# igmsalinas/unet-rir

Hardware: AMD Instinct MI355X
Metric: RIR spectrograms/sec (train step) on [B,2,256,256] U-Net (higher is better)
Workload: dtype bf16; 1 GPU; UNet 4 down/4 up, number_filters_0=64, kernels=3, per-GPU batch 32 of [2,256,256] + [2,16] (BASELINE.json configs[1] per GPU; global batch 32), full train step: fwd + loss + bwd + grad all-reduce + Adam; bf16 activations/gradients, fp32 accumulate/statistics/master weights; global_batch=32, parallelism=dp1, rccl_world_size=1, params=68613058, driven_by=Trainer.step(UNetEngine), schedule=side-stream weight gradients + bucket-wise Adam

## Files before the change

### include/unetrir.h

```cpp
#ifndef UNETRIR_H
#define UNETRIR_H

#include <stddef.h>
#include <stdint.h>

#ifdef __cplusplus
extern "C" {
#endif

#define UNETRIR_EINVAL 10001
#define UNETRIR_ABI_VERSION 1

typedef void* unetrir_stream_t;
typedef uint16_t unetrir_bf16;

typedef struct {
    int B, H, W;
    int Cin, Cout;
    int k;
    int stride;
} unetrir_conv_geom;

int unetrir_abi_version(void);

typedef struct {
    int conv3x3, conv3x3g, conv3x3g_pair, conv3x3h, conv3x3s, conv3x3r, stem, upconv3x3g, wgrad3x3g, wgrad3x3r, head_mfma,
        wgrad3x3d, conv3x3d, conv3x3p, upconv3x3q, dyn_tiles, pw1x1, igemm2;
} unetrir_config;
int unetrir_get_config(unetrir_config* out);
int unetrir_set_config(const unetrir_config* in);
int unetrir_reset_tile_tickets(void);

int unetrir_conv2d_fwd_f32(const unetrir_conv_geom* g, const float* x, int ldx, const float* w,
                           const float* bias, const float* addend, int ldadd, float* y, int ldy,
                           unetrir_stream_t stream);
int unetrir_conv2d_dgrad_f32(const unetrir_conv_geom* g, const float* dy, int lddy, const float* wt,
                             const float* addend, int ldadd, float* dx, int lddx,
                             unetrir_stream_t stream);
size_t unetrir_conv2d_wgrad_ws_bytes(const unetrir_conv_geom* g);
int unetrir_conv2d_wgrad_f32(const unetrir_conv_geom* g, const float* x, int ldx, const float* dy,
                             int lddy, float* dw, float reg_coef, const float* w, void* ws,
                             size_t ws_bytes, unetrir_stream_t stream);

int unetrir_conv2d_transpose_fwd_f32(const unetrir_conv_geom* g, const float* x, int ldx,
                                     const float* wt, const float* bias, float* y, int ldy,
                                     unetrir_stream_t stream);
int unetrir_conv2d_transpose_dgrad_f32(const unetrir_conv_geom* g, const float* dy, int lddy,
                                       const float* w, const float* addend, int ldadd, float* dx,
                                       int lddx, unetrir_stream_t stream);
size_t unetrir_conv2d_transpose_wgrad_ws_bytes(const unetrir_conv_geom* g);
int unetrir_conv2d_transpose_wgrad_f32(const unetrir_conv_geom* g, const float* x, int ldx,
                                       const float* dy, int lddy, float* dw, float reg_coef,
                                       const float* w, void* ws, size_t ws_bytes,
                                       unetrir_stream_t stream);

size_t unetrir_dense_fwd_ws_bytes(int B, int K, int N);
int unetrir_dense_fwd_f32(const float* x, int ldx, const float* w, const float* bias, float* y, int ldy, int B, int K,
                          int N, void* ws, size_t ws_bytes, unetrir_stream_t stream);
int unetrir_dense_dgrad_supported(int B, int K, int N);
size_t unetrir_dense_dgrad_ws_bytes(int B, int K, int N);
int unetrir_dense_dgrad_f32(const float* dy, int lddy, const float* w, float* dx, int lddx, int B, int K, int N, void* ws,
                            size_t ws_bytes, unetrir_stream_t stream);

int unetrir_transpose_weight_f32(const float* w, float* wt, int N, int T, int C,
                                 unetrir_stream_t stream);

size_t unetrir_bn_ws_bytes(long long P, int C);
int unetrir_bn_stats_f32(const float* x, int ldx, long long P, int C, const float* gamma,
                         const float* beta, float eps, float momentum, float* moving_mean,
                         float* moving_var, float* affine, float* saved, void* ws, size_t ws_bytes,
                         unetrir_stream_t stream);
int unetrir_bn_apply_f32(const float* x, int ldx, long long P, int C, const float* affine, int relu,
                         float* y, int ldy, unetrir_stream_t stream);
int unetrir_bn_bwd_f32(const float* da, int ldda, const float* x, int ldx, long long P, int C,
                       const float* gamma, const float* affine, const float* saved, int relu,
                       float* dx, int lddx, float* dgamma, float* dbeta, void* ws, size_t ws_bytes,
                       unetrir_stream_t stream);
int unetrir_colsum_f32(const float* x, int ldx, long long P, int C, float* out, void* ws,
                       size_t ws_bytes, unetrir_stream_t stream);
int unetrir_relu_fwd_f32(const float* x, int ldx, long long P, int C, float* y, int ldy,
                         unetrir_stream_t stream);
int unetrir_relu_bwd_f32(const float* da, int ldda, const float* x, int ldx, long long P, int C,
                         float* dx, int lddx, unetrir_stream_t stream);

int unetrir_bn_act_add_f32(const float* x, int ldx, long long P, int C, const float* affine, int act,
                           const float* addend, int ldadd, float* y, int ldy, unetrir_stream_t stream);
int unetrir_act_bwd_f32(const float* da, int ldda, const float* out, int ldo, long long P, int C, int act, float* g,
                        int ldg, unetrir_stream_t stream);
int unetrir_add_f32(const float* a, const float* b, float* y, long long n, unetrir_stream_t stream);
int unetrir_bn_bwd_junction_f32(const float* da, int ldda, const float* x, int ldx, const float* out, int ldo, long long P, int C,
                                const float* affine, const float* saved, int act, float* dx, int lddx, float* gskip, int ldgs,
                                const float* gskip_add, int ldga, float* dgamma, float* dbeta, void* ws, size_t ws_bytes,
                                unetrir_stream_t stream);

int unetrir_nchw_to_nhwc_pad_f32(const float* x, int B, int C, int H, int W, float* y, int Cpad,
                                 unetrir_stream_t stream);

size_t unetrir_loss_ws_bytes(long long npix);
int unetrir_sigmoid_loss_f32(const float* logits, int ldl, const float* target, int B, int H, int W,
                             float alpha, float inv_norm, float* pred, float* dlogits,
                             float* loss_out, void* ws, size_t ws_bytes, unetrir_stream_t stream);
int unetrir_sigmoid_loss_ex_f32(const float* logits, int ldl, const float* target, const float* phase_ref,
                                const float* phase_weight, int B, int H, int W, float alpha, float inv_norm, float* pred,
                                float* dlogits, float* loss_out, void* ws, size_t ws_bytes, unetrir_stream_t stream);
int unetrir_sigmoid_nchw_f32(const float* logits, int ldl, int B, int H, int W, float* pred,
                             unetrir_stream_t stream);
int unetrir_sigmoid_bwd_f32(const float* pred, const float* dpred, int B, int H, int W,
                            float* dlogits, unetrir_stream_t stream);

int unetrir_head6x6_supported(int C);
int unetrir_head6x6_fwd_f32(const float* x, int ldx, int B, int H, int W, int C, const float* w, const float* bias,
                            float* y, int ldy, unetrir_stream_t stream);
size_t unetrir_head6x6_wgrad_ws_bytes(int C);
int unetrir_head6x6_wgrad_f32(const float* x, int ldx, int B, int H, int W, int C, const float* dy, int lddy,
                              float* dw, void* ws, size_t ws_bytes, unetrir_stream_t stream);

int unetrir_embedding_fwd_f32(const int* idx, int n_idx, const float* table, int vocab, int dim,
                              float* out, unetrir_stream_t stream);
int unetrir_embedding_bwd_f32(const int* idx, int n_idx, const float* dout, int vocab, int dim,
                              float* dtable, unetrir_stream_t stream);
int unetrir_mul_f32(const float* x, const float* m, float* y, long long n, unetrir_stream_t stream);
int unetrir_sumsq_f32(const float* x, long long n, float coef, float* out, int accumulate,
                      void* ws, size_t ws_bytes, unetrir_stream_t stream);

int unetrir_adam_f32(float* theta, const float* g, float* m, float* v, long long n, float lr_t,
                     float beta1, float beta2, float eps, float grad_scale,
                     unetrir_stream_t stream);

int unetrir_sgd_f32(float* theta, const float* g, long long n, float lr, float grad_scale, unetrir_stream_t stream);
int unetrir_nadam_f32(float* theta, const float* g, float* m, float* v, long long n, float lr, float beta1, float beta2, float eps,
                      float c_g, float c_m, float c_v, float grad_scale, unetrir_stream_t stream);

int unetrir_step_advance(unsigned long long* state, const float* cfg, float* hyper, int n_draws, int advance_t,
                         unetrir_stream_t stream);
int unetrir_adam_dev_f32(float* theta, const float* g, float* m, float* v, long long n, const float* hyper,
                         unetrir_stream_t stream);
int unetrir_dropout_mask_dev_f32(float* mask, long long n, float p, unsigned long long seed,
                                 const unsigned long long* step_base, unsigned long long step_offset, unetrir_stream_t stream);

int unetrir_conv2d_fwd_bf16(const unetrir_conv_geom* g, const unetrir_bf16* x, int ldx, const unetrir_bf16* w,
                            const float* bias, const unetrir_bf16* addend, int ldadd, unetrir_bf16* y, int ldy,
                            unetrir_stream_t stream);
int unetrir_conv2d_dgrad_bf16(const unetrir_conv_geom* g, const unetrir_bf16* dy, int lddy, const unetrir_bf16* wt,
                              const unetrir_bf16* addend, int ldadd, unetrir_bf16* dx, int lddx,
                              unetrir_stream_t stream);
int unetrir_conv2d_wgrad_bf16(const unetrir_conv_geom* g, const unetrir_bf16* x, int ldx, const unetrir_bf16* dy,
                              int lddy, float* dw, float reg_coef, const float* w, void* ws, size_t ws_bytes,
                              unetrir_stream_t stream);
int unetrir_conv2d_transpose_fwd_bf16(const unetrir_conv_geom* g, const unetrir_bf16* x, int ldx,
                                      const unetrir_bf16* wt, const float* bias, unetrir_bf16* y, int ldy,
                                      unetrir_stream_t stream);
int unetrir_conv2d_transpose_dgrad_bf16(const unetrir_conv_geom* g, const unetrir_bf16* dy, int lddy,
                                        const unetrir_bf16* w, const unetrir_bf16* addend, int ldadd,
                                        unetrir_bf16* dx, int lddx, unetrir_stream_t stream);
int unetrir_conv2d_transpose_wgrad_bf16(const unetrir_conv_geom* g, const unetrir_bf16* x, int ldx,
                                        const unetrir_bf16* dy, int lddy, float* dw, float reg_coef, const float* w,
                                        void* ws, size_t ws_bytes, unetrir_stream_t stream);
typedef struct unetrir_reduce_desc {
    const float* part;
    int nsplit;
    size_t n;
    float* out;
    float reg;
    const float* w;
} unetrir_reduce_desc;
int unetrir_conv2d_wgrad_partials_bf16(const unetrir_conv_geom* g, const unetrir_bf16* x, int ldx, const unetrir_bf16* dy,
                                       int lddy, float* dw, float reg_coef, const float* w, void* ws, size_t ws_bytes,
                                       unetrir_reduce_desc* desc, unetrir_stream_t stream);
int unetrir_conv2d_transpose_wgrad_partials_bf16(const unetrir_conv_geom* g, const unetrir_bf16* x, int ldx,
                                                 const unetrir_bf16* dy, int lddy, float* dw, float reg_coef, const float* w,
                                                 void* ws, size_t ws_bytes, unetrir_reduce_desc* desc, unetrir_stream_t stream);
int unetrir_splitk_reduce_batched(const unetrir_reduce_desc* desc, int n, unetrir_stream_t stream);
size_t unetrir_conv3x3s2_packed_elems(int N, int C);
int unetrir_conv2d_fwd_packed_bf16(const unetrir_conv_geom* g, const unetrir_bf16* x, int ldx, const unetrir_bf16* w,
                                   const unetrir_bf16* w_packed, const float* bias, const unetrir_bf16* addend, int ldadd,
                                   unetrir_bf16* y, int ldy, unetrir_stream_t stream);
int unetrir_conv2d_transpose_dgrad_packed_bf16(const unetrir_conv_geom* g, const unetrir_bf16* dy, int lddy,
                                               const unetrir_bf16* w, const unetrir_bf16* w_packed,
                                               const unetrir_bf16* addend, int ldadd, unetrir_bf16* dx, int lddx,
                                               unetrir_stream_t stream);
int unetrir_cast_weight_bf16(const float* w, unetrir_bf16* o, int N, int T, int C, int Cp, unetrir_stream_t stream);
int unetrir_transpose_cast_weight_bf16(const float* w, unetrir_bf16* wt, int N, int T, int C, int Np,
                                       unetrir_stream_t stream);
typedef struct unetrir_cast_desc {
    const float* w;
    unetrir_bf16* same;
    unetrir_bf16* transposed;
    int N, T, C, Cp, Np, reserved;
    unetrir_bf16* packed_s2;
} unetrir_cast_desc;
int unetrir_cast_weights_batched_bf16(const unetrir_cast_desc* desc, int n_layers, unetrir_stream_t stream);
int unetrir_bn_stats_bf16(const unetrir_bf16* x, int ldx, long long P, int C, const float* gamma, const float* beta,
                          float eps, float momentum, float* moving_mean, float* moving_var, float* affine,
                          float* saved, void* ws, size_t ws_bytes, unetrir_stream_t stream);
int unetrir_bn_apply_bf16(const unetrir_bf16* x, int ldx, long long P, int C, const float* affine, int relu,
                          unetrir_bf16* y, int ldy, unetrir_stream_t stream);
int unetrir_bn_bwd_bf16(const unetrir_bf16* da, int ldda, const unetrir_bf16* x, int ldx, long long P, int C,
                        const float* affine, const float* saved, int relu, unetrir_bf16* dx, int lddx, float* dgamma,
                        float* dbeta, void* ws, size_t ws_bytes, unetrir_stream_t stream);
int unetrir_colsum_bf16(const unetrir_bf16* x, int ldx, long long P, int C, float* out, void* ws, size_t ws_bytes,
                        unetrir_stream_t stream);
int unetrir_relu_bwd_bf16(const unetrir_bf16* da, int ldda, const unetrir_bf16* x, int ldx, long long P, int C,
                          unetrir_bf16* dx, int lddx, unetrir_stream_t stream);
int unetrir_nchw_to_nhwc_pad_bf16(const float* x, int B, int C, int H, int W, unetrir_bf16* y, int Cpad,
                                  unetrir_stream_t stream);
int unetrir_head6x6_fwd_bf16(const unetrir_bf16* x, int ldx, int B, int H, int W, int C, const float* w,
                             const float* bias, float* y, int ldy, unetrir_stream_t stream);
int unetrir_head6x6_wgrad_bf16(const unetrir_bf16* x, int ldx, int B, int H, int W, int C, const unetrir_bf16* dy,
                               int lddy, float* dw, void* ws, size_t ws_bytes, unetrir_stream_t stream);
long long unetrir_conv2d_colstat_rows_bf16(const unetrir_conv_geom* g, int dgrad, int ld_in);
enum { UNETRIR_K3_TAPTABLE = 0, UNETRIR_K3_CONV3X3R = 1, UNETRIR_K3_CONV3X3G = 2, UNETRIR_K3_CONV3X3G_PAIR = 3, UNETRIR_K3_CONV3X3H = 4,
       UNETRIR_K3_CONV3X3S = 5, UNETRIR_K3_CONV3X3P = 6, UNETRIR_K3_STEM = 7, UNETRIR_K3_PATCH = 8 };
int unetrir_conv3x3_kernel_id_bf16(const unetrir_conv_geom* g, int dgrad, int ld_in);
int unetrir_conv2d_fwd_colstat_bf16(const unetrir_conv_geom* g, const unetrir_bf16* x, int ldx, const unetrir_bf16* w,
                                    const float* bias, const unetrir_bf16* addend, int ldadd, unetrir_bf16* y, int ldy,
                                    float* colstat, unetrir_stream_t stream);
int unetrir_conv2d_dgrad_colstat_bf16(const unetrir_conv_geom* g, const unetrir_bf16* dy, int lddy, const unetrir_bf16* wt,
                                      const unetrir_bf16* addend, int ldadd, unetrir_bf16* dx, int lddx, float* colstat,
                                      unetrir_stream_t stream);
long long unetrir_conv2d_transpose_colstat_rows_bf16(const unetrir_conv_geom* g, int ld_in);
int unetrir_conv2d_transpose_fwd_colstat_bf16(const unetrir_conv_geom* g, const unetrir_bf16* x, int ldx, const unetrir_bf16* wt,
                                              const float* bias, unetrir_bf16* y, int ldy, float* colstat,
                                              unetrir_stream_t stream);
int unetrir_bn_stats_colstat(const float* colstat, long long rows, long long P, int C, const float* gamma, const float* beta,
                             float eps, float momentum, float* moving_mean, float* moving_var, float* affine, float* saved,
                             unetrir_stream_t stream);
int unetrir_colsum_colstat(const float* colstat, long long rows, int ldc, int c0, int C, float* out, unetrir_stream_t stream);
int unetrir_bn_colstat_act_add_f32(const float* colstat, long long rows, const float* x, int ldx, long long P, int C, const float* gamma,
                                   const float* beta, float eps, float momentum, float* moving_mean, float* moving_var, float* affine,
                                   float* saved, int act, const float* addend, int ldadd, float* y, int ldy, unetrir_stream_t stream);
int unetrir_bn_colstat_act_add_bf16(const float* colstat, long long rows, const unetrir_bf16* x, int ldx, long long P, int C,
                                    const float* gamma, const float* beta, float eps, float momentum, float* moving_mean,
                                    float* moving_var, float* affine, float* saved, int act, const unetrir_bf16* addend, int ldadd,
                                    unetrir_bf16* y, int ldy, unetrir_stream_t stream);
int unetrir_head6x6_dgrad_supported(int W, int C);
int unetrir_head6x6_dgrad_bf16(const unetrir_bf16* dy, int lddy, int B, int H, int W, const float* w, int C,
                               unetrir_bf16* dx, int lddx, unetrir_stream_t stream);
int unetrir_sigmoid_loss_bf16(const float* logits, int ldl, const float* target, int B, int H, int W, float alpha,
                              float inv_norm, float* pred, unetrir_bf16* dlogits, float* loss_out, void* ws,
                              size_t ws_bytes, unetrir_stream_t stream);
int unetrir_sigmoid_loss_ex_bf16(const float* logits, int ldl, const float* target, const float* phase_ref,
                                 const float* phase_weight, int B, int H, int W, float alpha, float inv_norm, float* pred,
                                 unetrir_bf16* dlogits, float* loss_out, void* ws, size_t ws_bytes, unetrir_stream_t stream);
int unetrir_sigmoid_bwd_bf16(const float* pred, const float* dpred, int B, int H, int W, unetrir_bf16* dlogits,
                             unetrir_stream_t stream);
int unetrir_add_f32_to_bf16(const unetrir_bf16* a, const float* b, unetrir_bf16* y, long long n,
                            unetrir_stream_t stream);
int unetrir_cast_bf16_to_f32(const unetrir_bf16* a, float* y, long long n, unetrir_stream_t stream);
int unetrir_cast_f32_to_bf16(const float* a, unetrir_bf16* y, long long n, unetrir_stream_t stream);
int unetrir_bn_act_add_bf16(const unetrir_bf16* x, int ldx, long long P, int C, const float* affine, int act,
                            const unetrir_bf16* addend, int ldadd, unetrir_bf16* y, int ldy, unetrir_stream_t stream);
int unetrir_act_bwd_bf16(const unetrir_bf16* da, int ldda, const unetrir_bf16* out, int ldo, long long P, int C, int act,
                         unetrir_bf16* g, int ldg, unetrir_stream_t stream);
int unetrir_bn_bwd_junction_bf16(const unetrir_bf16* da, int ldda, const unetrir_bf16* x, int ldx, const unetrir_bf16* out, int ldo,
                                 long long P, int C, const float* affine, const float* saved, int act, unetrir_bf16* dx, int lddx,
                                 unetrir_bf16* gskip, int ldgs, const unetrir_bf16* gskip_add, int ldga, float* dgamma, float* dbeta,
                                 void* ws, size_t ws_bytes, unetrir_stream_t stream);

int unetrir_stft_frames(int T, int hop_length);
int unetrir_stft_features_f32(const float* wav, int B, int T, int n_fft, int win_length, int hop_length, int pad_mode,
                              int remove_mean, int normalize, float* out, int H, int W, unetrir_stream_t stream);
int unetrir_istft_features_f32(const float* feat, int B, int H, int W, int n_bins, int n_frames, int n_fft, int win_length,
                               int hop_length, int denormalize, float* wav, unetrir_stream_t stream);

int unetrir_eval_metrics_f32(const float* pred, const float* target, const float* phase_ref, int B, int H, int W,
                             const float* wav_pred, const float* wav_true, int T, int n50, double* out, unetrir_stream_t stream);
int unetrir_eval_accumulate(const double* out, const int* group, int B, int G, double* acc, unetrir_stream_t stream);

int unetrir_bn_inference_affine_f32(const float* gamma, const float* beta, const float* moving_mean, const float* moving_var,
                                    float eps, int C, float* affine, unetrir_stream_t stream);
int unetrir_dropout_mask_f32(float* mask, long long n, float p, unsigned long long seed, unsigned long long step,
                             unetrir_stream_t stream);
int unetrir_index_to_i32(const void* idx, int elem_bytes, long long n, int* out, unetrir_stream_t stream);

int unetrir_normal_f32(float* out, long long n, unsigned long long seed, unsigned long long step, unetrir_stream_t stream);
int unetrir_normal_dev_f32(float* out, long long n, unsigned long long seed, const unsigned long long* step_base,
                           unsigned long long step_offset, unetrir_stream_t stream);
int unetrir_vae_sample_kl_fwd_f32(const float* mu, int ld_mu, const float* log_var, int ld_lv, const float* eps, int B, int L,
                                  float inv_global_batch, float* z, int ld_z, float* kl_out, unetrir_stream_t stream);
int unetrir_vae_sample_kl_bwd_f32(const float* mu, int ld_mu, const float* log_var, int ld_lv, const float* eps, const float* dz,
                                  int ld_dz, int B, int L, float inv_global_batch, float* dmu, int ld_dmu, float* dlv, int ld_dlv,
                                  unetrir_stream_t stream);
int unetrir_vae_loss_add_f32(const float* kl_out, float* loss_out, unetrir_stream_t stream);

int unetrir_stage_h2d(int n, const void* const* src, void* const* pinned, void* const* dev, const size_t* bytes,
                      unetrir_stream_t stream);

int unetrir_gather_batch_f32(const float* bank, long long N, long long row_elems, const int32_t* emb_bank, int emb_len,
                             const float* wav_bank, long long wav_len, const int32_t* room_bank, const int32_t* idx_in,
                             const int32_t* idx_out, int B, float* spec_in, float* spec_out, int32_t* emb, float* wav_true,
                             int32_t* room, unetrir_stream_t stream);

size_t unetrir_griffinlim_ws_bytes(int B, int n_bins, int n_frames, int n_fft);
int unetrir_griffinlim_f32(const float* feat, int B, int H, int W, int n_bins, int n_frames, int n_fft, int win_length,
                           int hop_length, int pad_mode, int denormalize, int n_iter, float momentum, const float* init_phase,
                           unsigned long long seed, unsigned long long draw, float* wav, void* ws, size_t ws_bytes,
                           unetrir_stream_t stream);
int unetrir_uniform_f32(float* out, long long n, unsigned long long seed, unsigned long long step, unetrir_stream_t stream);

#define UNETRIR_PROF_FAMILIES 8
enum { UNETRIR_FAM_CONV_FWD = 0, UNETRIR_FAM_CONV_DGRAD = 1, UNETRIR_FAM_CONV_WGRAD = 2,
       UNETRIR_FAM_BN = 3, UNETRIR_FAM_OTHER = 4, UNETRIR_FAM_SMALL_CHANNEL = 5,
       UNETRIR_FAM_DOMINANT = 6  };
int unetrir_prof_enable(int on);
int unetrir_prof_collect(int* counts, double* ms, double* flops);

#ifdef __cplusplus
}
#endif
#endif
```

### unet-rir_amd/_lib.py

```python
import ctypes as C
import os

from . import build as _build

_LIB = None

c_f32p = C.c_void_p
c_stream = C.c_void_p


class CastDesc(C.Structure):
    _fields_ = [("w", C.c_void_p), ("same", C.c_void_p), ("transposed", C.c_void_p), ("N", C.c_int), ("T", C.c_int), ("C", C.c_int),
                ("Cp", C.c_int), ("Np", C.c_int), ("reserved", C.c_int), ("packed_s2", C.c_void_p)]


class ReduceDesc(C.Structure):
    _fields_ = [("part", C.c_void_p), ("nsplit", C.c_int), ("n", C.c_size_t), ("out", C.c_void_p), ("reg", C.c_float), ("w", C.c_void_p)]


class Config(C.Structure):
    _fields_ = [(n, C.c_int) for n in ("conv3x3", "conv3x3g", "conv3x3g_pair", "conv3x3h", "conv3x3s", "conv3x3r", "stem",
                                       "upconv3x3g", "wgrad3x3g", "wgrad3x3r", "head_mfma", "wgrad3x3d", "conv3x3d", "conv3x3p", "upconv3x3q", "dyn_tiles", "pw1x1", "igemm2")]


class ConvGeom(C.Structure):
    _fields_ = [("B", C.c_int), ("H", C.c_int), ("W", C.c_int), ("Cin", C.c_int), ("Cout", C.c_int),
                ("k", C.c_int), ("stride", C.c_int)]


_SIGS = {
    "unetrir_abi_version": (C.c_int, []),
    "unetrir_get_config": (C.c_int, [C.POINTER(Config)]),
    "unetrir_set_config": (C.c_int, [C.POINTER(Config)]),
    "unetrir_conv2d_fwd_f32": (C.c_int, [C.POINTER(ConvGeom), c_f32p, C.c_int, c_f32p, c_f32p, c_f32p, C.c_int,
                                         c_f32p, C.c_int, c_stream]),
    "unetrir_conv2d_dgrad_f32": (C.c_int, [C.POINTER(ConvGeom), c_f32p, C.c_int, c_f32p, c_f32p, C.c_int, c_f32p,
                                           C.c_int, c_stream]),
    "unetrir_conv2d_wgrad_ws_bytes": (C.c_size_t, [C.POINTER(ConvGeom)]),
    "unetrir_conv2d_wgrad_f32": (C.c_int, [C.POINTER(ConvGeom), c_f32p, C.c_int, c_f32p, C.c_int, c_f32p, C.c_float,
                                           c_f32p, C.c_void_p, C.c_size_t, c_stream]),
    "unetrir_conv2d_transpose_fwd_f32": (C.c_int, [C.POINTER(ConvGeom), c_f32p, C.c_int, c_f32p, c_f32p, c_f32p,
                                                   C.c_int, c_stream]),
    "unetrir_conv2d_transpose_dgrad_f32": (C.c_int, [C.POINTER(ConvGeom), c_f32p, C.c_int, c_f32p, c_f32p, C.c_int,
                                                     c_f32p, C.c_int, c_stream]),
    "unetrir_conv2d_transpose_wgrad_ws_bytes": (C.c_size_t, [C.POINTER(ConvGeom)]),
    "unetrir_conv2d_transpose_wgrad_f32": (C.c_int, [C.POINTER(ConvGeom), c_f32p, C.c_int, c_f32p, C.c_int, c_f32p,
                                                     C.c_float, c_f32p, C.c_void_p, C.c_size_t, c_stream]),
    "unetrir_dense_fwd_ws_bytes": (C.c_size_t, [C.c_int, C.c_int, C.c_int]),
    "unetrir_dense_fwd_f32": (C.c_int, [c_f32p, C.c_int, c_f32p, c_f32p, c_f32p, C.c_int, C.c_int, C.c_int, C.c_int,
                                        C.c_void_p, C.c_size_t, c_stream]),
    "unetrir_transpose_weight_f32": (C.c_int, [c_f32p, c_f32p, C.c_int, C.c_int, C.c_int, c_stream]),
    "unetrir_bn_ws_bytes": (C.c_size_t, [C.c_longlong, C.c_int]),
    "unetrir_bn_stats_f32": (C.c_int, [c_f32p, C.c_int, C.c_longlong, C.c_int, c_f32p, c_f32p, C.c_float, C.c_float,
                                       c_f32p, c_f32p, c_f32p, c_f32p, C.c_void_p, C.c_size_t, c_stream]),
    "unetrir_bn_apply_f32": (C.c_int, [c_f32p, C.c_int, C.c_longlong, C.c_int, c_f32p, C.c_int, c_f32p, C.c_int,
                                       c_stream]),
    "unetrir_bn_bwd_f32": (C.c_int, [c_f32p, C.c_int, c_f32p, C.c_int, C.c_longlong, C.c_int, c_f32p, c_f32p, c_f32p,
                                     C.c_int, c_f32p, C.c_int, c_f32p, c_f32p, C.c_void_p, C.c_size_t, c_stream]),
    "unetrir_colsum_f32": (C.c_int, [c_f32p, C.c_int, C.c_longlong, C.c_int, c_f32p, C.c_void_p, C.c_size_t,
                                     c_stream]),
    "unetrir_relu_fwd_f32": (C.c_int, [c_f32p, C.c_int, C.c_longlong, C.c_int, c_f32p, C.c_int, c_stream]),
    "unetrir_relu_bwd_f32": (C.c_int, [c_f32p, C.c_int, c_f32p, C.c_int, C.c_longlong, C.c_int, c_f32p, C.c_int,
                                       c_stream]),
    "unetrir_bn_act_add_f32": (C.c_int, [c_f32p, C.c_int, C.c_longlong, C.c_int, c_f32p, C.c_int, c_f32p, C.c_int, c_f32p,
                                         C.c_int, c_stream]),
    "unetrir_act_bwd_f32": (C.c_int, [c_f32p, C.c_int, c_f32p, C.c_int, C.c_longlong, C.c_int, C.c_int, c_f32p, C.c_int,
                                      c_stream]),
    "unetrir_add_f32": (C.c_int, [c_f32p, c_f32p, c_f32p, C.c_longlong, c_stream]),
    "unetrir_nchw_to_nhwc_pad_f32": (C.c_int, [c_f32p, C.c_int, C.c_int, C.c_int, C.c_int, c_f32p, C.c_int,
                                               c_stream]),
    "unetrir_head6x6_supported": (C.c_int, [C.c_int]),
    "unetrir_head6x6_fwd_f32": (C.c_int, [c_f32p, C.c_int, C.c_int, C.c_int, C.c_int, C.c_int, c_f32p, c_f32p, c_f32p,
                                          C.c_int, c_stream]),
    "unetrir_head6x6_wgrad_ws_bytes": (C.c_size_t, [C.c_int]),
    "unetrir_head6x6_wgrad_f32": (C.c_int, [c_f32p, C.c_int, C.c_int, C.c_int, C.c_int, C.c_int, c_f32p, C.c_int, c_f32p,
                                            C.c_void_p, C.c_size_t, c_stream]),
    "unetrir_loss_ws_bytes": (C.c_size_t, [C.c_longlong]),
    "unetrir_sigmoid_loss_f32": (C.c_int, [c_f32p, C.c_int, c_f32p, C.c_int, C.c_int, C.c_int, C.c_float, C.c_float,
                                           c_f32p, c_f32p, c_f32p, C.c_void_p, C.c_size_t, c_stream]),
    "unetrir_sigmoid_nchw_f32": (C.c_int, [c_f32p, C.c_int, C.c_int, C.c_int, C.c_int, c_f32p, c_stream]),
    "unetrir_sigmoid_bwd_f32": (C.c_int, [c_f32p, c_f32p, C.c_int, C.c_int, C.c_int, c_f32p, c_stream]),
    "unetrir_embedding_fwd_f32": (C.c_int, [C.c_void_p, C.c_int, c_f32p, C.c_int, C.c_int, c_f32p, c_stream]),
    "unetrir_embedding_bwd_f32": (C.c_int, [C.c_void_p, C.c_int, c_f32p, C.c_int, C.c_int, c_f32p, c_stream]),
    "unetrir_mul_f32": (C.c_int, [c_f32p, c_f32p, c_f32p, C.c_longlong, c_stream]),
    "unetrir_sumsq_f32": (C.c_int, [c_f32p, C.c_longlong, C.c_float, c_f32p, C.c_int, C.c_void_p, C.c_size_t,
                                    c_stream]),
    "unetrir_adam_f32": (C.c_int, [c_f32p, c_f32p, c_f32p, c_f32p, C.c_longlong, C.c_float, C.c_float, C.c_float,
                                   C.c_float, C.c_float, c_stream]),
    "unetrir_conv2d_fwd_bf16": (C.c_int, [C.POINTER(ConvGeom), c_f32p, C.c_int, c_f32p, c_f32p, c_f32p, C.c_int,
                                          c_f32p, C.c_int, c_stream]),
    "unetrir_conv3x3s2_packed_elems": (C.c_size_t, [C.c_int, C.c_int]),
    "unetrir_conv2d_fwd_packed_bf16": (C.c_int, [C.POINTER(ConvGeom), c_f32p, C.c_int, c_f32p, c_f32p, c_f32p, c_f32p, C.c_int,
                                                 c_f32p, C.c_int, c_stream]),
    "unetrir_conv2d_transpose_dgrad_packed_bf16": (C.c_int, [C.POINTER(ConvGeom), c_f32p, C.c_int, c_f32p, c_f32p, c_f32p, C.c_int,
                                                             c_f32p, C.c_int, c_stream]),
    "unetrir_conv2d_dgrad_bf16": (C.c_int, [C.POINTER(ConvGeom), c_f32p, C.c_int, c_f32p, c_f32p, C.c_int, c_f32p,
                                            C.c_int, c_stream]),
    "unetrir_conv2d_wgrad_bf16": (C.c_int, [C.POINTER(ConvGeom), c_f32p, C.c_int, c_f32p, C.c_int, c_f32p, C.c_float,
                                            c_f32p, C.c_void_p, C.c_size_t, c_stream]),
    "unetrir_conv2d_transpose_fwd_bf16": (C.c_int, [C.POINTER(ConvGeom), c_f32p, C.c_int, c_f32p, c_f32p, c_f32p,
                                                    C.c_int, c_stream]),
    "unetrir_conv2d_transpose_dgrad_bf16": (C.c_int, [C.POINTER(ConvGeom), c_f32p, C.c_int, c_f32p, c_f32p, C.c_int,
                                                      c_f32p, C.c_int, c_stream]),
    "unetrir_conv2d_wgrad_partials_bf16": (C.c_int, [C.POINTER(ConvGeom), c_f32p, C.c_int, c_f32p, C.c_int, c_f32p, C.c_float, c_f32p,
                                                     C.c_void_p, C.c_size_t, C.POINTER(ReduceDesc), c_stream]),
    "unetrir_conv2d_transpose_wgrad_partials_bf16": (C.c_int, [C.POINTER(ConvGeom), c_f32p, C.c_int, c_f32p, C.c_int, c_f32p, C.c_float,
                                                               c_f32p, C.c_void_p, C.c_size_t, C.POINTER(ReduceDesc), c_stream]),
    "unetrir_splitk_reduce_batched": (C.c_int, [C.POINTER(ReduceDesc), C.c_int, c_stream]),
    "unetrir_conv2d_transpose_wgrad_bf16": (C.c_int, [C.POINTER(ConvGeom), c_f32p, C.c_int, c_f32p, C.c_int, c_f32p,
                                                      C.c_float, c_f32p, C.c_void_p, C.c_size_t, c_stream]),
    "unetrir_cast_weight_bf16": (C.c_int, [c_f32p, c_f32p, C.c_int, C.c_int, C.c_int, C.c_int, c_stream]),
    "unetrir_transpose_cast_weight_bf16": (C.c_int, [c_f32p, c_f32p, C.c_int, C.c_int, C.c_int, C.c_int, c_stream]),
    "unetrir_bn_stats_bf16": (C.c_int, [c_f32p, C.c_int, C.c_longlong, C.c_int, c_f32p, c_f32p, C.c_float, C.c_float,
                                        c_f32p, c_f32p, c_f32p, c_f32p, C.c_void_p, C.c_size_t, c_stream]),
    "unetrir_bn_apply_bf16": (C.c_int, [c_f32p, C.c_int, C.c_longlong, C.c_int, c_f32p, C.c_int, c_f32p, C.c_int,
                                        c_stream]),
    "unetrir_bn_bwd_bf16": (C.c_int, [c_f32p, C.c_int, c_f32p, C.c_int, C.c_longlong, C.c_int, c_f32p, c_f32p,
                                      C.c_int, c_f32p, C.c_int, c_f32p, c_f32p, C.c_void_p, C.c_size_t, c_stream]),
    "unetrir_colsum_bf16": (C.c_int, [c_f32p, C.c_int, C.c_longlong, C.c_int, c_f32p, C.c_void_p, C.c_size_t,
                                      c_stream]),
    "unetrir_relu_bwd_bf16": (C.c_int, [c_f32p, C.c_int, c_f32p, C.c_int, C.c_longlong, C.c_int, c_f32p, C.c_int,
                                        c_stream]),
    "unetrir_nchw_to_nhwc_pad_bf16": (C.c_int, [c_f32p, C.c_int, C.c_int, C.c_int, C.c_int, c_f32p, C.c_int,
                                                c_stream]),
    "unetrir_head6x6_fwd_bf16": (C.c_int, [c_f32p, C.c_int, C.c_int, C.c_int, C.c_int, C.c_int, c_f32p, c_f32p, c_f32p,
                                           C.c_int, c_stream]),
    "unetrir_head6x6_wgrad_bf16": (C.c_int, [c_f32p, C.c_int, C.c_int, C.c_int, C.c_int, C.c_int, c_f32p, C.c_int,
                                             c_f32p, C.c_void_p, C.c_size_t, c_stream]),
    "unetrir_stage_h2d": (C.c_int, [C.c_int, C.POINTER(C.c_void_p), C.POINTER(C.c_void_p), C.POINTER(C.c_void_p), C.POINTER(C.c_size_t), c_stream]),
    "unetrir_conv2d_colstat_rows_bf16": (C.c_longlong, [C.POINTER(ConvGeom), C.c_int, C.c_int]),
    "unetrir_conv3x3_kernel_id_bf16": (C.c_int, [C.POINTER(ConvGeom), C.c_int, C.c_int]),
    "unetrir_conv2d_fwd_colstat_bf16": (C.c_int, [C.POINTER(ConvGeom), c_f32p, C.c_int, c_f32p, c_f32p, c_f32p, C.c_int, c_f32p, C.c_int,
                                                  c_f32p, c_stream]),
    "unetrir_conv2d_dgrad_colstat_bf16": (C.c_int, [C.POINTER(ConvGeom), c_f32p, C.c_int, c_f32p, c_f32p, C.c_int, c_f32p, C.c_int,
                                                    c_f32p, c_stream]),
    "unetrir_conv2d_transpose_colstat_rows_bf16": (C.c_longlong, [C.POINTER(ConvGeom), C.c_int]),
    "unetrir_conv2d_transpose_fwd_colstat_bf16": (C.c_int, [C.POINTER(ConvGeom), c_f32p, C.c_int, c_f32p, c_f32p, c_f32p, C.c_int, c_f32p,
                                                            c_stream]),
    "unetrir_bn_stats_colstat": (C.c_int, [c_f32p, C.c_longlong, C.c_longlong, C.c_int, c_f32p, c_f32p, C.c_float, C.c_float,
                                           c_f32p, c_f32p, c_f32p, c_f32p, c_stream]),
    "unetrir_bn_colstat_act_add_f32": (C.c_int, [c_f32p, C.c_longlong, c_f32p, C.c_int, C.c_longlong, C.c_int, c_f32p, c_f32p, C.c_float, C.c_float, c_f32p, c_f32p, c_f32p, c_f32p, C.c_int, c_f32p, C.c_int, c_f32p, C.c_int, c_stream]),
    "unetrir_bn_colstat_act_add_bf16": (C.c_int, [c_f32p, C.c_longlong, c_f32p, C.c_int, C.c_longlong, C.c_int, c_f32p, c_f32p, C.c_float, C.c_float, c_f32p, c_f32p, c_f32p, c_f32p, C.c_int, c_f32p, C.c_int, c_f32p, C.c_int, c_stream]),
    "unetrir_colsum_colstat": (C.c_int, [c_f32p, C.c_longlong, C.c_int, C.c_int, C.c_int, c_f32p, c_stream]),
    "unetrir_cast_weights_batched_bf16": (C.c_int, [C.c_void_p, C.c_int, c_stream]),
    "unetrir_dense_dgrad_supported": (C.c_int, [C.c_int, C.c_int, C.c_int]),
    "unetrir_dense_dgrad_ws_bytes": (C.c_size_t, [C.c_int, C.c_int, C.c_int]),
    "unetrir_dense_dgrad_f32": (C.c_int, [c_f32p, C.c_int, c_f32p, c_f32p, C.c_int, C.c_int, C.c_int, C.c_int, C.c_void_p, C.c_size_t,
                                          c_stream]),
    "unetrir_stft_frames": (C.c_int, [C.c_int, C.c_int]),
    "unetrir_stft_features_f32": (C.c_int, [c_f32p, C.c_int, C.c_int, C.c_int, C.c_int, C.c_int, C.c_int, C.c_int, C.c_int,
                                            c_f32p, C.c_int, C.c_int, c_stream]),
    "unetrir_istft_features_f32": (C.c_int, [c_f32p, C.c_int, C.c_int, C.c_int, C.c_int, C.c_int, C.c_int, C.c_int, C.c_int,
                                             C.c_int, c_f32p, c_stream]),
    "unetrir_eval_metrics_f32": (C.c_int, [c_f32p, c_f32p, c_f32p, C.c_int, C.c_int, C.c_int, c_f32p, c_f32p, C.c_int, C.c_int,
                                           C.c_void_p, c_stream]),
    "unetrir_eval_accumulate": (C.c_int, [C.c_void_p, C.c_void_p, C.c_int, C.c_int, C.c_void_p, c_stream]),
    "unetrir_head6x6_dgrad_supported": (C.c_int, [C.c_int, C.c_int]),
    "unetrir_head6x6_dgrad_bf16": (C.c_int, [c_f32p, C.c_int, C.c_int, C.c_int, C.c_int, c_f32p, C.c_int, c_f32p, C.c_int,
                                             c_stream]),
    "unetrir_sigmoid_loss_bf16": (C.c_int, [c_f32p, C.c_int, c_f32p, C.c_int, C.c_int, C.c_int, C.c_float, C.c_float,
                                            c_f32p, c_f32p, c_f32p, C.c_void_p, C.c_size_t, c_stream]),
    "unetrir_sigmoid_bwd_bf16": (C.c_int, [c_f32p, c_f32p, C.c_int, C.c_int, C.c_int, c_f32p, c_stream]),
    "unetrir_add_f32_to_bf16": (C.c_int, [c_f32p, c_f32p, c_f32p, C.c_longlong, c_stream]),
    "unetrir_cast_bf16_to_f32": (C.c_int, [c_f32p, c_f32p, C.c_longlong, c_stream]),
    "unetrir_cast_f32_to_bf16": (C.c_int, [c_f32p, c_f32p, C.c_longlong, c_stream]),
    "unetrir_bn_act_add_bf16": (C.c_int, [c_f32p, C.c_int, C.c_longlong, C.c_int, c_f32p, C.c_int, c_f32p, C.c_int, c_f32p,
                                          C.c_int, c_stream]),
    "unetrir_act_bwd_bf16": (C.c_int, [c_f32p, C.c_int, c_f32p, C.c_int, C.c_longlong, C.c_int, C.c_int, c_f32p, C.c_int,
                                       c_stream]),
    "unetrir_bn_inference_affine_f32": (C.c_int, [c_f32p, c_f32p, c_f32p, c_f32p, C.c_float, C.c_int, c_f32p, c_stream]),
    "unetrir_dropout_mask_f32": (C.c_int, [c_f32p, C.c_longlong, C.c_float, C.c_ulonglong, C.c_ulonglong, c_stream]),
    "unetrir_index_to_i32": (C.c_int, [C.c_void_p, C.c_int, C.c_longlong, C.c_void_p, c_stream]),
    "unetrir_reset_tile_tickets": (C.c_int, []),
    "unetrir_bn_bwd_junction_f32": (C.c_int, [c_f32p, C.c_int, c_f32p, C.c_int, c_f32p, C.c_int, C.c_longlong, C.c_int, c_f32p, c_f32p, C.c_int, c_f32p, C.c_int, c_f32p, C.c_int, c_f32p, C.c_int, c_f32p, c_f32p, C.c_void_p, C.c_size_t, c_stream]),
    "unetrir_bn_bwd_junction_bf16": (C.c_int, [c_f32p, C.c_int, c_f32p, C.c_int, c_f32p, C.c_int, C.c_longlong, C.c_int, c_f32p, c_f32p, C.c_int, c_f32p, C.c_int, c_f32p, C.c_int, c_f32p, C.c_int, c_f32p, c_f32p, C.c_void_p, C.c_size_t, c_stream]),
    "unetrir_sigmoid_loss_ex_f32": (C.c_int, [c_f32p, C.c_int, c_f32p, c_f32p, c_f32p, C.c_int, C.c_int, C.c_int, C.c_float, C.c_float,
                                              c_f32p, c_f32p, c_f32p, C.c_void_p, C.c_size_t, c_stream]),
    "unetrir_sigmoid_loss_ex_bf16": (C.c_int, [c_f32p, C.c_int, c_f32p, c_f32p, c_f32p, C.c_int, C.c_int, C.c_int, C.c_float, C.c_float,
                                               c_f32p, c_f32p, c_f32p, C.c_void_p, C.c_size_t, c_stream]),
    "unetrir_sgd_f32": (C.c_int, [c_f32p, c_f32p, C.c_longlong, C.c_float, C.c_float, c_stream]),
    "unetrir_nadam_f32": (C.c_int, [c_f32p, c_f32p, c_f32p, c_f32p, C.c_longlong, C.c_float, C.c_float, C.c_float, C.c_float, C.c_float,
                                    C.c_float, C.c_float, C.c_float, c_stream]),
    "unetrir_step_advance": (C.c_int, [C.c_void_p, c_f32p, c_f32p, C.c_int, C.c_int, c_stream]),
    "unetrir_adam_dev_f32": (C.c_int, [c_f32p, c_f32p, c_f32p, c_f32p, C.c_longlong, c_f32p, c_stream]),
    "unetrir_dropout_mask_dev_f32": (C.c_int, [c_f32p, C.c_longlong, C.c_float, C.c_ulonglong, C.c_void_p, C.c_ulonglong, c_stream]),
    "unetrir_normal_f32": (C.c_int, [c_f32p, C.c_longlong, C.c_ulonglong, C.c_ulonglong, c_stream]),
    "unetrir_normal_dev_f32": (C.c_int, [c_f32p, C.c_longlong, C.c_ulonglong, C.c_void_p, C.c_ulonglong, c_stream]),
    "unetrir_vae_sample_kl_fwd_f32": (C.c_int, [c_f32p, C.c_int, c_f32p, C.c_int, c_f32p, C.c_int, C.c_int, C.c_float, c_f32p, C.c_int,
                                                c_f32p, c_stream]),
    "unetrir_vae_sample_kl_bwd_f32": (C.c_int, [c_f32p, C.c_int, c_f32p, C.c_int, c_f32p, c_f32p, C.c_int, C.c_int, C.c_int, C.c_float,
                                                c_f32p, C.c_int, c_f32p, C.c_int, c_stream]),
    "unetrir_vae_loss_add_f32": (C.c_int, [c_f32p, c_f32p, c_stream]),
    "unetrir_gather_batch_f32": (C.c_int, [c_f32p, C.c_longlong, C.c_longlong, C.c_void_p, C.c_int, c_f32p, C.c_longlong, C.c_void_p,
                                           C.c_void_p, C.c_void_p, C.c_int, c_f32p, c_f32p, C.c_void_p, c_f32p, C.c_void_p, c_stream]),
    "unetrir_griffinlim_ws_bytes": (C.c_size_t, [C.c_int, C.c_int, C.c_int, C.c_int]),
    "unetrir_griffinlim_f32": (C.c_int, [c_f32p, C.c_int, C.c_int, C.c_int, C.c_int, C.c_int, C.c_int, C.c_int, C.c_int, C.c_int,
                                         C.c_int, C.c_int, C.c_float, c_f32p, C.c_ulonglong, C.c_ulonglong, c_f32p, C.c_void_p,
                                         C.c_size_t, c_stream]),
    "unetrir_uniform_f32": (C.c_int, [c_f32p, C.c_longlong, C.c_ulonglong, C.c_ulonglong, c_stream]),
    "unetrir_prof_enable": (C.c_int, [C.c_int]),
    "unetrir_prof_collect": (C.c_int, [C.POINTER(C.c_int), C.POINTER(C.c_double), C.POINTER(C.c_double)]),
}

EXPORTS = tuple(_SIGS)
PROF_FAMILIES = 8


class UnetrirError(RuntimeError):
    pass


_LIB_PATH = None


def use_library(path):
    global _LIB_PATH
    if _LIB is not None:
        raise UnetrirError("the library is already loaded")
    _LIB_PATH = path


def lib():
    global _LIB
    if _LIB is not None:
        return _LIB
    path = _LIB_PATH or _build.LIB
    if _LIB_PATH is None and _build.needs_build():
        path = _build.build()
    if not os.path.exists(path):
        raise UnetrirError(f"HIP extension missing: {path}")
    L = C.CDLL(path)
    for name, (res, args) in _SIGS.items():
        fn = getattr(L, name)
        fn.restype = res
        fn.argtypes = args
    if L.unetrir_abi_version() != 1:
        raise UnetrirError("libunetrir.so ABI version mismatch")
    _LIB = L
    return L


def check(err, what):
    if err != 0:
        raise UnetrirError(f"{what} failed with code {err}")
```

### unet-rir_amd/build.py

```python
import os
import subprocess
import sys
from concurrent.futures import ThreadPoolExecutor

HERE = os.path.dirname(os.path.abspath(__file__))
CSRC = os.path.join(HERE, "csrc")
OBJ = os.path.join(HERE, "build")
LIB = os.path.join(HERE, "libunetrir.so")
SOURCES = ["igemm.hip", "api.hip", "elementwise.hip", "head.hip", "head_mfma.hip", "wgrad3x3.hip", "wgrad3x3r.hip", "wgrad3x3g.hip", "wgrad3x3d.hip", "igemm_bf16.hip", "conv3x3.hip", "conv3x3r.hip", "conv3x3g.hip", "conv3x3h.hip", "conv3x3s.hip", "conv3x3d.hip", "conv3x3p.hip", "upconv3x3.hip", "upconv3x3g.hip", "upconv3x3q.hip", "features.hip", "dense.hip", "stem3x3.hip", "pw1x1.hip", "igemm2_bf16.hip", "evalmetrics.hip", "vae.hip", "dataset.hip", "griffinlim.hip"]
FLAGS = ["-O3", "--offload-arch=gfx950", "-std=c++17", "-fPIC", "-Wno-unused-value"]


def _headers():
    return [os.path.join(CSRC, f) for f in os.listdir(CSRC) if f.endswith(".h")] + [
        os.path.join(os.path.dirname(HERE), "include", "unetrir.h")]


def _stale(target, deps):
    if not os.path.exists(target):
        return True
    t = os.path.getmtime(target)
    return any(os.path.getmtime(d) > t for d in deps)


def needs_build():
    deps = [os.path.join(CSRC, f) for f in os.listdir(CSRC)] + _headers()
    return _stale(LIB, deps)


def build(force=False, verbose=False, extra_flags=(), lib=LIB, obj_dir=OBJ):
    if not force and lib == LIB and not needs_build():
        return LIB
    hipcc = os.environ.get("HIPCC", "/opt/rocm/bin/hipcc")
    os.makedirs(obj_dir, exist_ok=True)
    hdrs = _headers()
    jobs = []
    for s in SOURCES:
        src = os.path.join(CSRC, s)
        obj = os.path.join(obj_dir, s[:-4] + ".o")
        if force or _stale(obj, [src] + hdrs):
            jobs.append([hipcc] + FLAGS + list(extra_flags) + ["-c", src, "-o", obj])

    def run(cmd):
        if verbose:
            print(" ".join(cmd), file=sys.stderr)
        subprocess.run(cmd, check=True)

    with ThreadPoolExecutor(max_workers=min(8, os.cpu_count() or 1)) as ex:
        list(ex.map(run, jobs))
    run([hipcc, "--offload-arch=gfx950", "-shared", "-fPIC", "-o", lib] +
        [os.path.join(obj_dir, s[:-4] + ".o") for s in SOURCES])
    return lib


ABL_LIB = os.path.join(HERE, "libunetrir_abl.so")


def build_ablations(verbose=False):
    return build(force=False, verbose=verbose, extra_flags=["-DUNETRIR_ABLATIONS"], lib=ABL_LIB, obj_dir=os.path.join(HERE, "build_abl"))


if __name__ == "__main__":
    if "--ablations" in sys.argv:
        print(build_ablations(verbose=True))
    else:
        print(build(force="--force" in sys.argv, verbose=True))
```

### unet-rir_amd/csrc/api.hip

```cpp
#include <hip/hip_runtime.h>
#include <cstdlib>
#include <cstring>
#include <atomic>
#include <mutex>
#include <utility>
#include <vector>
#include "kernels.h"

namespace {
int env_int(const char* name, int dflt) {
    const char* e = getenv(name);
    return e ? atoi(e) : dflt;
}
const unetrir_config* load_config() {
    unetrir_config* c = new unetrir_config;
    c->conv3x3 = env_int("UNETRIR_CONV3X3", 1);
    c->conv3x3g = env_int("UNETRIR_CONV3X3G", 1);
    c->conv3x3g_pair = env_int("UNETRIR_CONV3X3G_PAIR", 1);
    c->conv3x3h = env_int("UNETRIR_CONV3X3H", 1);
    c->conv3x3s = env_int("UNETRIR_CONV3X3S", 1);
    c->conv3x3r = env_int("UNETRIR_CONV3X3R", 1);
    c->stem = env_int("UNETRIR_STEM", 1);
    c->upconv3x3g = env_int("UNETRIR_UPCONV3X3G", 1);
    c->wgrad3x3g = env_int("UNETRIR_WGRAD3X3G", 1);
    c->wgrad3x3r = env_int("UNETRIR_WGRAD3X3R", 1);
    c->wgrad3x3d = env_int("UNETRIR_WGRAD3X3D", 1);
    c->conv3x3d = env_int("UNETRIR_CONV3X3D", 1);
    c->conv3x3p = env_int("UNETRIR_CONV3X3P", 1);
    c->upconv3x3q = env_int("UNETRIR_UPCONV3X3Q", 1);
    c->dyn_tiles = env_int("UNETRIR_DYN_TILES", 1);
    c->head_mfma = env_int("UNETRIR_HEAD_MFMA", 1);
    c->pw1x1 = env_int("UNETRIR_PW1X1", 1);
    c->igemm2 = env_int("UNETRIR_IGEMM2", 1);
    return c;
}
std::atomic<const unetrir_config*>& config_slot() {
    static std::atomic<const unetrir_config*> p{load_config()};
    return p;
}
}
const unetrir_config& unetrir_cfg() { return *config_slot().load(std::memory_order_acquire); }
extern "C" int unetrir_get_config(unetrir_config* out) {
    if (!out) return UNETRIR_EINVAL;
    *out = unetrir_cfg();
    return 0;
}
extern "C" int unetrir_set_config(const unetrir_config* in) {
    if (!in) return UNETRIR_EINVAL;
    config_slot().store(new unetrir_config(*in), std::memory_order_release);
    return 0;
}

#ifdef UNETRIR_ABLATIONS
int g_unetrir_abl = 0;
extern "C" int unetrir_abl_set(int v) { g_unetrir_abl = v; return 0; }
__global__ void abl_hog_kernel(long long cycles, int lds, unsigned* sink) {
    extern __shared__ unsigned hog_smem[];
    if (lds > 0) hog_smem[threadIdx.x] = threadIdx.x;
    const long long t0 = wall_clock64();
    unsigned acc = 0;
    while (wall_clock64() - t0 < cycles) acc += hog_smem[(threadIdx.x + acc) & 63];
    if (acc == 0xFFFFFFFFu) *sink = acc;
}
extern "C" int unetrir_abl_hog(int n, long long cycles, int lds, void* sink, void* stream) {
    hipLaunchKernelGGL(abl_hog_kernel, dim3(n), dim3(256), (size_t)lds, (hipStream_t)stream, cycles, lds, (unsigned*)sink);
    return (int)hipGetLastError();
}
#endif

__device__ unsigned g_sched_slots[128][80];
namespace {
struct SlotTable { std::atomic<unsigned*> sched{nullptr}; hipStream_t owner[128]; std::atomic<int> used{0}; };
constexpr int MAX_DEV = 16;
std::mutex g_slot_mu;
SlotTable g_slot_tab[MAX_DEV];

int slot_index(hipStream_t s, unsigned** base) {
    int dev = -1;
    if (hipGetDevice(&dev) != hipSuccess || dev < 0 || dev >= MAX_DEV) return -1;
    SlotTable& d = g_slot_tab[dev];
    unsigned* sched = d.sched.load(std::memory_order_acquire);
    if (sched) {
        const int n = d.used.load(std::memory_order_acquire);
        for (int i = 0; i < n; ++i) if (d.owner[i] == s) { *base = sched; return i; }
    }
    std::lock_guard<std::mutex> lk(g_slot_mu);
    sched = d.sched.load(std::memory_order_relaxed);
    if (!sched) {
        void* p = nullptr;
        if (hipGetSymbolAddress(&p, HIP_SYMBOL(g_sched_slots)) != hipSuccess) return -1;
        if (hipMemset(p, 0, sizeof(unsigned) * 128 * 80) != hipSuccess) {
            (void)hipGetLastError();
            return -1;
        }
        sched = (unsigned*)p;
        d.sched.store(sched, std::memory_order_release);
    }
    *base = sched;
    const int n = d.used.load(std::memory_order_relaxed);
    for (int i = 0; i < n; ++i) if (d.owner[i] == s) return i;
    if (n == 128) return -1;
    d.owner[n] = s;
    d.used.store(n + 1, std::memory_order_release);
    return n;
}
}

unsigned* sched_slot(hipStream_t s) {
    if (!unetrir_cfg().dyn_tiles) return nullptr;
    unsigned* base = nullptr;
    const int i = slot_index(s, &base);
    return i < 0 ? nullptr : base + i * 80;
}

extern "C" int unetrir_reset_tile_tickets(void) {
    void* p = nullptr;
    if (hipGetSymbolAddress(&p, HIP_SYMBOL(g_sched_slots)) != hipSuccess) return UNETRIR_EINVAL;
    return (int)hipMemset(p, 0, sizeof(unsigned) * 128 * 80);
}

namespace {

struct Same { int out, before; };
inline Same same_geom(int n_in, int k, int s) {
    Same r;
    r.out = (n_in + s - 1) / s;
    int total = (r.out - 1) * s + k - n_in;
    if (total < 0) total = 0;
    r.before = total / 2;
    return r;
}

inline uint32_t pack_tap(int dy, int dx, int widx) {
    return (uint32_t)(uint8_t)(int8_t)dy | ((uint32_t)(uint8_t)(int8_t)dx << 8) | ((uint32_t)widx << 16);
}

inline bool geom_ok(const unetrir_conv_geom* g) {
    return g && g->B > 0 && g->H > 0 && g->W > 0 && g->Cin > 0 && g->Cout > 0 && g->k >= 1 && g->k <= 6 &&
           (g->stride == 1 || g->stride == 2);
}

struct ProfRec { int fam, tag; hipEvent_t e0, e1; double flops; };
std::mutex g_prof_mu;
bool g_prof_on = false;
unsigned g_prof_mask = ~0u;
std::vector<ProfRec> g_prof;

struct ProfScope {
    bool on; ProfRec r; hipStream_t s;
    ProfScope(int fam, double flops, hipStream_t st, int tag = -1) : on(g_prof_on && ((g_prof_mask >> fam) & 1u)), s(st) {
        if (!on) return;
        r.fam = fam; r.tag = tag; r.flops = flops;
        hipEventCreate(&r.e0); hipEventCreate(&r.e1);
        hipEventRecord(r.e0, s);
    }
    ~ProfScope() {
        if (!on) return;
        hipEventRecord(r.e1, s);
        std::lock_guard<std::mutex> lk(g_prof_mu);
        g_prof.push_back(r);
    }
};

inline double conv_flops(const unetrir_conv_geom* g) {
    const Same sy = same_geom(g->H, g->k, g->stride), sx = same_geom(g->W, g->k, g->stride);
    return 2.0 * g->B * sy.out * sx.out * (double)g->Cout * g->Cin * g->k * g->k;
}
inline int conv_family(const unetrir_conv_geom* g, int fam) {
    return (g->Cin <= 8 || g->Cout <= 8) ? 5 : fam;
}

enum class Kern { TAPTABLE, TAPTABLE_CLASSES, PATCH, STEM, CONV3X3G_PAIR, CONV3X3P, CONV3X3G, CONV3X3S, CONV3X3H, CONV3X3R, CONV3X3D,
                  UPCONV3X3, UPCONV3X3G, UPCONV3X3Q, PW1X1 };
struct ConvPlan {
    Kern kernel;
    long long colstat_rows;
};

enum Dir { FWD, DGRAD, TFWD };
struct ConvCall {
    const unetrir_conv_geom* g; Dir dir;
    const void* in; int ldi; const void* w; const void* wpk; const float* bias; const void* addend; int ldadd; void* out; int ldo;
    float* colstat;
};

inline double patch_util(int H, int W) { return (double)H * W / ((double)((H + 7) / 8 * 8) * ((W + 31) / 32 * 32)); }

Conv3Args conv3_args(const ConvCall& c) {
    const unetrir_conv_geom* g = c.g;
    const bool dg = c.dir != FWD;
    Conv3Args a{};
    a.in = c.in; a.ldi = c.ldi; a.w = c.w; a.bias = c.bias; a.addend = c.addend; a.ldadd = c.ldadd; a.out = c.out; a.ldo = c.ldo;
    a.colstat = c.colstat;
    a.B = g->B; a.H = g->H; a.W = g->W; a.C = dg ? g->Cout : g->Cin; a.N = dg ? g->Cin : g->Cout;
    if (g->stride == 1) {
        a.flip = dg ? 1 : UNETRIR_ABL(UNETRIR_ABL_HOST(), 256) ? 2 : 0;
    } else if (dg) {
        a.H = same_geom(g->H, 3, 2).out; a.W = same_geom(g->W, 3, 2).out;
    } else {
        a.wpk = (g->Cin % 64 == 0 && g->Cout % 64 == 0) ? c.wpk : nullptr;
    }
    return a;
}

PwArgs pw_args(const ConvCall& c) {
    const unetrir_conv_geom* g = c.g;
    const Same sy = same_geom(g->H, 1, g->stride), sx = same_geom(g->W, 1, g->stride);
    PwArgs a{};
    a.in = (const __bf16*)c.in; a.ldi = c.ldi; a.w = (const __bf16*)c.w; a.bias = c.bias; a.addend = (const __bf16*)c.addend;
    a.ldadd = c.ldadd; a.out = (__bf16*)c.out; a.ldo = c.ldo; a.colstat = c.colstat;
    a.B = g->B; a.PH = sy.out; a.PW = sx.out;
    if (c.dir == FWD) {
        a.IH = g->H; a.IW = g->W; a.OH = sy.out; a.OW = sx.out; a.SI = g->stride; a.SO = 1; a.C = g->Cin; a.N = g->Cout;
    } else {
        a.IH = sy.out; a.IW = sx.out; a.OH = g->H; a.OW = g->W; a.SI = 1; a.SO = g->stride; a.fill = g->stride == 2; a.C = g->Cout;
        a.N = g->Cin;
    }
    return a;
}

long long taptable_rows(const unetrir_conv_geom* g, Dir dir) {
    const Same sy = same_geom(g->H, g->k, g->stride), sx = same_geom(g->W, g->k, g->stride);
    if (dir == FWD) return igemm_colstat_rows((long long)g->B * sy.out * sx.out, g->Cout);
    if (g->stride == 1) return igemm_colstat_rows((long long)g->B * g->H * g->W, g->Cin);
    return 4 * igemm_colstat_rows((long long)g->B * sy.out * sx.out, g->Cin, 4);
}

ConvPlan plan_conv(const ConvCall& c, bool bf16, bool stats) {
    const unetrir_config& cfg = unetrir_cfg();
    const unetrir_conv_geom* g = c.g;
    if (g->k == 3 && g->stride == 1) {
        const Conv3Args a = conv3_args(c);
        const bool pair = bf16 && cfg.conv3x3g_pair && conv3x3g_pair_applies(a, cfg.conv3x3g_pair == 2);
        if ((cfg.conv3x3 && patch_util(g->H, g->W) >= 0.7) || pair) {
            if (!bf16) return {Kern::PATCH, 0};
            if (cfg.stem && !stats && stem3x3_applies(a)) return {Kern::STEM, 0};
            if (cfg.conv3x3g) {
                if (pair) return {Kern::CONV3X3G_PAIR, conv3x3g_colstat_rows(a, true)};
                if (cfg.conv3x3p && conv3x3p_applies(a)) return {Kern::CONV3X3P, conv3x3p_colstat_rows(a)};
                if (conv3x3g_applies(a)) return {Kern::CONV3X3G, conv3x3g_colstat_rows(a, false)};
            }
            if (cfg.conv3x3s && conv3x3s_applies(a)) return {Kern::CONV3X3S, conv3x3s_colstat_rows(a)};
            if (cfg.conv3x3h && conv3x3h_applies(a)) return {Kern::CONV3X3H, conv3x3h_colstat_rows(a)};
            if (cfg.conv3x3r && !(a.flip & 2)) return {Kern::CONV3X3R, conv3x3r_colstat_rows(a)};
            return {Kern::PATCH, 0};
        }
    }
    if (bf16 && g->k == 1 && cfg.pw1x1 && !(stats && c.addend) && pw1x1_applies(pw_args(c)))
        return {Kern::PW1X1, pw1x1_colstat_rows(pw_args(c))};
    if (g->stride == 1) return {Kern::TAPTABLE, taptable_rows(g, c.dir)};
    if (c.dir == FWD) {
        if (bf16 && g->k == 3 && cfg.conv3x3d && conv3x3d_applies(conv3_args(c))) return {Kern::CONV3X3D, 0};
        return {Kern::TAPTABLE, g->k == 3 ? 0 : taptable_rows(g, c.dir)};
    }
    const Same sy = same_geom(g->H, g->k, 2), sx = same_geom(g->W, g->k, 2);
    if (g->k == 3 && sy.before == 0 && sx.before == 0 && g->H == 2 * sy.out && g->W == 2 * sx.out && patch_util(sy.out, sx.out) >= 0.7) {
        const Conv3Args a = conv3_args(c);
        if (bf16 && cfg.upconv3x3g && upconv3x3g_applies(a))
            return {cfg.upconv3x3q && upconv3x3q_applies(a) ? Kern::UPCONV3X3Q : Kern::UPCONV3X3G, 0};
        if (cfg.conv3x3) return {Kern::UPCONV3X3, 0};
    }
    return {Kern::TAPTABLE_CLASSES, c.dir == TFWD && g->k != 3 ? taptable_rows(g, c.dir) : 0};
}

struct F32 {
    static constexpr int is_bf16 = 0;
    using T = float; using Args = IgemmArgs;
    static int launch(const Args& a, hipStream_t s) { return launch_igemm_fwd(a, s); }
    static int launch_classes(const Args* a, hipStream_t s) {
        for (int i = 0; i < 4; ++i) { const int err = launch_igemm_fwd(a[i], s); if (err) return err; }
        return 0;
    }
};
struct BF16 {
    static constexpr int is_bf16 = 1;
    using T = __bf16; using Args = IgemmArgsH;
    static int launch(const Args& a, hipStream_t s) { return launch_igemm_fwd_bf16(a, s); }
    static int launch_classes(const Args* a, hipStream_t s) {
        return launch_igemm_fwd_bf16_x4(a, s);
    }
};

template <class P>
int launch_taptable(const ConvCall& c, hipStream_t s) {
    const unetrir_conv_geom* g = c.g;
    const Same sy = same_geom(g->H, g->k, g->stride), sx = same_geom(g->W, g->k, g->stride);
    typename P::Args a{};
    a.g.B = g->B; a.g.wtaps = g->k * g->k; a.g.ntaps = g->k * g->k; a.g.SI = 1; a.g.SO = 1; a.g.ooy = 0; a.g.oox = 0;
    a.g.ldi = c.ldi; a.g.ldo = c.ldo;
    a.in = (const typename P::T*)c.in; a.w = (const typename P::T*)c.w; a.bias = c.bias; a.addend = (const typename P::T*)c.addend;
    a.ldadd = c.ldadd; a.out = (typename P::T*)c.out;
    if constexpr (P::is_bf16) a.colstat = c.colstat;
    if (c.dir == FWD) {
        a.g.PH = sy.out; a.g.PW = sx.out; a.g.IH = g->H; a.g.IW = g->W; a.g.C = g->Cin;
        a.g.OH = sy.out; a.g.OW = sx.out; a.g.N = g->Cout; a.g.SI = g->stride;
        for (int kh = 0; kh < g->k; ++kh)
            for (int kw = 0; kw < g->k; ++kw)
                a.g.tap[kh * g->k + kw] = pack_tap(kh - sy.before, kw - sx.before, kh * g->k + kw);
        return P::launch(a, s);
    }
    a.g.IH = sy.out; a.g.IW = sx.out; a.g.C = g->Cout;
    a.g.OH = g->H; a.g.OW = g->W; a.g.N = g->Cin;
    if (g->stride == 1) {
        a.g.PH = g->H; a.g.PW = g->W;
        for (int kh = 0; kh < g->k; ++kh)
            for (int kw = 0; kw < g->k; ++kw)
                a.g.tap[kh * g->k + kw] = pack_tap(-(kh - sy.before), -(kw - sx.before), kh * g->k + kw);
        return P::launch(a, s);
    }
    a.g.PH = (g->H + 1) / 2; a.g.PW = (g->W + 1) / 2; a.g.SO = 2;
    typename P::Args cls[4];
    for (int ay = 0; ay < 2; ++ay)
        for (int ax = 0; ax < 2; ++ax) {
            int nt = 0;
            for (int kh = 0; kh < g->k; ++kh) {
                const int offy = kh - sy.before;
                if (((offy - ay) & 1) != 0) continue;
                for (int kw = 0; kw < g->k; ++kw) {
                    const int offx = kw - sx.before;
                    if (((offx - ax) & 1) != 0) continue;
                    a.g.tap[nt++] = pack_tap((ay - offy) / 2, (ax - offx) / 2, kh * g->k + kw);
                }
            }
            a.g.ntaps = nt; a.g.ooy = ay; a.g.oox = ax;
            if constexpr (P::is_bf16) {
                if (c.colstat) a.colstat = c.colstat + (size_t)(ay * 2 + ax) * igemm_colstat_rows((long long)g->B * a.g.PH * a.g.PW, g->Cin, 4) * g->Cin * 2;
            }
            cls[ay * 2 + ax] = a;
        }
    return P::launch_classes(cls, s);
}

template <class P>
int launch_planned(const ConvCall& c, Kern k, hipStream_t s) {
    switch (k) {
        case Kern::TAPTABLE: case Kern::TAPTABLE_CLASSES: return launch_taptable<P>(c, s);
        case Kern::PATCH: return launch_conv3x3(conv3_args(c), P::is_bf16, s);
        case Kern::STEM: return launch_stem3x3_bf16(conv3_args(c), s);
        case Kern::CONV3X3G_PAIR: return launch_conv3x3g_bf16(conv3_args(c), true, s);
        case Kern::CONV3X3P: return launch_conv3x3p_bf16(conv3_args(c), s);
        case Kern::CONV3X3G: return launch_conv3x3g_bf16(conv3_args(c), false, s);
        case Kern::CONV3X3S: return launch_conv3x3s_bf16(conv3_args(c), s);
        case Kern::CONV3X3H: return launch_conv3x3h_bf16(conv3_args(c), s);
        case Kern::CONV3X3R: return launch_conv3x3r_bf16(conv3_args(c), s);
        case Kern::CONV3X3D: return launch_conv3x3d_bf16(conv3_args(c), s);
        case Kern::UPCONV3X3: return launch_upconv3x3(conv3_args(c), P::is_bf16, s);
        case Kern::UPCONV3X3G: return launch_upconv3x3g_bf16(conv3_args(c), s);
        case Kern::UPCONV3X3Q: return launch_upconv3x3q_bf16(conv3_args(c), s);
        case Kern::PW1X1: return launch_pw1x1_bf16(pw_args(c), s);
    }
    return UNETRIR_EINVAL;
}

template <class P>
int run_conv(const ConvCall& c, int fam, double flops, hipStream_t s, bool dominant = false) {
    const ConvPlan p = plan_conv(c, P::is_bf16, c.colstat != nullptr);
    if (c.colstat && p.colstat_rows == 0) return UNETRIR_EINVAL;
    ProfScope ps(fam, flops, s, dominant && p.kernel == Kern::CONV3X3P ? UNETRIR_FAM_DOMINANT : -1);
    return launch_planned<P>(c, p.kernel, s);
}

ConvPlan plan_query(const unetrir_conv_geom* g, Dir dir, int ld_in, bool stats) {
    const ConvCall c{g, dir, nullptr, ld_in, nullptr, nullptr, nullptr, nullptr, 0, nullptr, dir == FWD ? g->Cout : g->Cin, nullptr};
    return plan_conv(c, true, stats);
}

enum class WgKern { TAPTABLE, PATCH, PATCH1X1, WGRAD3X3G, WGRAD3X3R, WGRAD3X3D };
struct WgradPlan {
    WgKern kernel;
    int nslabs;
    long long per_split;
    int npy, npx;
};

void wgrad_args(const unetrir_conv_geom* g, int ldx, int lddy, WgradArgs* a) {
    const Same sy = same_geom(g->H, g->k, g->stride), sx = same_geom(g->W, g->k, g->stride);
    a->g.B = g->B; a->g.PH = sy.out; a->g.PW = sx.out;
    a->g.IH = g->H; a->g.IW = g->W; a->g.C = g->Cin; a->g.ldi = ldx;
    a->g.N = g->Cout; a->g.SI = g->stride;
    a->g.ntaps = g->k * g->k; a->g.wtaps = g->k * g->k;
    for (int kh = 0; kh < g->k; ++kh)
        for (int kw = 0; kw < g->k; ++kw)
            a->g.tap[kh * g->k + kw] = pack_tap(kh - sy.before, kw - sx.before, kh * g->k + kw);
    a->lddy = lddy;
}

template <class A>
A wgrad3_args(const unetrir_conv_geom* g, const void* x, int ldx, const void* dy, int lddy) {
    const Same sy = same_geom(g->H, g->k, g->stride), sx = same_geom(g->W, g->k, g->stride);
    A a{};
    a.x = (decltype(a.x))x; a.ldx = ldx; a.IH = g->H; a.IW = g->W;
    a.dy = (decltype(a.dy))dy; a.lddy = lddy; a.OH = sy.out; a.OW = sx.out;
    a.B = g->B; a.C = g->Cin; a.N = g->Cout;
    a.pad_t = sy.before; a.pad_l = sx.before;
    return a;
}

WgradPlan plan_patch(WgKern kernel, int tph, int tpw, const unetrir_conv_geom* g) {
    const Same sy = same_geom(g->H, g->k, g->stride), sx = same_geom(g->W, g->k, g->stride);
    WgradPlan p{kernel};
    p.npy = (sy.out + tph - 1) / tph;
    p.npx = (sx.out + tpw - 1) / tpw;
    const long long G = (long long)g->B * p.npy * p.npx;
    const long long tiles = (long long)((g->Cout + 63) / 64) * ((g->Cin + 63) / 64);
    long long want = (512 + tiles - 1) / tiles;
    long long maxs = (G + 3) / 4;
    if (maxs < 1) maxs = 1;
    if (want > maxs) want = maxs;
    if (want < 1) want = 1;
    p.per_split = (G + want - 1) / want;
    p.nslabs = (int)((G + p.per_split - 1) / p.per_split);
    return p;
}
WgradPlan plan_wgrad3x3g(const unetrir_conv_geom* g) {
    WgradPlan p = plan_patch(WgKern::WGRAD3X3G, WG_ROW_TPH, WG_ROW_TPW, g);
    p.nslabs = (p.nslabs + 1) / 2;
    return p;
}
WgradPlan plan_wgrad3x3d(const unetrir_conv_geom* g) {
    const Same sy = same_geom(g->H, 3, 2), sx = same_geom(g->W, 3, 2);
    WgradPlan p{WgKern::WGRAD3X3D};
    int per;
    wgrad3x3d_plan(g->B, sy.out, sx.out, g->Cout, g->Cin, &p.nslabs, &per, &p.npy, &p.npx);
    p.per_split = per;
    return p;
}
WgradPlan plan_taptable(const unetrir_conv_geom* g) {
    WgradArgs a{};
    wgrad_args(g, g->Cin, g->Cout, &a);
    WgradPlan p{WgKern::TAPTABLE};
    wgrad_plan(a.g, &p.nslabs, &p.per_split);
    return p;
}

WgradPlan plan_wgrad(const unetrir_conv_geom* g, bool bf16, int ldx, int lddy) {
    const unetrir_config& cfg = unetrir_cfg();
    const bool s1 = g->stride == 1;
    if (g->k == 3 && !bf16) return plan_patch(WgKern::PATCH, s1 ? WG_F32_TPH_S1 : WG_F32_TPH_S2, WG_TPW, g);
    if (g->k == 3) {
        const Wgrad3ArgsH a = wgrad3_args<Wgrad3ArgsH>(g, nullptr, ldx, nullptr, lddy);
        if (s1 && cfg.wgrad3x3g && wgrad3x3g_applies(a, true)) return plan_wgrad3x3g(g);
        if (s1 && cfg.wgrad3x3r && wgrad3x3r_applies(a)) return plan_patch(WgKern::WGRAD3X3R, WG_ROW_TPH, WG_ROW_TPW, g);
        if (!s1 && cfg.wgrad3x3d && wgrad3x3d_applies(a, true)) return plan_wgrad3x3d(g);
        return plan_patch(WgKern::PATCH, s1 ? WG_BF16_TPH_S1 : WG_BF16_TPH_S2, WG_TPW, g);
    }
    if (g->k == 1 && bf16) return plan_patch(WgKern::PATCH1X1, s1 ? WG_1X1_TPH_S1 : WG_1X1_TPH_S2, WG_TPW, g);
    return plan_taptable(g);
}

size_t wgrad_ws_bytes(const unetrir_conv_geom* g) {
    int slabs = 0;
    auto cover = [&](const WgradPlan& p) { if (p.nslabs > slabs) slabs = p.nslabs; };
    if (g->k == 3) {
        const Wgrad3ArgsH a = wgrad3_args<Wgrad3ArgsH>(g, nullptr, g->Cin, nullptr, g->Cout);
        const bool s1 = g->stride == 1;
        cover(plan_patch(WgKern::PATCH, s1 ? WG_F32_TPH_S1 : WG_F32_TPH_S2, WG_TPW, g));
        cover(plan_patch(WgKern::PATCH, s1 ? WG_BF16_TPH_S1 : WG_BF16_TPH_S2, WG_TPW, g));
        if (s1 && wgrad3x3g_applies(a, false)) cover(plan_wgrad3x3g(g));
        if (s1 && wgrad3x3r_applies(a)) cover(plan_patch(WgKern::WGRAD3X3R, WG_ROW_TPH, WG_ROW_TPW, g));
        if (!s1 && wgrad3x3d_applies(a, false)) cover(plan_wgrad3x3d(g));
    } else {
        cover(plan_taptable(g));
        if (g->k == 1) {
            cover(plan_patch(WgKern::PATCH1X1, WG_1X1_TPH_S1, WG_TPW, g));
            cover(plan_patch(WgKern::PATCH1X1, WG_1X1_TPH_S2, WG_TPW, g));
        }
    }
    return (size_t)slabs * g->Cout * g->k * g->k * g->Cin * sizeof(float);
}

int launch_wgrad(const unetrir_conv_geom* g, const WgradPlan& p, bool bf16, const void* x, int ldx, const void* dy, int lddy, float* part,
                 hipStream_t s) {
    if (p.kernel == WgKern::TAPTABLE) {
        WgradArgs a{};
        wgrad_args(g, ldx, lddy, &a);
        a.x = (const float*)x; a.dy = (const float*)dy; a.part = part; a.chunks_per_split = p.per_split;
        return launch_igemm_wgrad(a, p.nslabs, s, bf16);
    }
    if (!bf16) {
        Wgrad3Args a = wgrad3_args<Wgrad3Args>(g, x, ldx, dy, lddy);
        a.part = part; a.patches_per_split = (int)p.per_split; a.npy = p.npy; a.npx = p.npx;
        return launch_wgrad3x3(a, g->stride, p.nslabs, s);
    }
    Wgrad3ArgsH a = wgrad3_args<Wgrad3ArgsH>(g, x, ldx, dy, lddy);
    a.part = part; a.patches_per_split = (int)p.per_split; a.npy = p.npy; a.npx = p.npx;
    switch (p.kernel) {
        case WgKern::WGRAD3X3G: return launch_wgrad3x3g_bf16(a, p.nslabs, s);
        case WgKern::WGRAD3X3R: return launch_wgrad3x3r_bf16(a, p.nslabs, s);
        case WgKern::WGRAD3X3D: return launch_wgrad3x3d_bf16(a, p.nslabs, s);
        case WgKern::PATCH1X1: return launch_wgrad1x1_bf16(a, g->stride, p.nslabs, s);
        default: return launch_wgrad3x3_bf16(a, g->stride, p.nslabs, s);
    }
}

inline unetrir_conv_geom adjoint_geom(const unetrir_conv_geom* g) {
    unetrir_conv_geom c = *g;
    c.H = g->H * g->stride; c.W = g->W * g->stride;
    c.Cin = g->Cout; c.Cout = g->Cin;
    return c;
}

inline bool ld_ok(int ld, int c) { return ld >= c && (ld & 3) == 0; }
inline bool ldh_ok(int ld, int c) { return ld >= c && (ld & 7) == 0; }

template <class P>
int run_wgrad(const unetrir_conv_geom* gin, bool transposed, const void* x, int ldx, const void* dy, int lddy, float* dw, float reg,
              const float* w, void* ws, size_t ws_bytes, unetrir_reduce_desc* defer, hipStream_t s) {
    if (defer) *defer = unetrir_reduce_desc{};
    if (!geom_ok(gin)) return UNETRIR_EINVAL;
    const unetrir_conv_geom g = transposed ? adjoint_geom(gin) : *gin;
    if (transposed) { std::swap(x, dy); std::swap(ldx, lddy); }
    const bool ld_fits = P::is_bf16 ? (g.Cin & 7) == 0 && (g.Cout & 7) == 0 && ldh_ok(ldx, g.Cin) && ldh_ok(lddy, g.Cout)
                                    : (g.Cin & 3) == 0 && ld_ok(ldx, g.Cin) && ld_ok(lddy, g.Cout);
    if (!x || !dy || !dw || !ld_fits || (reg != 0.f && !w)) return UNETRIR_EINVAL;
    ProfScope ps(conv_family(&g, UNETRIR_FAM_CONV_WGRAD), conv_flops(&g), s);
    const WgradPlan p = plan_wgrad(&g, P::is_bf16, ldx, lddy);
    const size_t nout = (size_t)g.Cout * g.k * g.k * g.Cin;
    const bool direct = p.nslabs == 1 && reg == 0.f;
    if (!direct && ws_bytes < (size_t)p.nslabs * nout * sizeof(float)) return UNETRIR_EINVAL;
    float* part = direct ? dw : (float*)ws;
    const int err = launch_wgrad(&g, p, P::is_bf16, x, ldx, dy, lddy, part, s);
    if (err || direct) return err;
    if (!defer) return launch_splitk_reduce(part, p.nslabs, nout, dw, reg, w, s);
    *defer = unetrir_reduce_desc{part, p.nslabs, nout, dw, reg, w};
    return 0;
}

}

extern "C" {

int unetrir_abi_version(void) { return UNETRIR_ABI_VERSION; }

int unetrir_conv2d_fwd_f32(const unetrir_conv_geom* g, const float* x, int ldx, const float* w, const float* bias,
                           const float* addend, int ldadd, float* y, int ldy, unetrir_stream_t stream) {
    if (!geom_ok(g) || !x || !w || !y || (g->Cin & 3) || !ld_ok(ldx, g->Cin) || ldy < g->Cout) return UNETRIR_EINVAL;
    return run_conv<F32>({g, FWD, x, ldx, w, nullptr, bias, addend, ldadd, y, ldy, nullptr}, conv_family(g, UNETRIR_FAM_CONV_FWD),
                         conv_flops(g), (hipStream_t)stream);
}

int unetrir_conv2d_dgrad_f32(const unetrir_conv_geom* g, const float* dy, int lddy, const float* wt,
                             const float* addend, int ldadd, float* dx, int lddx, unetrir_stream_t stream) {
    if (!geom_ok(g) || !dy || !wt || !dx || (g->Cout & 3) || !ld_ok(lddy, g->Cout) || lddx < g->Cin) return UNETRIR_EINVAL;
    return run_conv<F32>({g, DGRAD, dy, lddy, wt, nullptr, nullptr, addend, ldadd, dx, lddx, nullptr},
                         conv_family(g, UNETRIR_FAM_CONV_DGRAD), conv_flops(g), (hipStream_t)stream);
}

size_t unetrir_conv2d_wgrad_ws_bytes(const unetrir_conv_geom* g) { return geom_ok(g) ? wgrad_ws_bytes(g) : 0; }

int unetrir_conv2d_wgrad_f32(const unetrir_conv_geom* g, const float* x, int ldx, const float* dy, int lddy, float* dw,
                             float reg_coef, const float* w, void* ws, size_t ws_bytes, unetrir_stream_t stream) {
    return run_wgrad<F32>(g, false, x, ldx, dy, lddy, dw, reg_coef, w, ws, ws_bytes, nullptr, (hipStream_t)stream);
}

int unetrir_conv2d_transpose_fwd_f32(const unetrir_conv_geom* g, const float* x, int ldx, const float* wt,
                                     const float* bias, float* y, int ldy, unetrir_stream_t stream) {
    if (!geom_ok(g) || !x || !wt || !y || (g->Cin & 3) || !ld_ok(ldx, g->Cin) || ldy < g->Cout)
        return UNETRIR_EINVAL;
    const unetrir_conv_geom c = adjoint_geom(g);
    return run_conv<F32>({&c, TFWD, x, ldx, wt, nullptr, bias, nullptr, 0, y, ldy, nullptr}, conv_family(g, UNETRIR_FAM_CONV_FWD),
                         conv_flops(&c), (hipStream_t)stream);
}

int unetrir_conv2d_transpose_dgrad_f32(const unetrir_conv_geom* g, const float* dy, int lddy, const float* w,
                                       const float* addend, int ldadd, float* dx, int lddx, unetrir_stream_t stream) {
    if (!geom_ok(g) || !dy || !w || !dx || (g->Cout & 3) || !ld_ok(lddy, g->Cout) || lddx < g->Cin)
        return UNETRIR_EINVAL;
    const unetrir_conv_geom c = adjoint_geom(g);
    return run_conv<F32>({&c, FWD, dy, lddy, w, nullptr, nullptr, addend, ldadd, dx, lddx, nullptr},
                         conv_family(g, UNETRIR_FAM_CONV_DGRAD), conv_flops(&c), (hipStream_t)stream);
}

size_t unetrir_conv2d_transpose_wgrad_ws_bytes(const unetrir_conv_geom* g) {
    if (!geom_ok(g)) return 0;
    const unetrir_conv_geom c = adjoint_geom(g);
    return wgrad_ws_bytes(&c);
}

int unetrir_conv2d_transpose_wgrad_f32(const unetrir_conv_geom* g, const float* x, int ldx, const float* dy, int lddy,
                                       float* dw, float reg_coef, const float* w, void* ws, size_t ws_bytes,
                                       unetrir_stream_t stream) {
    return run_wgrad<F32>(g, true, x, ldx, dy, lddy, dw, reg_coef, w, ws, ws_bytes, nullptr, (hipStream_t)stream);
}

int unetrir_conv2d_fwd_bf16(const unetrir_conv_geom* g, const unetrir_bf16* x, int ldx, const unetrir_bf16* w, const float* bias,
                            const unetrir_bf16* addend, int ldadd, unetrir_bf16* y, int ldy, unetrir_stream_t stream) {
    if (!geom_ok(g) || !x || !w || !y || (g->Cin & 7) || !ldh_ok(ldx, g->Cin) || ldy < g->Cout) return UNETRIR_EINVAL;
    return run_conv<BF16>({g, FWD, x, ldx, w, nullptr, bias, addend, ldadd, y, ldy, nullptr}, conv_family(g, UNETRIR_FAM_CONV_FWD),
                          conv_flops(g), (hipStream_t)stream, true);
}

size_t unetrir_conv3x3s2_packed_elems(int N, int C) {
    if (N <= 0 || C <= 0 || (N & 63) || (C & 63)) return 0;
    return (size_t)((N + 127) / 128) * 128 * 9 * C;
}

int unetrir_conv2d_fwd_packed_bf16(const unetrir_conv_geom* g, const unetrir_bf16* x, int ldx, const unetrir_bf16* w,
                                   const unetrir_bf16* w_packed, const float* bias, const unetrir_bf16* addend, int ldadd,
                                   unetrir_bf16* y, int ldy, unetrir_stream_t stream) {
    if (!geom_ok(g) || !x || !w || !y || (g->Cin & 7) || !ldh_ok(ldx, g->Cin) || ldy < g->Cout) return UNETRIR_EINVAL;
    return run_conv<BF16>({g, FWD, x, ldx, w, w_packed, bias, addend, ldadd, y, ldy, nullptr}, conv_family(g, UNETRIR_FAM_CONV_FWD),
                          conv_flops(g), (hipStream_t)stream);
}

int unetrir_conv2d_dgrad_bf16(const unetrir_conv_geom* g, const unetrir_bf16* dy, int lddy, const unetrir_bf16* wt,
                              const unetrir_bf16* addend, int ldadd, unetrir_bf16* dx, int lddx, unetrir_stream_t stream) {
    if (!geom_ok(g) || !dy || !wt || !dx || (g->Cout & 7) || !ldh_ok(lddy, g->Cout) || lddx < g->Cin) return UNETRIR_EINVAL;
    return run_conv<BF16>({g, DGRAD, dy, lddy, wt, nullptr, nullptr, addend, ldadd, dx, lddx, nullptr},
                          conv_family(g, UNETRIR_FAM_CONV_DGRAD), conv_flops(g), (hipStream_t)stream, true);
}

long long unetrir_conv2d_colstat_rows_bf16(const unetrir_conv_geom* g, int dgrad, int ld_in) {
    return geom_ok(g) ? plan_query(g, dgrad ? DGRAD : FWD, ld_in, true).colstat_rows : 0;
}

long long unetrir_conv2d_transpose_colstat_rows_bf16(const unetrir_conv_geom* g, int ld_in) {
    if (!geom_ok(g)) return 0;
    const unetrir_conv_geom c = adjoint_geom(g);
    return plan_query(&c, TFWD, ld_in, true).colstat_rows;
}

int unetrir_conv3x3_kernel_id_bf16(const unetrir_conv_geom* g, int dgrad, int ld_in) {
    if (!geom_ok(g) || g->k != 3 || g->stride != 1) return UNETRIR_K3_TAPTABLE;
    switch (plan_query(g, dgrad ? DGRAD : FWD, ld_in, false).kernel) {
        case Kern::PATCH: return UNETRIR_K3_PATCH;
        case Kern::STEM: return UNETRIR_K3_STEM;
        case Kern::CONV3X3G_PAIR: return UNETRIR_K3_CONV3X3G_PAIR;
        case Kern::CONV3X3P: return UNETRIR_K3_CONV3X3P;
        case Kern::CONV3X3G: return UNETRIR_K3_CONV3X3G;
        case Kern::CONV3X3S: return UNETRIR_K3_CONV3X3S;
        case Kern::CONV3X3H: return UNETRIR_K3_CONV3X3H;
        case Kern::CONV3X3R: return UNETRIR_K3_CONV3X3R;
        default: return UNETRIR_K3_TAPTABLE;
    }
}

int unetrir_conv2d_fwd_colstat_bf16(const unetrir_conv_geom* g, const unetrir_bf16* x, int ldx, const unetrir_bf16* w, const float* bias,
                                    const unetrir_bf16* addend, int ldadd, unetrir_bf16* y, int ldy, float* colstat,
                                    unetrir_stream_t stream) {
    if (!geom_ok(g) || !x || !w || !y || !colstat || (g->Cin & 7) || !ldh_ok(ldx, g->Cin) || ldy < g->Cout) return UNETRIR_EINVAL;
    return run_conv<BF16>({g, FWD, x, ldx, w, nullptr, bias, addend, ldadd, y, ldy, colstat}, conv_family(g, UNETRIR_FAM_CONV_FWD),
                          conv_flops(g), (hipStream_t)stream, true);
}

int unetrir_conv2d_dgrad_colstat_bf16(const unetrir_conv_geom* g, const unetrir_bf16* dy, int lddy, const unetrir_bf16* wt,
                                      const unetrir_bf16* addend, int ldadd, unetrir_bf16* dx, int lddx, float* colstat,
                                      unetrir_stream_t stream) {
    if (!geom_ok(g) || !dy || !wt || !dx || !colstat || (g->Cout & 7) || !ldh_ok(lddy, g->Cout) || lddx < g->Cin) return UNETRIR_EINVAL;
    return run_conv<BF16>({g, DGRAD, dy, lddy, wt, nullptr, nullptr, addend, ldadd, dx, lddx, colstat},
                          conv_family(g, UNETRIR_FAM_CONV_DGRAD), conv_flops(g), (hipStream_t)stream, true);
}

int unetrir_conv2d_transpose_fwd_colstat_bf16(const unetrir_conv_geom* g, const unetrir_bf16* x, int ldx, const unetrir_bf16* wt,
                                              const float* bias, unetrir_bf16* y, int ldy, float* colstat, unetrir_stream_t stream) {
    if (!geom_ok(g) || !x || !wt || !y || !colstat || (g->Cin & 7) || !ldh_ok(ldx, g->Cin) || ldy < g->Cout) return UNETRIR_EINVAL;
    const unetrir_conv_geom c = adjoint_geom(g);
    return run_conv<BF16>({&c, TFWD, x, ldx, wt, nullptr, bias, nullptr, 0, y, ldy, colstat}, conv_family(g, UNETRIR_FAM_CONV_FWD),
                          conv_flops(&c), (hipStream_t)stream);
}

int unetrir_conv2d_wgrad_bf16(const unetrir_conv_geom* g, const unetrir_bf16* x, int ldx, const unetrir_bf16* dy, int lddy,
                              float* dw, float reg_coef, const float* w, void* ws, size_t ws_bytes, unetrir_stream_t stream) {
    return run_wgrad<BF16>(g, false, x, ldx, dy, lddy, dw, reg_coef, w, ws, ws_bytes, nullptr, (hipStream_t)stream);
}

int unetrir_conv2d_wgrad_partials_bf16(const unetrir_conv_geom* g, const unetrir_bf16* x, int ldx, const unetrir_bf16* dy, int lddy,
                                       float* dw, float reg_coef, const float* w, void* ws, size_t ws_bytes, unetrir_reduce_desc* desc,
                                       unetrir_stream_t stream) {
    if (!desc) return UNETRIR_EINVAL;
    return run_wgrad<BF16>(g, false, x, ldx, dy, lddy, dw, reg_coef, w, ws, ws_bytes, desc, (hipStream_t)stream);
}

int unetrir_conv2d_transpose_wgrad_partials_bf16(const unetrir_conv_geom* g, const unetrir_bf16* x, int ldx, const unetrir_bf16* dy,
                                                 int lddy, float* dw, float reg_coef, const float* w, void* ws, size_t ws_bytes,
                                                 unetrir_reduce_desc* desc, unetrir_stream_t stream) {
    if (!desc) return UNETRIR_EINVAL;
    return run_wgrad<BF16>(g, true, x, ldx, dy, lddy, dw, reg_coef, w, ws, ws_bytes, desc, (hipStream_t)stream);
}

int unetrir_conv2d_transpose_fwd_bf16(const unetrir_conv_geom* g, const unetrir_bf16* x, int ldx, const unetrir_bf16* wt,
                                      const float* bias, unetrir_bf16* y, int ldy, unetrir_stream_t stream) {
    if (!geom_ok(g) || !x || !wt || !y || (g->Cin & 7) || !ldh_ok(ldx, g->Cin) || ldy < g->Cout)
        return UNETRIR_EINVAL;
    const unetrir_conv_geom c = adjoint_geom(g);
    return run_conv<BF16>({&c, TFWD, x, ldx, wt, nullptr, bias, nullptr, 0, y, ldy, nullptr}, conv_family(g, UNETRIR_FAM_CONV_FWD),
                          conv_flops(&c), (hipStream_t)stream);
}

int unetrir_conv2d_transpose_dgrad_packed_bf16(const unetrir_conv_geom* g, const unetrir_bf16* dy, int lddy, const unetrir_bf16* w,
                                               const unetrir_bf16* w_packed, const unetrir_bf16* addend, int ldadd,
                                               unetrir_bf16* dx, int lddx, unetrir_stream_t stream) {
    if (!geom_ok(g) || !dy || !w || !dx || (g->Cout & 7) || !ldh_ok(lddy, g->Cout) || lddx < g->Cin)
        return UNETRIR_EINVAL;
    const unetrir_conv_geom c = adjoint_geom(g);
    return run_conv<BF16>({&c, FWD, dy, lddy, w, w_packed, nullptr, addend, ldadd, dx, lddx, nullptr},
                          conv_family(g, UNETRIR_FAM_CONV_DGRAD), conv_flops(&c), (hipStream_t)stream);
}

int unetrir_conv2d_transpose_dgrad_bf16(const unetrir_conv_geom* g, const unetrir_bf16* dy, int lddy, const unetrir_bf16* w,
                                        const unetrir_bf16* addend, int ldadd, unetrir_bf16* dx, int lddx,
                                        unetrir_stream_t stream) {
    if (!geom_ok(g) || !dy || !w || !dx || (g->Cout & 7) || !ldh_ok(lddy, g->Cout) || lddx < g->Cin)
        return UNETRIR_EINVAL;
    const unetrir_conv_geom c = adjoint_geom(g);
    return run_conv<BF16>({&c, FWD, dy, lddy, w, nullptr, nullptr, addend, ldadd, dx, lddx, nullptr},
                          conv_family(g, UNETRIR_FAM_CONV_DGRAD), conv_flops(&c), (hipStream_t)stream);
}

int unetrir_conv2d_transpose_wgrad_bf16(const unetrir_conv_geom* g, const unetrir_bf16* x, int ldx, const unetrir_bf16* dy,
                                        int lddy, float* dw, float reg_coef, const float* w, void* ws, size_t ws_bytes,
                                        unetrir_stream_t stream) {
    return run_wgrad<BF16>(g, true, x, ldx, dy, lddy, dw, reg_coef, w, ws, ws_bytes, nullptr, (hipStream_t)stream);
}

int unetrir_cast_weight_bf16(const float* w, unetrir_bf16* o, int N, int T, int C, int Cp, unetrir_stream_t stream) {
    if (!w || !o || N <= 0 || T <= 0 || C <= 0 || Cp < C) return UNETRIR_EINVAL;
    return launch_cast_weight(w, o, N, T, C, Cp, (hipStream_t)stream);
}

int unetrir_transpose_cast_weight_bf16(const float* w, unetrir_bf16* wt, int N, int T, int C, int Np, unetrir_stream_t stream) {
    if (!w || !wt || N <= 0 || T <= 0 || C <= 0 || Np < N) return UNETRIR_EINVAL;
    return launch_transpose_cast_weight(w, wt, N, T, C, Np, (hipStream_t)stream);
}

int unetrir_cast_weights_batched_bf16(const unetrir_cast_desc* desc, int n_layers, unetrir_stream_t stream) {
    if (!desc || n_layers <= 0 || n_layers > 65535) return UNETRIR_EINVAL;
    return launch_cast_weights_batched(desc, n_layers, (hipStream_t)stream);
}

size_t unetrir_dense_fwd_ws_bytes(int B, int K, int N) { return dense_fwd_ws_bytes(B, K, N); }

int unetrir_dense_fwd_f32(const float* x, int ldx, const float* w, const float* bias, float* y, int ldy, int B, int K, int N,
                          void* ws, size_t ws_bytes, unetrir_stream_t stream) {
    if (!x || !w || !y || !ws || B <= 0 || K <= 0 || N <= 0 || (K & 3) || ldx < K || (ldx & 3) || ldy < N) return UNETRIR_EINVAL;
    return launch_dense_fwd(x, ldx, w, bias, y, ldy, B, K, N, ws, ws_bytes, (hipStream_t)stream);
}

int unetrir_dense_dgrad_supported(int B, int K, int N) { return dense_dgrad_applies(B, K, N) ? 1 : 0; }

size_t unetrir_dense_dgrad_ws_bytes(int B, int K, int N) { return dense_dgrad_applies(B, K, N) ? dense_dgrad_ws_bytes(B, K, N) : 0; }

int unetrir_dense_dgrad_f32(const float* dy, int lddy, const float* w, float* dx, int lddx, int B, int K, int N, void* ws,
                            size_t ws_bytes, unetrir_stream_t stream) {
    if (!dy || !w || !dx || !ws || !dense_dgrad_applies(B, K, N) || lddy < N || lddx < K || ((uintptr_t)w & 15) || ((uintptr_t)ws & 15))
        return UNETRIR_EINVAL;
    return launch_dense_dgrad(dy, lddy, w, dx, lddx, B, K, N, ws, ws_bytes, (hipStream_t)stream);
}

int unetrir_transpose_weight_f32(const float* w, float* wt, int N, int T, int C, unetrir_stream_t stream) {
    if (!w || !wt || N <= 0 || T <= 0 || C <= 0) return UNETRIR_EINVAL;
    return launch_transpose_weight(w, wt, N, T, C, (hipStream_t)stream);
}

int unetrir_stage_h2d(int n, const void* const* src, void* const* pinned, void* const* dev, const size_t* bytes,
                      unetrir_stream_t stream) {
    if (n <= 0 || !src || !pinned || !dev || !bytes) return UNETRIR_EINVAL;
    for (int k = 0; k < n; ++k) {
        if (!src[k] || !pinned[k] || !dev[k]) return UNETRIR_EINVAL;
        std::memcpy(pinned[k], src[k], bytes[k]);
        const hipError_t e = hipMemcpyAsync(dev[k], pinned[k], bytes[k], hipMemcpyHostToDevice, (hipStream_t)stream);
        if (e != hipSuccess) return (int)e;
    }
    return 0;
}

int unetrir_eval_metrics_f32(const float* pred, const float* target, const float* phase_ref, int B, int H, int W,
                             const float* wav_pred, const float* wav_true, int T, int n50, double* out, unetrir_stream_t stream) {
    if (!pred || !target || !out || B <= 0 || H <= 0 || W <= 0) return UNETRIR_EINVAL;
    if ((wav_pred == nullptr) != (wav_true == nullptr)) return UNETRIR_EINVAL;
    if (wav_pred && (T <= 0 || n50 <= 0)) return UNETRIR_EINVAL;
    return launch_eval_metrics(pred, target, phase_ref, B, H, W, wav_pred, wav_true, T, n50, out, (hipStream_t)stream);
}

int unetrir_eval_accumulate(const double* out, const int* group, int B, int G, double* acc, unetrir_stream_t stream) {
    if (!out || !group || !acc || B <= 0 || G < 1 || G > (0x7fffffff >> 3) - 1) return UNETRIR_EINVAL;
    return launch_eval_accumulate(out, group, B, G, acc, (hipStream_t)stream);
}

int unetrir_prof_enable(int on) {
    std::lock_guard<std::mutex> lk(g_prof_mu);
    g_prof_on = on != 0;
    g_prof_mask = on == 2 ? (1u << UNETRIR_FAM_CONV_FWD) : ~0u;
    if (!g_prof_on) {
        for (auto& r : g_prof) { hipEventDestroy(r.e0); hipEventDestroy(r.e1); }
        g_prof.clear();
    }
    return 0;
}

int unetrir_prof_collect(int* counts, double* ms, double* flops) {
    std::lock_guard<std::mutex> lk(g_prof_mu);
    for (int i = 0; i < UNETRIR_PROF_FAMILIES; ++i) { counts[i] = 0; ms[i] = 0.0; flops[i] = 0.0; }
    for (auto& r : g_prof) {
        hipEventSynchronize(r.e1);
        float t = 0.f;
        hipEventElapsedTime(&t, r.e0, r.e1);
        if (r.fam >= 0 && r.fam < UNETRIR_PROF_FAMILIES) { counts[r.fam]++; ms[r.fam] += t; flops[r.fam] += r.flops; }
        if (r.tag >= 0 && r.tag < UNETRIR_PROF_FAMILIES) { counts[r.tag]++; ms[r.tag] += t; flops[r.tag] += r.flops; }
        hipEventDestroy(r.e0); hipEventDestroy(r.e1);
    }
    g_prof.clear();
    return 0;
}

}
```

### unet-rir_amd/csrc/kernels.h

```cpp
#pragma once
#include <hip/hip_runtime.h>
#include <stdint.h>
#include <stddef.h>
#include "../../include/unetrir.h"

#define UNETRIR_MAX_TAPS 36

const unetrir_config& unetrir_cfg();

#ifdef UNETRIR_ABLATIONS
extern int g_unetrir_abl;
#define UNETRIR_ABL_HOST() g_unetrir_abl
#define UNETRIR_ABL(v, bit) (((v) & (bit)) != 0)
#else
#define UNETRIR_ABL_HOST() 0
#define UNETRIR_ABL(v, bit) false
#endif

struct IgemmGeom {
    int B, PH, PW;
    int IH, IW, C, ldi;
    int OH, OW, N, ldo;
    int SI, SO, ooy, oox;
    int ntaps, wtaps;
    uint32_t tap[UNETRIR_MAX_TAPS];
};

struct IgemmArgs {
    IgemmGeom g;
    const float* in;
    const float* w;
    const float* bias;
    const float* addend;
    int ldadd;
    float* out;
    int ksplit;
    float* part;
};

struct WgradArgs {
    IgemmGeom g;
    const float* x;
    const float* dy;
    int lddy;
    float* part;
    long long chunks_per_split;
};

int launch_igemm_fwd(const IgemmArgs& a, hipStream_t s);
int launch_transpose_weight(const float* w, float* wt, int N, int T, int C, hipStream_t s);
int launch_splitk_reduce(const float* part, int nsplit, size_t n, float* out, float reg, const float* w, hipStream_t s);

#define WG_TPW 8
#define WG_F32_TPH_S1 4
#define WG_F32_TPH_S2 2
#define WG_BF16_TPH_S1 8
#define WG_BF16_TPH_S2 4
#define WG_1X1_TPH_S1 16
#define WG_1X1_TPH_S2 8
#define WG_ROW_TPH 8
#define WG_ROW_TPW 16
int wgrad_plan(const IgemmGeom& g, int* nsplit, long long* chunks_per_split);
int launch_igemm_wgrad(const WgradArgs& a, int nsplit, hipStream_t s, int bf16_operands);

struct Wgrad3Args {
    const float* x; int ldx; int IH, IW;
    const float* dy; int lddy; int OH, OW;
    int B, C, N;
    int pad_t, pad_l;
    float* part;
    int patches_per_split, npy, npx;
};
int launch_wgrad3x3(const Wgrad3Args& a, int stride, int nslabs, hipStream_t s);

struct IgemmArgsH {
    IgemmGeom g;
    const __bf16* in;
    const __bf16* w;
    const float* bias;
    const __bf16* addend;
    int ldadd;
    __bf16* out;
    float* colstat;
};
int igemm_bf16_tile_m(long long M, int N, int ncls);
int launch_igemm2_fwd_bf16(const IgemmArgsH* a, int ncls, hipStream_t s);
struct IgemmArgsH4 { IgemmArgsH a[4]; };
inline long long igemm_colstat_rows(long long M, int N, int ncls = 1) {
    const int bm = igemm_bf16_tile_m(M, N, ncls);
    return (M + (bm ? bm : 128) - 1) / (bm ? bm : 128);
}
struct Wgrad3ArgsH {
    const __bf16* x; int ldx; int IH, IW;
    const __bf16* dy; int lddy; int OH, OW;
    int B, C, N;
    int pad_t, pad_l;
    float* part;
    int patches_per_split, npy, npx;
    int xcd_remap;
};
int launch_igemm_fwd_bf16(const IgemmArgsH& a, hipStream_t s);
int launch_igemm_fwd_bf16_x4(const IgemmArgsH* a, hipStream_t s);
int launch_wgrad3x3_bf16(const Wgrad3ArgsH& a, int stride, int nslabs, hipStream_t s);
int launch_wgrad1x1_bf16(const Wgrad3ArgsH& a, int stride, int nslabs, hipStream_t s);
bool wgrad3x3g_applies(const Wgrad3ArgsH& a, bool with_ld);
int launch_wgrad3x3g_bf16(Wgrad3ArgsH a, int ns, hipStream_t s);
bool wgrad3x3r_applies(const Wgrad3ArgsH& a);
int launch_wgrad3x3r_bf16(const Wgrad3ArgsH& a, int nslabs, hipStream_t s);
bool wgrad3x3d_applies(const Wgrad3ArgsH& a, bool with_ld);
void wgrad3x3d_plan(int B, int OH, int OW, int N, int C, int* nsplit, int* per_split, int* npy, int* npx);
int launch_wgrad3x3d_bf16(Wgrad3ArgsH a, int nslabs, hipStream_t s);
int launch_cast_weight(const float* w, void* o, int N, int T, int C, int Cp, hipStream_t s);
int launch_cast_weights_batched(const unetrir_cast_desc* desc_dev, int n_layers, hipStream_t s);
int launch_transpose_cast_weight(const float* w, void* wt, int N, int T, int C, int Np, hipStream_t s);

struct Conv3Args {
    const void* in; int ldi;
    const void* w;
    const float* bias;
    const void* addend; int ldadd;
    void* out; int ldo;
    int B, H, W, C, N;
    int flip;
    const void* wpk;
    float* colstat;
};
int launch_conv3x3(const Conv3Args& a, int bf16, hipStream_t s);
long long conv3x3r_colstat_rows(const Conv3Args& a);
int launch_conv3x3r_bf16(const Conv3Args& a, hipStream_t s);
bool head_mfma_applies(int W, int C);
int launch_head_fwd_mfma(const void* x, int ldx, int B, int H, int W, int C, const float* w, const float* bias, float* y, int ldy, hipStream_t s);
int launch_head_wgrad_mfma(const void* x, int ldx, int B, int H, int W, int C, const void* dy, int lddy, float* part, int max_blocks,
                           int* nblk_out, hipStream_t s);
bool head_dgrad_mfma_applies(int W, int C);
int launch_head_dgrad_mfma(const void* dy, int lddy, int B, int H, int W, const float* w, int C, void* dx, int lddx, hipStream_t s);
bool upconv3x3g_applies(const Conv3Args& a);
bool upconv3x3q_applies(const Conv3Args& a);
int launch_upconv3x3q_bf16(const Conv3Args& a, hipStream_t s);
int launch_upconv3x3g_bf16(const Conv3Args& a, hipStream_t s);
bool conv3x3g_applies(const Conv3Args& a);
bool conv3x3g_pair_applies(const Conv3Args& a, bool any_size);
long long conv3x3g_colstat_rows(const Conv3Args& a, bool pair);
int launch_conv3x3g_bf16(const Conv3Args& a, bool pair, hipStream_t s);
bool stem3x3_applies(const Conv3Args& a);
int launch_stem3x3_bf16(const Conv3Args& a, hipStream_t s);
bool conv3x3s_applies(const Conv3Args& a);
long long conv3x3s_colstat_rows(const Conv3Args& a);
int launch_conv3x3s_bf16(const Conv3Args& a, hipStream_t s);
unsigned* sched_slot(hipStream_t s);
bool conv3x3p_applies(const Conv3Args& a);
long long conv3x3p_colstat_rows(const Conv3Args& a);
int launch_conv3x3p_bf16(const Conv3Args& a, hipStream_t s);
bool conv3x3d_applies(const Conv3Args& a);
int launch_conv3x3d_bf16(const Conv3Args& a, hipStream_t s);
bool conv3x3h_applies(const Conv3Args& a);
long long conv3x3h_colstat_rows(const Conv3Args& a);
int launch_conv3x3h_bf16(const Conv3Args& a, hipStream_t s);
int launch_dense_fwd(const float* x, int ldx, const float* w, const float* bias, float* y, int ldy, int B, int K, int N,
                     void* ws, size_t ws_bytes, hipStream_t s);
size_t dense_fwd_ws_bytes(int B, int K, int N);
int launch_splitk_rows_reduce(const float* part, int nsplit, long long M, int N, const float* bias, float* y, int ldy, hipStream_t s);
bool dense_dgrad_applies(int B, int K, int N);
size_t dense_dgrad_ws_bytes(int B, int K, int N);
int launch_dense_dgrad(const float* dy, int lddy, const float* w, float* dx, int lddx, int B, int K, int N, void* ws, size_t ws_bytes,
                       hipStream_t s);
int launch_upconv3x3(const Conv3Args& a, int bf16, hipStream_t s);

struct PwArgs {
    const __bf16* in; int ldi; int IH, IW;
    const __bf16* w;
    const float* bias;
    const __bf16* addend; int ldadd;
    __bf16* out; int ldo; int OH, OW;
    int B, PH, PW, SI, SO, fill;
    int C, N;
    float* colstat;
};
bool pw1x1_applies(const PwArgs& a);
long long pw1x1_colstat_rows(const PwArgs& a);
int launch_pw1x1_bf16(const PwArgs& a, hipStream_t s);

__device__ __forceinline__ unsigned long long mix64(unsigned long long z) {
    z = (z ^ (z >> 30)) * 0xBF58476D1CE4E5B9ULL;
    z = (z ^ (z >> 27)) * 0x94D049BB133111EBULL;
    return z ^ (z >> 31);
}

int launch_eval_metrics(const float* pred, const float* target, const float* phase_ref, int B, int H, int W, const float* wav_pred,
                        const float* wav_true, int T, int n50, double* out, hipStream_t s);
int launch_eval_accumulate(const double* out, const int* group, int B, int G, double* acc, hipStream_t s);
```

### unet-rir_amd/engine.py

```python
import math

import torch

from . import _lib, ops
from .engine_base import BN_EPS, BN_MOMENTUM, L2_COEF, EngineBase, ParamSpec
from .ops import Act

VOCAB, EMB_DIM, VEC_CH = 2000, 256, 16


def same_out(n, s):
    return -(-n // s)


def pick_concurrent_streams(device, n, candidates=12):
    dev = torch.device(device)
    main = torch.cuda.current_stream(dev)
    a = torch.empty(64 << 20, dtype=torch.uint8, device=dev)
    b = torch.empty_like(a)
    tiny = torch.zeros(64, device=dev)

    def runs_beside(busy, cand):
        torch.cuda.synchronize(dev)
        with torch.cuda.stream(busy):
            for _ in range(24):
                b.copy_(a, non_blocking=True)
            end_busy = torch.cuda.Event()
            end_busy.record(busy)
        with torch.cuda.stream(cand):
            tiny.add_(1.0)
            end_cand = torch.cuda.Event()
            end_cand.record(cand)
        end_cand.synchronize()
        ok = not end_busy.query()
        torch.cuda.synchronize(dev)
        return ok

    chosen, pool = [], [torch.cuda.Stream(device=dev) for _ in range(candidates)]
    for c in pool:
        if len(chosen) == n:
            break
        if all(runs_beside(o, c) and runs_beside(c, o) for o in [main] + chosen):
            chosen.append(c)
    for c in pool:
        if len(chosen) == n:
            break
        if c not in chosen:
            chosen.append(c)
    return chosen


class UNetEngine(EngineBase):
    mask_on_side_stream = True

    def __init__(self, H, W, B, F0=32, k=3, depth=4, batchnorm=True, inf_vector_shape=(2, 16), s0=1, s=2,
                 device="cuda:0", n_replicas=1, dtype="f32", overlap_wgrad=False, runtime=None, share=None):
        super().__init__(device, n_replicas, dtype, runtime, share)
        if s0 != 1 or s != 2:
            raise NotImplementedError("HIP path implements resize_factor_0=[1,1], res_factor=[2,2] (the reference defaults)")
        self._cst_rows, self._cst_buf, self._cst_gen = {}, None, ops.config_generation()
        if F0 % self.PAD:
            raise ValueError(f"number_filters_0 must be a multiple of {self.PAD} for dtype {dtype}")
        if k < 1 or k > 6:
            raise ValueError("kernels must be in 1..6")
        self.H, self.W, self.B, self.F0, self.k, self.depth = H, W, B, F0, k, depth
        self.batchnorm = batchnorm
        self.inf_vector_shape = tuple(inf_vector_shape)
        self.L = depth + 1
        self.ch = [F0 * 2 ** l for l in range(self.L)]
        self.hw = [(H, W)]
        for _ in range(depth):
            h, w = self.hw[-1]
            self.hw.append((same_out(h, 2), same_out(w, 2)))
        for l in range(depth):
            if self.hw[l][0] != 2 * self.hw[l + 1][0] or self.hw[l][1] != 2 * self.hw[l + 1][1]:
                raise ValueError("spatial size must halve exactly at every level that feeds a skip concat")
        self.h5, self.w5 = self.hw[-1]
        self.n_idx = int(math.prod(self.inf_vector_shape))
        self.vec_in = self.n_idx * EMB_DIM
        self.vec_dim = self.h5 * self.w5 * VEC_CH
        if share is not None and (share.H, share.W, share.F0, share.k, share.depth, share.batchnorm, share.dtype, share.inf_vector_shape) != \
                (H, W, F0, k, depth, batchnorm, dtype, self.inf_vector_shape):
            raise ValueError("share= needs an engine of the same configuration (only the batch size may differ)")
        self._build_params(share)
        self._alloc()
        self.ws = ops.Workspace(self.device)
        self._reserve_workspace()
        self._init_side_stream(share, overlap_wgrad, 96 << 20, park_max_bytes=16 << 20)
        self.head_direct = ops.head6x6_supported(self.ch[0])
        if self.head_direct:
            self.ws.reserve(512 * 2 * 36 * self.ch[0] * 4)
            self.ws_w.reserve(512 * 2 * 36 * self.ch[0] * 4)
        elif self.dtype == "bf16":
            raise ValueError("the bf16 path needs number_filters_0 % 8 == 0 (direct head kernels)")

    def _build_params(self, share=None):
        k, ch, L = self.k, self.ch, self.L
        specs = []

        def add(name, shape, kind, keras_shape):
            specs.append(ParamSpec(name, shape, kind, keras_shape))

        def bn(prefix, c):
            if self.batchnorm:
                add(prefix + ".gamma", (c,), "gamma", (c,))
                add(prefix + ".beta", (c,), "beta", (c,))

        PAD = self.PAD
        add("head.kernel", (PAD, 6, 6, ch[0]), "conv_padout", (6, 6, ch[0], 2))
        add("head.bias", (PAD,), "bias_pad", (2,))
        for l in range(1, self.depth + 1):
            c = ch[l - 1]
            add(f"dec{l}.cb1b.kernel", (c, 3, 3, c), "conv", (3, 3, c, c))
            add(f"dec{l}.cb1b.bias", (c,), "bias", (c,))
            bn(f"dec{l}.cb1b", c)
            add(f"dec{l}.cb1a.kernel", (c, k, k, 2 * c), "conv", (k, k, 2 * c, c))
            add(f"dec{l}.cb1a.bias", (c,), "bias", (c,))
            bn(f"dec{l}.cb1a", c)
            add(f"dec{l}.up.kernel", (ch[l], k, k, c), "convT", (k, k, c, ch[l]))
            add(f"dec{l}.up.bias", (c,), "bias", (c,))
        add("vec.conv.kernel", (ch[-1], 1, 1, VEC_CH), "conv", (1, 1, VEC_CH, ch[-1]))
        add("vec.conv.bias", (ch[-1],), "bias", (ch[-1],))
        add("vec.dense.kernel", (self.vec_dim, self.vec_in), "dense", (self.vec_in, self.vec_dim))
        add("vec.dense.bias", (self.vec_dim,), "bias", (self.vec_dim,))
        add("vec.embedding", (VOCAB, EMB_DIM), "embedding", (VOCAB, EMB_DIM))
        for l in range(L, 0, -1):
            c = ch[l - 1]
            cin = ch[l - 2] if l > 1 else 2
            add(f"enc{l}.cb1.kernel", (c, 3, 3, c), "conv", (3, 3, c, c))
            add(f"enc{l}.cb1.bias", (c,), "bias", (c,))
            bn(f"enc{l}.cb1", c)
            if l > 1:
                add(f"enc{l}.down.kernel", (c, k, k, cin), "conv", (k, k, cin, c))
            else:
                add(f"enc{l}.down.kernel", (c, k, k, PAD), "conv_padin", (k, k, 2, c))
            add(f"enc{l}.down.bias", (c,), "bias", (c,))
        self.dense_direct = ops.dense_dgrad_supported(self.B, self.vec_in, self.vec_dim) if share is None else share.dense_direct
        if share is not None and self.dense_direct and not ops.dense_dgrad_supported(self.B, self.vec_in, self.vec_dim):
            raise ValueError("this batch size needs a transposed Dense kernel copy the shared parameter set does not hold")
        t_names = [s_.name for s_ in specs if s_.kind in ("conv", "convT", "conv_padout") or (s_.kind == "dense" and not self.dense_direct)]
        trunk = [s_ for s_ in specs if s_.kind in ("conv", "convT", "conv_padin", "conv_padout") and not s_.name.startswith("vec.")]
        trunk = trunk if self.dtype == "bf16" else []
        strided = lambda n: n.endswith(".up.kernel") or (n.endswith(".down.kernel") and not n.startswith("enc1."))
        self._layout_params(specs, t_names, [s_.name for s_ in trunk], [s_.name for s_ in trunk if strided(s_.name) and s_.shape[1] == 3], share)
        dev = self.device
        self.bn_names = [n[:-len(".gamma")] for n in self.specs if n.endswith(".gamma")]
        self.moving = share.moving if share is not None else {}
        for b in self.bn_names if share is None else ():
            c = self.specs[b + ".gamma"].numel
            self.moving[b + ".moving_mean"] = torch.zeros(c, dtype=torch.float32, device=dev)
            self.moving[b + ".moving_variance"] = torch.ones(c, dtype=torch.float32, device=dev)
        self.l2_names = [f"enc{l}.down.kernel" for l in range(1, L + 1)] + [f"dec{l}.up.kernel" for l in range(1, self.depth + 1)]

    def _alloc(self):
        B, dev, ch, hw, D = self.B, self.device, self.ch, self.hw, self.depth
        A = lambda h, w, c: ops.new_act(B, h, w, c, dev, dtype=self.adt)
        F = lambda h, w, c: ops.new_act(B, h, w, c, dev)
        PAD = self.PAD
        self.x4, self.down, self.y, self.a = A(self.H, self.W, PAD), {}, {}, {}
        self.cat, self.g_cat = {}, {}
        self.g_down, self.g_y = {}, {}
        for l in range(1, self.L + 1):
            h, w = hw[l - 1]
            c = ch[l - 1]
            self.down[l], self.y[l] = A(h, w, c), A(h, w, c)
            self.g_down[l], self.g_y[l] = A(h, w, c), A(h, w, c)
            if l <= D:
                self.cat[l], self.g_cat[l] = A(h, w, 2 * c), A(h, w, 2 * c)
                self.a[l] = self.cat[l].slice(0, c)
            else:
                self.a[l] = A(h, w, c)
        cL = ch[-1]
        self.emb_out = torch.empty((B * self.n_idx, EMB_DIM), dtype=torch.float32, device=dev)
        self.g_emb_out = torch.empty_like(self.emb_out)
        self.flat = Act(self.emb_out.view(B, 1, 1, self.vec_in))
        self.g_flat = Act(self.g_emb_out.view(B, 1, 1, self.vec_in))
        self.v = ops.new_act(B, 1, 1, self.vec_dim, dev)
        self.vd = ops.new_act(B, 1, 1, self.vec_dim, dev)
        self.g_v = ops.new_act(B, 1, 1, self.vec_dim, dev)
        self.g_vd = ops.new_act(B, 1, 1, self.vec_dim, dev)
        self.vd_sp = Act(self.vd.base.view(B, self.h5, self.w5, VEC_CH))
        self.g_vd_sp = Act(self.g_vd.base.view(B, self.h5, self.w5, VEC_CH))
        self.z, self.g_z = A(self.h5, self.w5, cL), A(self.h5, self.w5, cL)
        self.ya, self.aa, self.yb, self.ab = {}, {}, {}, {}
        self.g_ya, self.g_aa, self.g_yb, self.g_ab = {}, {}, {}, {}
        for l in range(1, D + 1):
            h, w = hw[l - 1]
            c = ch[l - 1]
            for d_ in (self.ya, self.aa, self.yb, self.ab, self.g_ya, self.g_aa, self.g_yb, self.g_ab):
                d_[l] = A(h, w, c)
        self.logits, self.g_logits = F(self.H, self.W, 4), A(self.H, self.W, PAD)
        if self.dtype == "bf16":
            self.v1x1, self.g_z32 = F(self.h5, self.w5, cL), F(self.h5, self.w5, cL)
        self.pred = torch.empty((B, 2, self.H, self.W), dtype=torch.float32, device=dev)
        self.loss_out = torch.zeros(4, dtype=torch.float32, device=dev)
        self.reg_out = torch.zeros(1, dtype=torch.float32, device=dev)
        self.loss_tot = torch.zeros(1, dtype=torch.float32, device=dev)
        self.bn_affine = {b: torch.empty(2 * self.specs[b + ".gamma"].numel, dtype=torch.float32, device=dev) for b in self.bn_names}
        self.bn_saved = {b: torch.empty(2 * self.specs[b + ".gamma"].numel, dtype=torch.float32, device=dev) for b in self.bn_names}
        self._mask = None
        self.emb_idx = torch.zeros(B * self.n_idx, dtype=torch.int32, device=dev)
        G, k = ops.geom, self.k
        self.geo = {}
        for l in range(1, self.L + 1):
            h, w = hw[l - 1]
            c = ch[l - 1]
            if l == 1:
                self.geo["enc1.down"] = G(B, h, w, PAD, c, k, 1)
            else:
                hi, wi = hw[l - 2]
                self.geo[f"enc{l}.down"] = G(B, hi, wi, ch[l - 2], c, k, 2)
            self.geo[f"enc{l}.cb1"] = G(B, h, w, c, c, 3, 1)
        self.geo["vec.dense"] = G(B, 1, 1, self.vec_in, self.vec_dim, 1, 1)
        self.geo["vec.conv"] = G(B, self.h5, self.w5, VEC_CH, cL, 1, 1)
        for l in range(1, D + 1):
            h, w = hw[l - 1]
            c = ch[l - 1]
            hl, wl = hw[l]
            self.geo[f"dec{l}.up"] = G(B, hl, wl, ch[l], c, k, 2)
            self.geo[f"dec{l}.cb1a"] = G(B, h, w, 2 * c, c, k, 1)
            self.geo[f"dec{l}.cb1b"] = G(B, h, w, c, c, 3, 1)
        self.geo["head"] = G(B, self.H, self.W, ch[0], PAD, 6, 1)

    def _reserve_workspace(self):
        need = 1 << 16
        for n, g in self.geo.items():
            if n.endswith(".up"):
                need = max(need, ops.conv2d_transpose_wgrad_ws_bytes(g))
            else:
                need = max(need, ops.conv2d_wgrad_ws_bytes(g))
        P0 = self.B * self.H * self.W
        need = max(need, ops.bn_ws_bytes(P0, max(self.ch[0], 4)), ops.bn_ws_bytes(self.B * self.h5 * self.w5, self.ch[-1]),
                   ops.bn_ws_bytes(self.B, self.vec_dim))
        for l in range(1, self.L + 1):
            h, w = self.hw[l - 1]
            need = max(need, ops.bn_ws_bytes(self.B * h * w, 2 * self.ch[l - 1]))
        if self.dense_direct:
            need = max(need, _lib.lib().unetrir_dense_dgrad_ws_bytes(self.B, self.vec_in, self.vec_dim))
        self.ws.reserve(need)

    def wf(self, name):
        return self.ph[name] if self.dtype == "bf16" else self.p[name]

    def wb(self, name):
        return self.pth[name] if self.dtype == "bf16" else self.pt[name]

    def _bn_relu_fwd(self, name, y: Act, out: Act):
        if self.batchnorm:
            if self.training:
                ops.bn_stats(y, self.p[name + ".gamma"], self.p[name + ".beta"], self.bn_affine[name], self.bn_saved[name],
                             self.ws, self.moving[name + ".moving_mean"], self.moving[name + ".moving_variance"],
                             BN_EPS, BN_MOMENTUM)
            else:
                ops.bn_inference_affine(self.p[name + ".gamma"], self.p[name + ".beta"], self.moving[name + ".moving_mean"],
                                        self.moving[name + ".moving_variance"], BN_EPS, self.bn_affine[name])
            ops.bn_apply(y, self.bn_affine[name], out, relu=True)
        else:
            ops.relu_fwd(y, out)

    def _colstat(self, name, dgrad, x: Act, n_out):
        key = (name, dgrad)
        if self._cst_gen != ops.config_generation():
            self._cst_rows, self._cst_gen = {}, ops.config_generation()
        if key not in self._cst_rows:
            self._cst_rows[key] = ops.conv2d_colstat_rows(self.geo[name], dgrad, x) if self.dtype == "bf16" else 0
        rows = self._cst_rows[key]
        if rows == 0:
            return 0, None
        need = rows * n_out * 2
        if self._cst_buf is None or self._cst_buf.numel() < need:
            self._cst_buf = torch.empty(need, device=self.device, dtype=torch.float32)
        return rows, self._cst_buf

    def _conv_bn_relu_fwd(self, name, x: Act, y: Act, out: Act):
        p = self.p
        rows, buf = self._colstat(name, 0, x, y.C) if (self.batchnorm and self.training) else (0, None)
        if rows == 0:
            ops.conv2d_fwd(self.geo[name], x, self.wf(name + ".kernel"), p[name + ".bias"], y)
            self._bn_relu_fwd(name, y, out)
            return
        ops.conv2d_fwd_colstat(self.geo[name], x, self.wf(name + ".kernel"), p[name + ".bias"], y, buf)
        ops.bn_colstat_act_add(buf, rows, y, p[name + ".gamma"], p[name + ".beta"], self.bn_affine[name], self.bn_saved[name], out, 1, None,
                               self.moving[name + ".moving_mean"], self.moving[name + ".moving_variance"], BN_EPS, BN_MOMENTUM)

    def _dgrad_colsum(self, name, dy: Act, dx: Act, bias_grad, c0, c_n):
        rows, buf = self._colstat(name, 1, dy, dx.C)
        if rows == 0:
            ops.conv2d_dgrad(self.geo[name], dy, self.wb(name + ".kernel"), dx)
            return False
        ops.conv2d_dgrad_colstat(self.geo[name], dy, self.wb(name + ".kernel"), dx, buf)
        ops.colsum_colstat(buf, rows, dx.C, c0, c_n, bias_grad)
        return True

    def _bn_relu_bwd(self, name, da: Act, y: Act, dy: Act):
        if self.batchnorm:
            ops.bn_bwd(da, y, self.p[name + ".gamma"], self.bn_affine[name], self.bn_saved[name], dy,
                       self.g[name + ".gamma"], self.g[name + ".beta"], self.ws, relu=True)
        else:
            ops.relu_bwd(da, y, dy)

    def forward(self, spec, emb, dropout_mask=None, target=None, global_batch=None, alpha=0.9):
        B, D, p = self.B, self.depth, self.p
        if tuple(spec.shape) != (B, 2, self.H, self.W) or spec.dtype != torch.float32 or not spec.is_contiguous():
            raise ValueError(f"spec must be a contiguous float32 [{B},2,{self.H},{self.W}] tensor, got {tuple(spec.shape)} {spec.dtype}")
        if tuple(emb.shape) != (B,) + self.inf_vector_shape:
            raise ValueError(f"emb must be [{B},{self.inf_vector_shape}]")
        if spec.device != self.device:
            raise ValueError("inputs must live on the engine's device")
        if self.t_dirty or self.training:
            self.refresh_transposed()
        if emb.dtype not in (torch.int32, torch.int64):
            emb = emb.to(torch.int64)
        if emb.device != self.device:
            emb = emb.to(self.device)
        ops.index_to_i32(emb.contiguous(), self.emb_idx)
        self._mask = dropout_mask

        def vec_branch(ws_):
            ops.embedding_fwd(self.emb_idx, p["vec.embedding"], self.emb_out)
            ops.dense_fwd(self.flat, p["vec.dense.kernel"], p["vec.dense.bias"], self.v, ws_)
            if dropout_mask is not None:
                ops.mul(self.v.base, dropout_mask, self.vd.base)
                vsp_ = self.vd_sp
            else:
                vsp_ = Act(self.v.base.view(B, self.h5, self.w5, VEC_CH))
            if self.dtype != "f32":
                ops.conv2d_fwd(self.geo["vec.conv"], vsp_, p["vec.conv.kernel"], p["vec.conv.bias"], self.v1x1)
            return vsp_

        vsp = None
        if self.wg_stream is not None:
            with self._wg() as ws_:
                vsp = vec_branch(ws_)
        ops.nchw_to_nhwc_pad(spec, self.x4)
        prev = self.x4
        for l in range(1, self.L + 1):
            ops.conv2d_fwd(self.geo[f"enc{l}.down"], prev, self.wf(f"enc{l}.down.kernel"), p[f"enc{l}.down.bias"], self.down[l],
                           w_packed=self.ppk.get(f"enc{l}.down.kernel"))
            self._conv_bn_relu_fwd(f"enc{l}.cb1", self.down[l], self.y[l], self.a[l])
            prev = self.a[l]
        if self.wg_stream is None:
            vsp = vec_branch(self.ws)
        else:
            self._join_wg()
        if self.dtype == "f32":
            ops.conv2d_fwd(self.geo["vec.conv"], vsp, p["vec.conv.kernel"], p["vec.conv.bias"], self.z, addend=self.a[self.L])
        else:
            ops.add_f32_to_bf16(self.a[self.L], self.v1x1, self.z)
        cur = self.z
        for l in range(D, 0, -1):
            c = self.ch[l - 1]
            ops.conv2d_transpose_fwd(self.geo[f"dec{l}.up"], cur, self.wb(f"dec{l}.up.kernel"), p[f"dec{l}.up.bias"],
                                     self.cat[l].slice(c, c))
            self._conv_bn_relu_fwd(f"dec{l}.cb1a", self.cat[l], self.ya[l], self.aa[l])
            self._conv_bn_relu_fwd(f"dec{l}.cb1b", self.aa[l], self.yb[l], self.ab[l])
            cur = self.ab[l]
        if self.head_direct:
            ops.head6x6_fwd(cur, p["head.kernel"], p["head.bias"], self.logits)
        else:
            ops.conv2d_fwd(self.geo["head"], cur, p["head.kernel"], p["head.bias"], self.logits)
        if target is not None:
            gb = B if global_batch is None else global_batch
            inv_norm = 1.0 / (2.0 * self.H * self.W * gb)
            ops.sigmoid_loss(self.logits, target, alpha, inv_norm, self.pred, self.g_logits, self.loss_out, self.ws, **self._loss_extras(spec))
        else:
            self._last_spec = spec
            ops.sigmoid_nchw(self.logits, self.pred)
        return self.pred

    def loss_from_logits(self, target, global_batch=None, alpha=0.9):
        gb = self.B if global_batch is None else global_batch
        if tuple(target.shape) != (self.B, 2, self.H, self.W) or target.dtype != torch.float32 or not target.is_contiguous():
            raise ValueError(f"target must be a contiguous float32 [{self.B},2,{self.H},{self.W}] tensor")
        ops.sigmoid_loss(self.logits, target, alpha, 1.0 / (2.0 * self.H * self.W * gb), self.pred, self.g_logits, self.loss_out, self.ws,
                         **self._loss_extras())

    def backward(self, dpred=None, on_ready=None, include_reg=True):
        D, p, pt, g, ws = self.depth, self.p, self.pt, self.g, self.ws
        reg = 2.0 * L2_COEF / self.n_replicas if include_reg else 0.0
        if dpred is not None:
            ops.sigmoid_bwd(self.pred, dpred, self.g_logits)

        def ready(name):
            if on_ready is not None:
                self._ready(on_ready, self.specs[name].end)

        gl = self.g_logits
        if self.head_direct:
            with self._wg() as ws_:
                ops.head6x6_wgrad(self.ab[1] if D >= 1 else self.a[1], gl, g["head.kernel"], ws_)
        else:
            with self._wg() as ws_:
                ops.conv2d_wgrad(self.geo["head"], self.ab[1] if D >= 1 else self.a[1], gl, g["head.kernel"], ws_)
        with self._wg() as ws_:
            ops.colsum(gl, g["head.bias"], ws_)
        top = self.ab[1] if D >= 1 else self.a[1]
        g_cur = self.g_ab[1] if D >= 1 else self.g_z
        if self.head_direct and self.dtype == "bf16" and ops.head6x6_dgrad_supported(self.W, self.ch[0]):
            ops.head6x6_dgrad(gl, self.p["head.kernel"], g_cur)
        else:
            ops.conv2d_dgrad(self.geo["head"], gl, self.wb("head.kernel"), g_cur)
        ready("head.bias")
        for l in range(1, D + 1):
            c = self.ch[l - 1]
            self._bn_relu_bwd(f"dec{l}.cb1b", self.g_ab[l], self.yb[l], self.g_yb[l])
            with self._wg() as ws_:
                ops.conv2d_wgrad(self.geo[f"dec{l}.cb1b"], self.aa[l], self.g_yb[l], g[f"dec{l}.cb1b.kernel"], ws_, defer=self._rb if self.park_reduces else None)
            if not self.batchnorm:
                with self._wg() as ws_:
                    ops.colsum(self.g_yb[l], g[f"dec{l}.cb1b.bias"], ws_)
            ops.conv2d_dgrad(self.geo[f"dec{l}.cb1b"], self.g_yb[l], self.wb(f"dec{l}.cb1b.kernel"), self.g_aa[l])
            self._bn_relu_bwd(f"dec{l}.cb1a", self.g_aa[l], self.ya[l], self.g_ya[l])
            with self._wg() as ws_:
                ops.conv2d_wgrad(self.geo[f"dec{l}.cb1a"], self.cat[l], self.g_ya[l], g[f"dec{l}.cb1a.kernel"], ws_, defer=self._rb if self.park_reduces else None)
            if not self.batchnorm:
                with self._wg() as ws_:
                    ops.colsum(self.g_ya[l], g[f"dec{l}.cb1a.bias"], ws_)
            up_bias_done = self._dgrad_colsum(f"dec{l}.cb1a", self.g_ya[l], self.g_cat[l], g[f"dec{l}.up.bias"], c, c)
            g_up = self.g_cat[l].slice(c, c)
            x_in = self.ab[l + 1] if l < D else self.z
            g_in = self.g_ab[l + 1] if l < D else self.g_z
            with self._wg() as ws_:
                ops.conv2d_transpose_wgrad(self.geo[f"dec{l}.up"], x_in, g_up, g[f"dec{l}.up.kernel"], ws_, reg=reg,
                                           w=p[f"dec{l}.up.kernel"], defer=self._rb if self.park_reduces else None)
            if not up_bias_done:
                with self._wg() as ws_:
                    ops.colsum(g_up, g[f"dec{l}.up.bias"], ws_)
            ops.conv2d_transpose_dgrad(self.geo[f"dec{l}.up"], g_up, self.wf(f"dec{l}.up.kernel"), g_in,
                                       w_packed=self.ppk.get(f"dec{l}.up.kernel"))
            ready(f"dec{l}.up.bias")
        B = self.B
        has_do = self._mask is not None
        vsp = self.vd_sp if has_do else Act(self.v.base.view(B, self.h5, self.w5, VEC_CH))
        with self._wg() as ws_:
            gz = self.g_z
            if self.dtype == "bf16":
                ops.cast_bf16_to_f32(self.g_z, self.g_z32)
                gz = self.g_z32
            ops.conv2d_wgrad(self.geo["vec.conv"], vsp, gz, g["vec.conv.kernel"], ws_)
            ops.colsum(gz, g["vec.conv.bias"], ws_)
            ops.conv2d_dgrad(self.geo["vec.conv"], gz, pt["vec.conv.kernel"], self.g_vd_sp)
            if has_do:
                ops.mul(self.g_vd.base, self._mask, self.g_v.base)
                gv = self.g_v
            else:
                gv = self.g_vd
            ops.conv2d_wgrad(self.geo["vec.dense"], self.flat, gv, g["vec.dense.kernel"], ws_)
            ops.colsum(gv, g["vec.dense.bias"], ws_)
            if self.dense_direct:
                ops.dense_dgrad(gv, p["vec.dense.kernel"], self.g_flat, ws_)
            else:
                ops.dense_fwd(gv, pt["vec.dense.kernel"], None, self.g_flat, ws_)
            ops.embedding_bwd(self.emb_idx, self.g_emb_out, g["vec.embedding"])
        ready("vec.embedding")
        g_a = self.g_z
        for l in range(self.L, 0, -1):
            self._bn_relu_bwd(f"enc{l}.cb1", g_a, self.y[l], self.g_y[l])
            with self._wg() as ws_:
                ops.conv2d_wgrad(self.geo[f"enc{l}.cb1"], self.down[l], self.g_y[l], g[f"enc{l}.cb1.kernel"], ws_, defer=self._rb if self.park_reduces else None)
            if not self.batchnorm:
                with self._wg() as ws_:
                    ops.colsum(self.g_y[l], g[f"enc{l}.cb1.bias"], ws_)
            down_bias_done = self._dgrad_colsum(f"enc{l}.cb1", self.g_y[l], self.g_down[l], g[f"enc{l}.down.bias"], 0, self.g_down[l].C)
            x_in = self.a[l - 1] if l > 1 else self.x4
            with self._wg() as ws_:
                ops.conv2d_wgrad(self.geo[f"enc{l}.down"], x_in, self.g_down[l], g[f"enc{l}.down.kernel"], ws_, reg=reg,
                                 w=p[f"enc{l}.down.kernel"], defer=self._rb if self.park_reduces else None)
            if not down_bias_done:
                with self._wg() as ws_:
                    ops.colsum(self.g_down[l], g[f"enc{l}.down.bias"], ws_)
            ready(f"enc{l}.down.bias")
            if l > 1:
                skip = self.g_cat[l - 1].slice(0, self.ch[l - 2])
                ops.conv2d_dgrad(self.geo[f"enc{l}.down"], self.g_down[l], self.wb(f"enc{l}.down.kernel"), skip, addend=skip)
                g_a = skip
        self._end_backward()

    def make_dropout_mask(self, generator=None):
        return self.dropout_mask(self.vec_dim, generator)
```

### unet-rir_amd/ops.py

```python
import ctypes as C

import torch

from . import _lib
from ._lib import ConvGeom, check


class Act:
    __slots__ = ("base", "B", "H", "W", "C", "ld", "c0", "ptr", "sfx")

    def __init__(self, base: torch.Tensor, c0: int = 0, C_: int = None):
        if base.dim() != 4 or not base.is_contiguous() or base.dtype not in (torch.float32, torch.bfloat16):
            raise ValueError("Act needs a contiguous fp32 or bf16 [B,H,W,ld] tensor")
        self.base = base
        self.B, self.H, self.W, self.ld = base.shape
        self.c0 = c0
        self.C = self.ld - c0 if C_ is None else C_
        self.sfx = "f32" if base.dtype == torch.float32 else "bf16"
        al = 16 // base.element_size()
        if self.c0 % al or self.ld % al or self.c0 + self.C > self.ld:
            raise ValueError(f"channel offset and pixel stride must be multiples of {al}")
        self.ptr = base.data_ptr() + base.element_size() * c0

    @property
    def P(self):
        return self.B * self.H * self.W

    def slice(self, c0, C_):
        return Act(self.base, self.c0 + c0, C_)

    def dense(self):
        return self.base[..., self.c0:self.c0 + self.C].contiguous()


def new_act(B, H, W, C_, device, ld=None, dtype=torch.float32):
    return Act(torch.empty((B, H, W, C_ if ld is None else ld), dtype=dtype, device=device), 0, C_)


def _fn(name, sfx):
    return getattr(_lib.lib(), f"unetrir_{name}_{sfx}")


def _stream():
    return C.c_void_p(torch.cuda.current_stream().cuda_stream)


def _p(t):
    if t is None:
        return None
    if isinstance(t, Act):
        return C.c_void_p(t.ptr)
    return C.c_void_p(t.data_ptr())


def geom(B, H, W, Cin, Cout, k, stride):
    return ConvGeom(B, H, W, Cin, Cout, k, stride)


class Workspace:

    def __init__(self, device, nbytes=0):
        self.device = device
        self.buf = torch.empty(max(nbytes, 16), dtype=torch.uint8, device=device)

    def reserve(self, nbytes):
        if nbytes > self.buf.numel():
            self.buf = torch.empty(int(nbytes), dtype=torch.uint8, device=self.device)

    @property
    def ptr(self):
        return C.c_void_p(self.buf.data_ptr())

    @property
    def nbytes(self):
        return self.buf.numel()



def conv3x3s2_packed_elems(N, C_):
    return int(_lib.lib().unetrir_conv3x3s2_packed_elems(int(N), int(C_)))


def conv2d_fwd(g, x: Act, w, bias, y: Act, addend: Act = None, w_packed=None):
    if w_packed is not None:
        check(_lib.lib().unetrir_conv2d_fwd_packed_bf16(C.byref(g), _p(x), x.ld, _p(w), _p(w_packed), _p(bias), _p(addend),
                                                        addend.ld if addend is not None else 0, _p(y), y.ld, _stream()),
              "conv2d_fwd_packed")
        return
    check(_fn("conv2d_fwd", x.sfx)(C.byref(g), _p(x), x.ld, _p(w), _p(bias), _p(addend),
                                            addend.ld if addend is not None else 0, _p(y), y.ld, _stream()),
          "conv2d_fwd")


def conv2d_dgrad(g, dy: Act, wt, dx: Act, addend: Act = None):
    check(_fn("conv2d_dgrad", dy.sfx)(C.byref(g), _p(dy), dy.ld, _p(wt), _p(addend),
                                              addend.ld if addend is not None else 0, _p(dx), dx.ld, _stream()),
          "conv2d_dgrad")


def conv2d_colstat_rows(g, dgrad, x: Act):
    if x.sfx != "bf16":
        return 0
    return int(_lib.lib().unetrir_conv2d_colstat_rows_bf16(C.byref(g), int(bool(dgrad)), x.ld))


K3_NAMES = ("tap-table", "conv3x3r", "conv3x3g", "conv3x3g pair", "conv3x3h", "conv3x3s", "conv3x3p", "stem", "patch")


def conv3x3_kernel(g, dgrad, x: Act):
    return K3_NAMES[int(_lib.lib().unetrir_conv3x3_kernel_id_bf16(C.byref(g), int(bool(dgrad)), x.ld))]


def conv2d_fwd_colstat(g, x: Act, w, bias, y: Act, colstat, addend: Act = None):
    check(_lib.lib().unetrir_conv2d_fwd_colstat_bf16(C.byref(g), _p(x), x.ld, _p(w), _p(bias), _p(addend),
                                                     addend.ld if addend is not None else 0, _p(y), y.ld, _p(colstat), _stream()),
          "conv2d_fwd_colstat")


def conv2d_dgrad_colstat(g, dy: Act, wt, dx: Act, colstat, addend: Act = None):
    check(_lib.lib().unetrir_conv2d_dgrad_colstat_bf16(C.byref(g), _p(dy), dy.ld, _p(wt), _p(addend),
                                                       addend.ld if addend is not None else 0, _p(dx), dx.ld, _p(colstat), _stream()),
          "conv2d_dgrad_colstat")


def conv2d_transpose_colstat_rows(g, x: Act):
    if x.sfx != "bf16":
        return 0
    return int(_lib.lib().unetrir_conv2d_transpose_colstat_rows_bf16(C.byref(g), x.ld))


def conv2d_transpose_fwd_colstat(g, x: Act, wt, bias, y: Act, colstat):
    check(_lib.lib().unetrir_conv2d_transpose_fwd_colstat_bf16(C.byref(g), _p(x), x.ld, _p(wt), _p(bias), _p(y), y.ld, _p(colstat),
                                                               _stream()), "conv2d_transpose_fwd_colstat")


def bn_stats_colstat(colstat, rows, P, C_, gamma, beta, affine, saved, moving_mean=None, moving_var=None, eps=1e-3, momentum=0.99):
    check(_lib.lib().unetrir_bn_stats_colstat(_p(colstat), rows, P, C_, _p(gamma), _p(beta), eps, momentum, _p(moving_mean),
                                              _p(moving_var), _p(affine), _p(saved), _stream()), "bn_stats_colstat")


def bn_colstat_act_add(colstat, rows, x: Act, gamma, beta, affine, saved, y: Act, act=2, addend: Act = None, moving_mean=None,
                       moving_var=None, eps=1e-3, momentum=0.99):
    check(_fn("bn_colstat_act_add", x.sfx)(_p(colstat), rows, _p(x), x.ld, x.P, x.C, _p(gamma), _p(beta), eps, momentum, _p(moving_mean),
                                            _p(moving_var), _p(affine), _p(saved), int(act), _p(addend),
                                            addend.ld if addend is not None else 0, _p(y), y.ld, _stream()), "bn_colstat_act_add")


def colsum_colstat(colstat, rows, ldc, c0, C_, out):
    check(_lib.lib().unetrir_colsum_colstat(_p(colstat), rows, ldc, c0, C_, _p(out), _stream()), "colsum_colstat")


def conv2d_wgrad_ws_bytes(g):
    return _lib.lib().unetrir_conv2d_wgrad_ws_bytes(C.byref(g))


def wgrad_defer_supported(storage):
    return storage == "bf16"


class ReduceBatch:

    def __init__(self, device, arena_bytes, capacity=64, park_max_bytes=None):
        self.arena = Workspace(device, int(arena_bytes))
        self.descs = (_lib.ReduceDesc * capacity)()
        self.n, self.used, self.capacity = 0, 0, capacity
        self.park_max_bytes = park_max_bytes

    def __len__(self):
        return self.n

    def take(self, nbytes):
        nbytes = -(-int(nbytes) // 256) * 256
        if self.n == 0 and nbytes > self.arena.nbytes:
            self.arena.reserve(4 * nbytes)
        if self.n == self.capacity or self.used + nbytes > self.arena.nbytes:
            return None
        ptr = self.arena.buf.data_ptr() + self.used
        self.used += nbytes
        return C.c_void_p(ptr), nbytes

    def flush(self):
        if self.n:
            check(_lib.lib().unetrir_splitk_reduce_batched(self.descs, self.n, _stream()), "splitk_reduce_batched")
        self.n, self.used = 0, 0


def _wgrad(name, g, x: Act, dy: Act, dw, ws: Workspace, reg, w, defer, need):
    if defer is not None and x.sfx == "bf16" and (defer.park_max_bytes is None or need <= defer.park_max_bytes):
        got = defer.take(need)
        if got is None and len(defer):
            defer.flush()
            got = defer.take(need)
        if got is not None:
            ptr, nbytes = got
            check(getattr(_lib.lib(), f"unetrir_{name}_partials_bf16")(C.byref(g), _p(x), x.ld, _p(dy), dy.ld, _p(dw), float(reg), _p(w), ptr, nbytes,
                                                                       C.byref(defer.descs[defer.n]), _stream()), name + "_partials")
            if defer.descs[defer.n].nsplit:
                defer.n += 1
            else:
                defer.used -= nbytes
            return
    ws.reserve(need)
    check(_fn(name, x.sfx)(C.byref(g), _p(x), x.ld, _p(dy), dy.ld, _p(dw), float(reg), _p(w), ws.ptr, ws.nbytes, _stream()), name)


def conv2d_wgrad(g, x: Act, dy: Act, dw, ws: Workspace, reg=0.0, w=None, defer: ReduceBatch = None):
    _wgrad("conv2d_wgrad", g, x, dy, dw, ws, reg, w, defer, conv2d_wgrad_ws_bytes(g))


def conv2d_transpose_fwd(g, x: Act, wt, bias, y: Act):
    check(_fn("conv2d_transpose_fwd", x.sfx)(C.byref(g), _p(x), x.ld, _p(wt), _p(bias), _p(y), y.ld,
                                                      _stream()), "conv2d_transpose_fwd")


def conv2d_transpose_dgrad(g, dy: Act, w, dx: Act, addend: Act = None, w_packed=None):
    if w_packed is not None:
        check(_lib.lib().unetrir_conv2d_transpose_dgrad_packed_bf16(C.byref(g), _p(dy), dy.ld, _p(w), _p(w_packed), _p(addend),
                                                                    addend.ld if addend is not None else 0, _p(dx), dx.ld,
                                                                    _stream()), "conv2d_transpose_dgrad_packed")
        return
    check(_fn("conv2d_transpose_dgrad", dy.sfx)(C.byref(g), _p(dy), dy.ld, _p(w), _p(addend),
                                                        addend.ld if addend is not None else 0, _p(dx), dx.ld,
                                                        _stream()), "conv2d_transpose_dgrad")


def conv2d_transpose_wgrad_ws_bytes(g):
    return _lib.lib().unetrir_conv2d_transpose_wgrad_ws_bytes(C.byref(g))


def conv2d_transpose_wgrad(g, x: Act, dy: Act, dw, ws: Workspace, reg=0.0, w=None, defer: ReduceBatch = None):
    _wgrad("conv2d_transpose_wgrad", g, x, dy, dw, ws, reg, w, defer, conv2d_transpose_wgrad_ws_bytes(g))


def dense_fwd(x: Act, w, bias, y: Act, ws: Workspace):
    B, K, N = x.B, x.C, y.C
    ws.reserve(_lib.lib().unetrir_dense_fwd_ws_bytes(B, K, N))
    check(_lib.lib().unetrir_dense_fwd_f32(_p(x), x.ld, _p(w), _p(bias), _p(y), y.ld, B, K, N, ws.ptr, ws.nbytes, _stream()),
          "dense_fwd")


def dense_dgrad_supported(B, K, N):
    return bool(_lib.lib().unetrir_dense_dgrad_supported(B, K, N))


def dense_dgrad(dy: Act, w, dx: Act, ws: Workspace):
    B, N, K = dy.P, dy.C, dx.C
    ws.reserve(_lib.lib().unetrir_dense_dgrad_ws_bytes(B, K, N))
    check(_lib.lib().unetrir_dense_dgrad_f32(_p(dy), dy.ld, _p(w), _p(dx), dx.ld, B, K, N, ws.ptr, ws.nbytes, _stream()),
          "dense_dgrad")


def transpose_weight(w, wt, N, T, C_):
    check(_lib.lib().unetrir_transpose_weight_f32(_p(w), _p(wt), N, T, C_, _stream()), "transpose_weight")


def cast_weight_bf16(w, o, N, T, C_, Cp):
    check(_lib.lib().unetrir_cast_weight_bf16(_p(w), _p(o), N, T, C_, Cp, _stream()), "cast_weight_bf16")


def transpose_cast_weight_bf16(w, wt, N, T, C_, Np):
    check(_lib.lib().unetrir_transpose_cast_weight_bf16(_p(w), _p(wt), N, T, C_, Np, _stream()),
          "transpose_cast_weight_bf16")


def make_cast_table(entries, device):
    arr = (_lib.CastDesc * len(entries))()
    for i, ent in enumerate(entries):
        w, same, tr, N, T, C_, Cp, Np = ent[:8]
        pk = ent[8] if len(ent) > 8 else None
        arr[i] = _lib.CastDesc(w.data_ptr(), same.data_ptr() if same is not None else None,
                               tr.data_ptr() if tr is not None else None, N, T, C_, Cp, Np, 0,
                               pk.data_ptr() if pk is not None else None)
    raw = torch.frombuffer(bytearray(bytes(arr)), dtype=torch.uint8)
    return raw.to(device), len(entries)


def cast_weights_batched(table):
    dev, n = table
    check(_lib.lib().unetrir_cast_weights_batched_bf16(dev.data_ptr(), n, _stream()), "cast_weights_batched")


def stage_h2d(src_ptrs, pinned, dev, stream):
    n = len(src_ptrs)
    vp, sz = C.c_void_p * n, C.c_size_t * n
    nbytes = [p.numel() * p.element_size() for p in pinned]
    check(_lib.lib().unetrir_stage_h2d(n, vp(*src_ptrs), vp(*[p.data_ptr() for p in pinned]), vp(*[d.data_ptr() for d in dev]),
                                       sz(*nbytes), C.c_void_p(stream.cuda_stream)), "stage_h2d")


def add_f32_to_bf16(a: Act, b: Act, y: Act):
    check(_lib.lib().unetrir_add_f32_to_bf16(_p(a), _p(b), _p(y), a.base.numel(), _stream()), "add_f32_to_bf16")


def cast_f32_to_bf16(a: Act, y: Act):
    check(_lib.lib().unetrir_cast_f32_to_bf16(_p(a), _p(y), a.base.numel(), _stream()), "cast_f32_to_bf16")


def cast_bf16_to_f32(a: Act, y: Act):
    check(_lib.lib().unetrir_cast_bf16_to_f32(_p(a), _p(y), a.base.numel(), _stream()), "cast_bf16_to_f32")



def bn_ws_bytes(P, C_):
    return _lib.lib().unetrir_bn_ws_bytes(P, C_)


def bn_stats(x: Act, gamma, beta, affine, saved, ws: Workspace, moving_mean=None, moving_var=None,
             eps=1e-3, momentum=0.99):
    ws.reserve(bn_ws_bytes(x.P, x.C))
    check(_fn("bn_stats", x.sfx)(_p(x), x.ld, x.P, x.C, _p(gamma), _p(beta), eps, momentum,
                                          _p(moving_mean), _p(moving_var), _p(affine), _p(saved), ws.ptr, ws.nbytes,
                                          _stream()), "bn_stats")


def bn_apply(x: Act, affine, y: Act, relu=True):
    check(_fn("bn_apply", x.sfx)(_p(x), x.ld, x.P, x.C, _p(affine), int(relu), _p(y), y.ld, _stream()),
          "bn_apply")


def bn_bwd(da: Act, x: Act, gamma, affine, saved, dx: Act, dgamma, dbeta, ws: Workspace, relu=True):
    ws.reserve(bn_ws_bytes(x.P, x.C))
    if x.sfx == "f32":
        check(_lib.lib().unetrir_bn_bwd_f32(_p(da), da.ld, _p(x), x.ld, x.P, x.C, _p(gamma), _p(affine), _p(saved),
                                            int(relu), _p(dx), dx.ld, _p(dgamma), _p(dbeta), ws.ptr, ws.nbytes,
                                            _stream()), "bn_bwd")
    else:
        check(_lib.lib().unetrir_bn_bwd_bf16(_p(da), da.ld, _p(x), x.ld, x.P, x.C, _p(affine), _p(saved), int(relu),
                                             _p(dx), dx.ld, _p(dgamma), _p(dbeta), ws.ptr, ws.nbytes, _stream()),
              "bn_bwd")


def bn_inference_affine(gamma, beta, moving_mean, moving_var, eps, affine):
    check(_lib.lib().unetrir_bn_inference_affine_f32(_p(gamma), _p(beta), _p(moving_mean), _p(moving_var), eps, moving_mean.numel(),
                                                     _p(affine), _stream()), "bn_inference_affine")


def bn_act_add(x: Act, affine, y: Act, act=2, addend: Act = None):
    check(_fn("bn_act_add", x.sfx)(_p(x), x.ld, x.P, x.C, _p(affine), int(act), _p(addend),
                                   addend.ld if addend is not None else 0, _p(y), y.ld, _stream()), "bn_act_add")


def bn_bwd_junction(da: Act, x: Act, out: Act, affine, saved, dx: Act, dgamma, dbeta, ws: Workspace, act=2, gskip: Act = None,
                    gskip_add: Act = None):
    ws.reserve(bn_ws_bytes(x.P, x.C))
    check(_fn("bn_bwd_junction", x.sfx)(_p(da), da.ld, _p(x), x.ld, _p(out), out.ld, x.P, x.C, _p(affine), _p(saved), int(act), _p(dx), dx.ld,
                                        _p(gskip), gskip.ld if gskip is not None else 0, _p(gskip_add),
                                        gskip_add.ld if gskip_add is not None else 0, _p(dgamma), _p(dbeta), ws.ptr, ws.nbytes, _stream()),
          "bn_bwd_junction")


def act_bwd(da: Act, out: Act, g: Act, act=2):
    check(_fn("act_bwd", out.sfx)(_p(da), da.ld, _p(out), out.ld, out.P, out.C, int(act), _p(g), g.ld, _stream()), "act_bwd")


def add(a, b, y):
    check(_lib.lib().unetrir_add_f32(_p(a), _p(b), _p(y), a.numel(), _stream()), "add")


def colsum(x: Act, out, ws: Workspace):
    ws.reserve(bn_ws_bytes(x.P, x.C))
    check(_fn("colsum", x.sfx)(_p(x), x.ld, x.P, x.C, _p(out), ws.ptr, ws.nbytes, _stream()), "colsum")


def relu_fwd(x: Act, y: Act):
    if x.sfx == "f32":
        check(_lib.lib().unetrir_relu_fwd_f32(_p(x), x.ld, x.P, x.C, _p(y), y.ld, _stream()), "relu_fwd")
    else:
        check(_lib.lib().unetrir_bn_apply_bf16(_p(x), x.ld, x.P, x.C, None, 1, _p(y), y.ld, _stream()), "relu_fwd")


def relu_bwd(da: Act, x: Act, dx: Act):
    check(_fn("relu_bwd", x.sfx)(_p(da), da.ld, _p(x), x.ld, x.P, x.C, _p(dx), dx.ld, _stream()),
          "relu_bwd")



def nchw_to_nhwc_pad(x, y: Act):
    B, C_, H, W = x.shape
    check(_fn("nchw_to_nhwc_pad", y.sfx)(_p(x), B, C_, H, W, _p(y), y.ld, _stream()), "nchw_to_nhwc_pad")


def head6x6_supported(C_):
    return bool(_lib.lib().unetrir_head6x6_supported(C_))


def head6x6_fwd(x: Act, w, bias, y: Act):
    check(_fn("head6x6_fwd", x.sfx)(_p(x), x.ld, x.B, x.H, x.W, x.C, _p(w), _p(bias), _p(y), y.ld, _stream()),
          "head6x6_fwd")


def head6x6_wgrad(x: Act, dy: Act, dw, ws: Workspace):
    ws.reserve(_lib.lib().unetrir_head6x6_wgrad_ws_bytes(x.C))
    check(_fn("head6x6_wgrad", x.sfx)(_p(x), x.ld, x.B, x.H, x.W, x.C, _p(dy), dy.ld, _p(dw), ws.ptr, ws.nbytes,
                                               _stream()), "head6x6_wgrad")


def head6x6_dgrad_supported(W_, C_):
    return bool(_lib.lib().unetrir_head6x6_dgrad_supported(W_, C_))


def head6x6_dgrad(dy: Act, w, dx: Act):
    if dy.sfx != "bf16" or dx.sfx != "bf16":
        raise ValueError("head6x6_dgrad is a bf16-storage kernel")
    check(_lib.lib().unetrir_head6x6_dgrad_bf16(_p(dy), dy.ld, dy.B, dy.H, dy.W, _p(w), dx.C, _p(dx), dx.ld, _stream()),
          "head6x6_dgrad")



PAD_MODES = {"reflect": 0, "constant": 1}


def stft_frames(T, hop_length):
    return _lib.lib().unetrir_stft_frames(int(T), int(hop_length))


def stft_features(wav, out, n_fft=256, win_length=128, hop_length=64, pad_mode="reflect", remove_mean=True, normalize=True):
    if wav.dtype != torch.float32 or out.dtype != torch.float32 or not wav.is_contiguous() or not out.is_contiguous():
        raise ValueError("stft_features takes contiguous fp32 tensors")
    if wav.dim() != 2 or out.dim() != 4 or out.shape[0] != wav.shape[0] or out.shape[1] != 2:
        raise ValueError("stft_features: wav [B, T], out [B, 2, H, W]")
    if pad_mode not in PAD_MODES:
        raise ValueError(f"pad_mode must be one of {sorted(PAD_MODES)}")
    B, T = wav.shape
    check(_lib.lib().unetrir_stft_features_f32(_p(wav), B, T, n_fft, win_length, hop_length, PAD_MODES[pad_mode], int(remove_mean),
                                               int(normalize), _p(out), out.shape[2], out.shape[3], _stream()), "stft_features")


def istft_features(feat, wav, n_bins, n_frames, n_fft=256, win_length=128, hop_length=64, denormalize=True):
    if feat.dtype != torch.float32 or wav.dtype != torch.float32 or not feat.is_contiguous() or not wav.is_contiguous():
        raise ValueError("istft_features takes contiguous fp32 tensors")
    if feat.dim() != 4 or feat.shape[1] != 2 or wav.dim() != 2 or wav.shape[0] != feat.shape[0] or \
            wav.shape[1] != hop_length * (n_frames - 1):
        raise ValueError("istft_features: feat [B, 2, H, W], wav [B, hop_length * (n_frames - 1)]")
    B, _, H, W = feat.shape
    check(_lib.lib().unetrir_istft_features_f32(_p(feat), B, H, W, n_bins, n_frames, n_fft, win_length, hop_length,
                                                int(denormalize), _p(wav), _stream()), "istft_features")


def griffinlim_ws_bytes(B, n_bins, n_frames, n_fft):
    return int(_lib.lib().unetrir_griffinlim_ws_bytes(int(B), int(n_bins), int(n_frames), int(n_fft)))


def griffinlim(feat, wav, n_bins, n_frames, n_fft, win_length, hop_length, ws: Workspace, pad_mode="reflect", denormalize=True,
               n_iter=32, momentum=0.99, init_phase=None, seed=0, draw=0):
    if feat.dtype != torch.float32 or wav.dtype != torch.float32 or not feat.is_contiguous() or not wav.is_contiguous():
        raise ValueError("griffinlim takes contiguous fp32 tensors")
    if feat.dim() != 4 or feat.shape[1] != 2 or wav.dim() != 2 or wav.shape[0] != feat.shape[0] or \
            wav.shape[1] != hop_length * (n_frames - 1):
        raise ValueError("griffinlim: feat [B, 2, H, W], wav [B, hop_length * (n_frames - 1)]")
    if pad_mode not in PAD_MODES:
        raise ValueError(f"pad_mode must be one of {sorted(PAD_MODES)}")
    B, _, H, W = feat.shape
    if init_phase is not None:
        _f32c(init_phase, (B, n_bins, n_frames), "init_phase", feat)
    need = griffinlim_ws_bytes(B, n_bins, n_frames, n_fft)
    if need:
        ws.reserve(need)
    check(_lib.lib().unetrir_griffinlim_f32(_p(feat), B, H, W, n_bins, n_frames, n_fft, win_length, hop_length, PAD_MODES[pad_mode],
                                            int(denormalize), int(n_iter), float(momentum), _p(init_phase), int(seed), int(draw),
                                            _p(wav), ws.ptr, ws.nbytes, _stream()), "griffinlim")


def uniform(out, seed, step):
    check(_lib.lib().unetrir_uniform_f32(_p(out), out.numel(), int(seed), int(step), _stream()), "uniform")


def _f32c(t, shape, what, like):
    if t.dtype != torch.float32 or not t.is_contiguous() or tuple(t.shape) != tuple(shape) or t.device != like.device:
        raise ValueError(f"{what} must be a contiguous float32 tensor of shape {tuple(shape)} on {like.device}")


def eval_metrics(pred, target, out, wav_pred=None, wav_true=None, phase_ref=None, n50=2400):
    if not pred.is_cuda or pred.dim() != 4 or pred.shape[1] != 2:
        raise ValueError("eval_metrics: pred must be a CUDA tensor [B, 2, H, W]")
    B, _, H, W = pred.shape
    _f32c(pred, pred.shape, "pred", pred)
    _f32c(target, pred.shape, "target", pred)
    if phase_ref is not None:
        _f32c(phase_ref, pred.shape, "phase_ref", pred)
    if (wav_pred is None) != (wav_true is None):
        raise ValueError("eval_metrics: wav_pred and wav_true come as a pair")
    T = 0
    if wav_pred is not None:
        if wav_pred.dim() != 2 or wav_pred.shape[0] != B:
            raise ValueError("eval_metrics: waveforms must be [B, T]")
        T = wav_pred.shape[1]
        _f32c(wav_pred, (B, T), "wav_pred", pred)
        _f32c(wav_true, (B, T), "wav_true", pred)
    if out.dtype != torch.float64 or not out.is_contiguous() or tuple(out.shape) != (B, 7) or out.device != pred.device:
        raise ValueError(f"eval_metrics: out must be a contiguous float64 [{B}, 7] tensor on {pred.device}")
    check(_lib.lib().unetrir_eval_metrics_f32(_p(pred), _p(target), _p(phase_ref), B, H, W, _p(wav_pred), _p(wav_true), T, int(n50),
                                              _p(out), _stream()), "eval_metrics")


def eval_accumulate(out, group, acc):
    if not out.is_cuda or out.dtype != torch.float64 or out.dim() != 2 or out.shape[1] != 7 or not out.is_contiguous():
        raise ValueError("eval_accumulate: out must be a contiguous float64 CUDA tensor [B, 7]")
    B = out.shape[0]
    if group.dtype != torch.int32 or tuple(group.shape) != (B,) or not group.is_contiguous() or group.device != out.device:
        raise ValueError(f"eval_accumulate: group must be a contiguous int32 [{B}] tensor on {out.device}")
    if acc.dtype != torch.float64 or acc.dim() != 2 or acc.shape[0] < 2 or acc.shape[1] != 8 or not acc.is_contiguous() or \
            acc.device != out.device:
        raise ValueError(f"eval_accumulate: acc must be a contiguous float64 [G + 1, 8] tensor on {out.device}")
    check(_lib.lib().unetrir_eval_accumulate(_p(out), _p(group), B, acc.shape[0] - 1, _p(acc), _stream()), "eval_accumulate")



def _bank(t, dtype, what, like=None, rows=None):
    if not isinstance(t, torch.Tensor) or not t.is_cuda or t.dtype != dtype or not t.is_contiguous():
        raise ValueError(f"gather_batch: {what} must be a contiguous {dtype} CUDA tensor")
    if like is not None and t.device != like.device:
        raise ValueError(f"gather_batch: {what} lives on {t.device}, the bank on {like.device}")
    if rows is not None and (t.dim() < 1 or t.shape[0] != rows):
        raise ValueError(f"gather_batch: {what} must have {rows} rows")


def gather_batch(bank, emb_bank, idx_in, idx_out, spec_in, spec_out, emb, wav_bank=None, room_bank=None, wav_true=None, room=None):
    _bank(bank, torch.float32, "bank")
    if bank.dim() < 2:
        raise ValueError("gather_batch: bank must be [N, ...]")
    N, B = bank.shape[0], idx_in.numel()
    _bank(emb_bank, torch.int32, "emb_bank", bank, N)
    if emb_bank.dim() != 2:
        raise ValueError("gather_batch: emb_bank must be [N, L]")
    _bank(idx_in, torch.int32, "idx_in", bank)
    _bank(idx_out, torch.int32, "idx_out", bank, B)
    if idx_in.dim() != 1:
        raise ValueError("gather_batch: idx_in / idx_out must be [B]")
    for t, what in ((spec_in, "spec_in"), (spec_out, "spec_out")):
        _bank(t, torch.float32, what, bank)
        if tuple(t.shape) != (B,) + tuple(bank.shape[1:]):
            raise ValueError(f"gather_batch: {what} must be {(B,) + tuple(bank.shape[1:])}")
    _bank(emb, torch.int32, "emb", bank)
    if tuple(emb.shape) != (B, 2, emb_bank.shape[1]):
        raise ValueError(f"gather_batch: emb must be {(B, 2, emb_bank.shape[1])}")
    T = 0
    if (wav_true is None) != (wav_bank is None):
        raise ValueError("gather_batch: wav_true and wav_bank come as a pair")
    if wav_bank is not None:
        _bank(wav_bank, torch.float32, "wav_bank", bank, N)
        _bank(wav_true, torch.float32, "wav_true", bank, B)
        if wav_bank.dim() != 2 or tuple(wav_true.shape) != (B, wav_bank.shape[1]):
            raise ValueError("gather_batch: wav_bank [N, T], wav_true [B, T]")
        T = wav_bank.shape[1]
    if room is not None:
        if room_bank is None:
            raise ValueError("gather_batch: room needs room_bank")
        _bank(room_bank, torch.int32, "room_bank", bank, N)
        _bank(room, torch.int32, "room", bank, B)
        if room_bank.dim() != 1 or room.dim() != 1:
            raise ValueError("gather_batch: room_bank [N], room [B]")
    else:
        room_bank = None
    check(_lib.lib().unetrir_gather_batch_f32(_p(bank), N, bank[0].numel(), _p(emb_bank), emb_bank.shape[1], _p(wav_bank), T,
                                              _p(room_bank), _p(idx_in), _p(idx_out), B, _p(spec_in), _p(spec_out), _p(emb),
                                              _p(wav_true), _p(room), _stream()), "gather_batch")


def sigmoid_loss(logits: Act, target, alpha, inv_norm, pred, dlogits: Act, loss_out, ws: Workspace, phase_ref=None, phase_weight=None):
    B, _, H, W = target.shape
    ws.reserve(_lib.lib().unetrir_loss_ws_bytes(B * H * W))
    if phase_ref is None and phase_weight is None:
        check(_fn("sigmoid_loss", dlogits.sfx)(_p(logits), logits.ld, _p(target), B, H, W, alpha, inv_norm, _p(pred),
                                               _p(dlogits), _p(loss_out), ws.ptr, ws.nbytes, _stream()), "sigmoid_loss")
        return
    if phase_ref is not None and (tuple(phase_ref.shape) != tuple(target.shape) or phase_ref.dtype != torch.float32 or
                                  not phase_ref.is_contiguous() or phase_ref.device != target.device):
        raise ValueError("phase_ref must be a contiguous float32 tensor of the target's shape on the same device")
    if phase_weight is not None and (tuple(phase_weight.shape) != (W,) or phase_weight.dtype != torch.float32 or
                                     phase_weight.device != target.device):
        raise ValueError(f"phase_weight must be float32 [{W}] on the target's device")
    check(_fn("sigmoid_loss_ex", dlogits.sfx)(_p(logits), logits.ld, _p(target), _p(phase_ref), _p(phase_weight), B, H, W, alpha,
                                              inv_norm, _p(pred), _p(dlogits), _p(loss_out), ws.ptr, ws.nbytes, _stream()),
          "sigmoid_loss_ex")


def sigmoid_nchw(logits: Act, pred):
    B, _, H, W = pred.shape
    check(_lib.lib().unetrir_sigmoid_nchw_f32(_p(logits), logits.ld, B, H, W, _p(pred), _stream()), "sigmoid_nchw")


def sigmoid_bwd(pred, dpred, dlogits: Act):
    B, _, H, W = pred.shape
    check(_fn("sigmoid_bwd", dlogits.sfx)(_p(pred), _p(dpred), B, H, W, _p(dlogits), _stream()), "sigmoid_bwd")



def embedding_fwd(idx, table, out):
    check(_lib.lib().unetrir_embedding_fwd_f32(_p(idx), idx.numel(), _p(table), table.shape[0], table.shape[1],
                                               _p(out), _stream()), "embedding_fwd")


def embedding_bwd(idx, dout, dtable):
    check(_lib.lib().unetrir_embedding_bwd_f32(_p(idx), idx.numel(), _p(dout), dtable.shape[0], dtable.shape[1],
                                               _p(dtable), _stream()), "embedding_bwd")


def dropout_mask(mask, p, seed, step):
    check(_lib.lib().unetrir_dropout_mask_f32(_p(mask), mask.numel(), float(p), int(seed), int(step), _stream()), "dropout_mask")


def index_to_i32(idx, out):
    if idx.dtype not in (torch.int32, torch.int64) or not idx.is_contiguous() or idx.numel() != out.numel():
        raise ValueError("indices must be a contiguous int32 or int64 tensor of the expected size")
    if idx.device != out.device:
        raise ValueError(f"indices live on {idx.device}, the engine on {out.device}")
    check(_lib.lib().unetrir_index_to_i32(_p(idx), idx.element_size(), idx.numel(), _p(out), _stream()), "index_to_i32")


def mul(x, m, y):
    check(_lib.lib().unetrir_mul_f32(_p(x), _p(m), _p(y), x.numel(), _stream()), "mul")


def sumsq(x, coef, out, accumulate, ws: Workspace):
    ws.reserve(512 * 8)
    check(_lib.lib().unetrir_sumsq_f32(_p(x), x.numel(), float(coef), _p(out), int(accumulate), ws.ptr, ws.nbytes,
                                       _stream()), "sumsq")


def adam(theta, g, m, v, lr_t, beta1=0.9, beta2=0.999, eps=1e-7, grad_scale=1.0):
    check(_lib.lib().unetrir_adam_f32(_p(theta), _p(g), _p(m), _p(v), theta.numel(), float(lr_t), beta1, beta2, eps,
                                      float(grad_scale), _stream()), "adam")


def sgd(theta, g, lr, grad_scale=1.0):
    check(_lib.lib().unetrir_sgd_f32(_p(theta), _p(g), theta.numel(), float(lr), float(grad_scale), _stream()), "sgd")


def nadam(theta, g, m, v, lr, beta1, beta2, eps, c_g, c_m, c_v, grad_scale=1.0):
    check(_lib.lib().unetrir_nadam_f32(_p(theta), _p(g), _p(m), _p(v), theta.numel(), float(lr), beta1, beta2, eps, float(c_g), float(c_m),
                                       float(c_v), float(grad_scale), _stream()), "nadam")


def adam_dev(theta, g, m, v, hyper):
    check(_lib.lib().unetrir_adam_dev_f32(_p(theta), _p(g), _p(m), _p(v), theta.numel(), _p(hyper), _stream()), "adam_dev")


def dropout_mask_dev(mask, p, seed, state, offset):
    check(_lib.lib().unetrir_dropout_mask_dev_f32(_p(mask), mask.numel(), float(p), int(seed), C.c_void_p(state.data_ptr() + 16),
                                                  int(offset), _stream()), "dropout_mask_dev")


def step_advance(state, cfg, hyper, n_draws, advance_t=True):
    check(_lib.lib().unetrir_step_advance(_p(state), _p(cfg), _p(hyper), int(n_draws), int(bool(advance_t)), _stream()), "step_advance")



def normal(out, seed, step):
    check(_lib.lib().unetrir_normal_f32(_p(out), out.numel(), int(seed), int(step), _stream()), "normal")


def normal_dev(out, seed, state, offset):
    check(_lib.lib().unetrir_normal_dev_f32(_p(out), out.numel(), int(seed), C.c_void_p(state.data_ptr() + 16), int(offset), _stream()),
          "normal_dev")


def vae_sample_kl_fwd(mu: Act, log_var: Act, eps, inv_global_batch, z: Act, kl_out):
    if eps.dtype != torch.float32 or not eps.is_contiguous() or eps.numel() != mu.B * mu.C:
        raise ValueError(f"eps must be a contiguous float32 [{mu.B},{mu.C}] tensor")
    check(_lib.lib().unetrir_vae_sample_kl_fwd_f32(_p(mu), mu.ld, _p(log_var), log_var.ld, _p(eps), mu.P, mu.C, float(inv_global_batch),
                                                   _p(z), z.ld, _p(kl_out), _stream()), "vae_sample_kl_fwd")


def vae_sample_kl_bwd(mu: Act, log_var: Act, eps, dz: Act, inv_global_batch, dmu: Act, dlv: Act):
    check(_lib.lib().unetrir_vae_sample_kl_bwd_f32(_p(mu), mu.ld, _p(log_var), log_var.ld, _p(eps), _p(dz), dz.ld, mu.P, mu.C,
                                                   float(inv_global_batch), _p(dmu), dmu.ld, _p(dlv), dlv.ld, _stream()),
          "vae_sample_kl_bwd")


def vae_loss_add(kl_out, loss_out):
    check(_lib.lib().unetrir_vae_loss_add_f32(_p(kl_out), _p(loss_out), _stream()), "vae_loss_add")


def reset_tile_tickets():
    check(_lib.lib().unetrir_reset_tile_tickets(), "reset_tile_tickets")



def get_config():
    c = _lib.Config()
    check(_lib.lib().unetrir_get_config(C.byref(c)), "get_config")
    return {n: getattr(c, n) for n, _ in _lib.Config._fields_}


_CONFIG_GEN = [0]


def config_generation():
    return _CONFIG_GEN[0]


def set_config(**switches):
    old = get_config()
    new = dict(old)
    for k, v in switches.items():
        if k not in new:
            raise KeyError(f"unknown switch {k}")
        new[k] = int(v)
    c = _lib.Config(*[new[n] for n, _ in _lib.Config._fields_])
    check(_lib.lib().unetrir_set_config(C.byref(c)), "set_config")
    if new != old:
        _CONFIG_GEN[0] += 1
    return old



def prof_enable(on):
    _lib.lib().unetrir_prof_enable(int(on))


def prof_collect():
    n = _lib.PROF_FAMILIES
    counts = (C.c_int * n)()
    ms = (C.c_double * n)()
    fl = (C.c_double * n)()
    _lib.lib().unetrir_prof_collect(counts, ms, fl)
    return list(counts), list(ms), list(fl)
```

Measured before the change: 2584 spectrograms/s.

## Fuse bottleneck vector 1x1 conv with residual add and add small-Cin wgrad kernel

Result: no change. 2593 spectrograms/s (median of 6 runs) (+0.4%).

```diff
diff --git a/include/unetrir.h b/include/unetrir.h
--- a/include/unetrir.h
+++ b/include/unetrir.h
@@ -248,6 +248,12 @@
                             unetrir_stream_t stream);
 int unetrir_cast_bf16_to_f32(const unetrir_bf16* a, float* y, long long n, unetrir_stream_t stream);
 int unetrir_cast_f32_to_bf16(const float* a, unetrir_bf16* y, long long n, unetrir_stream_t stream);
+int unetrir_vec1x1_supported(int K, int N);
+int unetrir_vec1x1_fwd_bf16(const float* v, int ldv, const float* w, const float* bias, const unetrir_bf16* a, int lda, unetrir_bf16* z,
+                            int ldz, long long P, int K, int N, unetrir_stream_t stream);
+size_t unetrir_vec1x1_bwd_ws_bytes(long long P, int K, int N);
+int unetrir_vec1x1_bwd_bf16(const unetrir_bf16* g, int ldg, const float* v, int ldv, const float* wt, long long P, int K, int N, float* dw,
+                            float* db, float* dv, int lddv, void* ws, size_t ws_bytes, unetrir_stream_t stream);
 int unetrir_bn_act_add_bf16(const unetrir_bf16* x, int ldx, long long P, int C, const float* affine, int act,
                             const unetrir_bf16* addend, int ldadd, unetrir_bf16* y, int ldy, unetrir_stream_t stream);
 int unetrir_act_bwd_bf16(const unetrir_bf16* da, int ldda, const unetrir_bf16* out, int ldo, long long P, int C, int act,
diff --git a/unet-rir_amd/_lib.py b/unet-rir_amd/_lib.py
--- a/unet-rir_amd/_lib.py
+++ b/unet-rir_amd/_lib.py
@@ -164,6 +164,12 @@
     "unetrir_add_f32_to_bf16": (C.c_int, [c_f32p, c_f32p, c_f32p, C.c_longlong, c_stream]),
     "unetrir_cast_bf16_to_f32": (C.c_int, [c_f32p, c_f32p, C.c_longlong, c_stream]),
     "unetrir_cast_f32_to_bf16": (C.c_int, [c_f32p, c_f32p, C.c_longlong, c_stream]),
+    "unetrir_vec1x1_supported": (C.c_int, [C.c_int, C.c_int]),
+    "unetrir_vec1x1_fwd_bf16": (C.c_int, [c_f32p, C.c_int, c_f32p, c_f32p, c_f32p, C.c_int, c_f32p, C.c_int, C.c_longlong, C.c_int, C.c_int,
+                                          c_stream]),
+    "unetrir_vec1x1_bwd_ws_bytes": (C.c_size_t, [C.c_longlong, C.c_int, C.c_int]),
+    "unetrir_vec1x1_bwd_bf16": (C.c_int, [c_f32p, C.c_int, c_f32p, C.c_int, c_f32p, C.c_longlong, C.c_int, C.c_int, c_f32p, c_f32p, c_f32p,
+                                          C.c_int, C.c_void_p, C.c_size_t, c_stream]),
     "unetrir_bn_act_add_bf16": (C.c_int, [c_f32p, C.c_int, C.c_longlong, C.c_int, c_f32p, C.c_int, c_f32p, C.c_int, c_f32p,
                                           C.c_int, c_stream]),
     "unetrir_act_bwd_bf16": (C.c_int, [c_f32p, C.c_int, c_f32p, C.c_int, C.c_longlong, C.c_int, C.c_int, c_f32p, C.c_int,
diff --git a/unet-rir_amd/build.py b/unet-rir_amd/build.py
--- a/unet-rir_amd/build.py
+++ b/unet-rir_amd/build.py
@@ -7,7 +7,7 @@
 CSRC = os.path.join(HERE, "csrc")
 OBJ = os.path.join(HERE, "build")
 LIB = os.path.join(HERE, "libunetrir.so")
-SOURCES = ["igemm.hip", "api.hip", "elementwise.hip", "head.hip", "head_mfma.hip", "wgrad3x3.hip", "wgrad3x3r.hip", "wgrad3x3g.hip", "wgrad3x3d.hip", "igemm_bf16.hip", "conv3x3.hip", "conv3x3r.hip", "conv3x3g.hip", "conv3x3h.hip", "conv3x3s.hip", "conv3x3d.hip", "conv3x3p.hip", "upconv3x3.hip", "upconv3x3g.hip", "upconv3x3q.hip", "features.hip", "dense.hip", "stem3x3.hip", "pw1x1.hip", "igemm2_bf16.hip", "evalmetrics.hip", "vae.hip", "dataset.hip", "griffinlim.hip"]
+SOURCES = ["igemm.hip", "api.hip", "elementwise.hip", "head.hip", "head_mfma.hip", "wgrad3x3.hip", "wgrad3x3r.hip", "wgrad3x3g.hip", "wgrad3x3d.hip", "wgrad3x3c.hip", "igemm_bf16.hip", "conv3x3.hip", "conv3x3r.hip", "conv3x3g.hip", "conv3x3h.hip", "conv3x3s.hip", "conv3x3d.hip", "conv3x3p.hip", "upconv3x3.hip", "upconv3x3g.hip", "upconv3x3q.hip", "features.hip", "dense.hip", "stem3x3.hip", "pw1x1.hip", "vec1x1.hip", "igemm2_bf16.hip", "evalmetrics.hip", "vae.hip", "dataset.hip", "griffinlim.hip"]
 FLAGS = ["-O3", "--offload-arch=gfx950", "-std=c++17", "-fPIC", "-Wno-unused-value"]
 
 
diff --git a/unet-rir_amd/csrc/api.hip b/unet-rir_amd/csrc/api.hip
--- a/unet-rir_amd/csrc/api.hip
+++ b/unet-rir_amd/csrc/api.hip
@@ -365,7 +365,7 @@
     return plan_conv(c, true, stats);
 }
 
-enum class WgKern { TAPTABLE, PATCH, PATCH1X1, WGRAD3X3G, WGRAD3X3R, WGRAD3X3D };
+enum class WgKern { TAPTABLE, PATCH, PATCH1X1, WGRAD3X3G, WGRAD3X3R, WGRAD3X3D, WGRAD3X3C };
 struct WgradPlan {
     WgKern kernel;
     int nslabs;
@@ -425,6 +425,15 @@
     p.per_split = per;
     return p;
 }
+WgradPlan plan_wgrad3x3c(const unetrir_conv_geom* g) {
+    const WgradPlan cap = plan_patch(WgKern::PATCH, WG_BF16_TPH_S1, WG_TPW, g);
+    const Wgrad3ArgsH a = wgrad3_args<Wgrad3ArgsH>(g, nullptr, g->Cin, nullptr, g->Cout);
+    WgradPlan p{WgKern::WGRAD3X3C};
+    int per;
+    wgrad3x3c_plan(a, cap.nslabs, &p.nslabs, &per);
+    p.per_split = per;
+    return p;
+}
 WgradPlan plan_taptable(const unetrir_conv_geom* g) {
     WgradArgs a{};
     wgrad_args(g, g->Cin, g->Cout, &a);
@@ -439,6 +448,7 @@
     if (g->k == 3 && !bf16) return plan_patch(WgKern::PATCH, s1 ? WG_F32_TPH_S1 : WG_F32_TPH_S2, WG_TPW, g);
     if (g->k == 3) {
         const Wgrad3ArgsH a = wgrad3_args<Wgrad3ArgsH>(g, nullptr, ldx, nullptr, lddy);
+        if (s1 && g->Cin <= 8 && wgrad3x3c_applies(a, true)) return plan_wgrad3x3c(g);
         if (s1 && cfg.wgrad3x3g && wgrad3x3g_applies(a, true)) return plan_wgrad3x3g(g);
         if (s1 && cfg.wgrad3x3r && wgrad3x3r_applies(a)) return plan_patch(WgKern::WGRAD3X3R, WG_ROW_TPH, WG_ROW_TPW, g);
         if (!s1 && cfg.wgrad3x3d && wgrad3x3d_applies(a, true)) return plan_wgrad3x3d(g);
@@ -456,6 +466,7 @@
         const bool s1 = g->stride == 1;
         cover(plan_patch(WgKern::PATCH, s1 ? WG_F32_TPH_S1 : WG_F32_TPH_S2, WG_TPW, g));
         cover(plan_patch(WgKern::PATCH, s1 ? WG_BF16_TPH_S1 : WG_BF16_TPH_S2, WG_TPW, g));
+        if (s1 && g->Cin <= 8 && wgrad3x3c_applies(a, false)) cover(plan_wgrad3x3c(g));
         if (s1 && wgrad3x3g_applies(a, false)) cover(plan_wgrad3x3g(g));
         if (s1 && wgrad3x3r_applies(a)) cover(plan_patch(WgKern::WGRAD3X3R, WG_ROW_TPH, WG_ROW_TPW, g));
         if (!s1 && wgrad3x3d_applies(a, false)) cover(plan_wgrad3x3d(g));
@@ -488,6 +499,7 @@
         case WgKern::WGRAD3X3G: return launch_wgrad3x3g_bf16(a, p.nslabs, s);
         case WgKern::WGRAD3X3R: return launch_wgrad3x3r_bf16(a, p.nslabs, s);
         case WgKern::WGRAD3X3D: return launch_wgrad3x3d_bf16(a, p.nslabs, s);
+        case WgKern::WGRAD3X3C: return launch_wgrad3x3c_bf16(a, p.nslabs, (int)p.per_split, s);
         case WgKern::PATCH1X1: return launch_wgrad1x1_bf16(a, g->stride, p.nslabs, s);
         default: return launch_wgrad3x3_bf16(a, g->stride, p.nslabs, s);
     }
@@ -747,6 +759,28 @@
     return launch_dense_dgrad(dy, lddy, w, dx, lddx, B, K, N, ws, ws_bytes, (hipStream_t)stream);
 }
 
+int unetrir_vec1x1_supported(int K, int N) { return vec1x1_applies(K, N) ? 1 : 0; }
+
+int unetrir_vec1x1_fwd_bf16(const float* v, int ldv, const float* w, const float* bias, const unetrir_bf16* a, int lda, unetrir_bf16* z,
+                            int ldz, long long P, int K, int N, unetrir_stream_t stream) {
+    if (!v || !w || !bias || !a || !z || P <= 0 || !vec1x1_applies(K, N) || !ld_ok(ldv, K) || !ldh_ok(lda, N) || !ldh_ok(ldz, N) ||
+        (((uintptr_t)v | (uintptr_t)w | (uintptr_t)a | (uintptr_t)z) & 15))
+        return UNETRIR_EINVAL;
+    ProfScope ps(UNETRIR_FAM_CONV_FWD, 2.0 * (double)P * K * N, (hipStream_t)stream);
+    return launch_vec1x1_fwd_bf16(v, ldv, w, bias, a, lda, z, ldz, P, N, (hipStream_t)stream);
+}
+
+size_t unetrir_vec1x1_bwd_ws_bytes(long long P, int K, int N) { return P > 0 && vec1x1_applies(K, N) ? vec1x1_bwd_ws_bytes(P, N) : 0; }
+
+int unetrir_vec1x1_bwd_bf16(const unetrir_bf16* g, int ldg, const float* v, int ldv, const float* wt, long long P, int K, int N, float* dw,
+                            float* db, float* dv, int lddv, void* ws, size_t ws_bytes, unetrir_stream_t stream) {
+    if (!g || !v || !wt || !dw || !db || !dv || !ws || P <= 0 || !vec1x1_applies(K, N) || !ldh_ok(ldg, N) || ldv < K || lddv < K ||
+        (((uintptr_t)g | (uintptr_t)wt | (uintptr_t)dw | (uintptr_t)db | (uintptr_t)ws) & 15) || ws_bytes < vec1x1_bwd_ws_bytes(P, N))
+        return UNETRIR_EINVAL;
+    ProfScope ps(UNETRIR_FAM_CONV_WGRAD, 4.0 * (double)P * K * N, (hipStream_t)stream);
+    return launch_vec1x1_bwd_bf16(g, ldg, v, ldv, wt, P, N, dw, db, dv, lddv, ws, (hipStream_t)stream);
+}
+
 int unetrir_transpose_weight_f32(const float* w, float* wt, int N, int T, int C, unetrir_stream_t stream) {
     if (!w || !wt || N <= 0 || T <= 0 || C <= 0) return UNETRIR_EINVAL;
     return launch_transpose_weight(w, wt, N, T, C, (hipStream_t)stream);
diff --git a/unet-rir_amd/csrc/kernels.h b/unet-rir_amd/csrc/kernels.h
--- a/unet-rir_amd/csrc/kernels.h
+++ b/unet-rir_amd/csrc/kernels.h
@@ -110,6 +110,9 @@
 bool wgrad3x3d_applies(const Wgrad3ArgsH& a, bool with_ld);
 void wgrad3x3d_plan(int B, int OH, int OW, int N, int C, int* nsplit, int* per_split, int* npy, int* npx);
 int launch_wgrad3x3d_bf16(Wgrad3ArgsH a, int nslabs, hipStream_t s);
+bool wgrad3x3c_applies(const Wgrad3ArgsH& a, bool with_ld);
+void wgrad3x3c_plan(const Wgrad3ArgsH& a, int max_slabs, int* nslabs, int* units_per_slab);
+int launch_wgrad3x3c_bf16(const Wgrad3ArgsH& a, int nslabs, int units_per_slab, hipStream_t s);
 int launch_cast_weight(const float* w, void* o, int N, int T, int C, int Cp, hipStream_t s);
 int launch_cast_weights_batched(const unetrir_cast_desc* desc_dev, int n_layers, hipStream_t s);
 int launch_transpose_cast_weight(const float* w, void* wt, int N, int T, int C, int Np, hipStream_t s);
@@ -180,6 +183,13 @@
 long long pw1x1_colstat_rows(const PwArgs& a);
 int launch_pw1x1_bf16(const PwArgs& a, hipStream_t s);
 
+bool vec1x1_applies(int K, int N);
+size_t vec1x1_bwd_ws_bytes(long long P, int N);
+int launch_vec1x1_fwd_bf16(const float* v, int ldv, const float* w, const float* bias, const void* a, int lda, void* z, int ldz,
+                           long long P, int N, hipStream_t s);
+int launch_vec1x1_bwd_bf16(const void* g, int ldg, const float* v, int ldv, const float* wt, long long P, int N, float* dw, float* db,
+                           float* dv, int lddv, void* ws, hipStream_t s);
+
 __device__ __forceinline__ unsigned long long mix64(unsigned long long z) {
     z = (z ^ (z >> 30)) * 0xBF58476D1CE4E5B9ULL;
     z = (z ^ (z >> 27)) * 0x94D049BB133111EBULL;
diff --git a/unet-rir_amd/csrc/vec1x1.hip b/unet-rir_amd/csrc/vec1x1.hip
--- /dev/null
+++ b/unet-rir_amd/csrc/vec1x1.hip
@@ -0,0 +1,185 @@
+#include <hip/hip_runtime.h>
+#include <stdint.h>
+#include "kernels.h"
+
+typedef float vc_f32x16 __attribute__((ext_vector_type(16)));
+typedef float vc_f32x4 __attribute__((ext_vector_type(4)));
+typedef __bf16 vc_bf16x8 __attribute__((ext_vector_type(8)));
+
+#define VC_K 16
+#define VC_FWD_N 256
+#define VC_BWD_P 64
+#define VC_BWD_N 128
+
+bool vec1x1_applies(int K, int N) { return K == VC_K && N >= 64 && N <= 4096 && (N & 63) == 0; }
+
+extern "C" __global__ __launch_bounds__(256) void vec1x1_fwd_bf16_kernel(const float* __restrict__ v, int ldv, const float* __restrict__ w,
+                                                                         const float* __restrict__ bias, const __bf16* __restrict__ a, int lda,
+                                                                         __bf16* __restrict__ z, int ldz, long long P, int N) {
+    const int lane = threadIdx.x & 63, wave = threadIdx.x >> 6;
+    const long long p0 = ((long long)blockIdx.x * 4 + wave) * 32;
+    if (p0 >= P) return;
+    const int nl = blockIdx.y * VC_FWD_N + 8 * (lane & 31);
+    const bool nok = nl < N;
+    const int koff = (lane >> 5) * 4;
+
+    float4 fa[2], fb[8][2];
+    const long long pa = p0 + (lane & 31);
+#pragma unroll
+    for (int kk = 0; kk < 2; ++kk) {
+        fa[kk] = make_float4(0.f, 0.f, 0.f, 0.f);
+        if (pa < P) fa[kk] = *reinterpret_cast<const float4*>(v + pa * ldv + kk * 8 + koff);
+    }
+#pragma unroll
+    for (int j = 0; j < 8; ++j)
+#pragma unroll
+        for (int kk = 0; kk < 2; ++kk) {
+            fb[j][kk] = make_float4(0.f, 0.f, 0.f, 0.f);
+            if (nok) fb[j][kk] = *reinterpret_cast<const float4*>(w + (size_t)(nl + j) * VC_K + kk * 8 + koff);
+        }
+    float bs[8];
+#pragma unroll
+    for (int j = 0; j < 8; ++j) bs[j] = nok ? bias[nl + j] : 0.f;
+
+    vc_f32x16 acc[8];
+#pragma unroll
+    for (int j = 0; j < 8; ++j)
+#pragma unroll
+        for (int r = 0; r < 16; ++r) acc[j][r] = 0.f;
+#pragma unroll
+    for (int kk = 0; kk < 2; ++kk) {
+#pragma unroll
+        for (int j = 0; j < 8; ++j) acc[j] = __builtin_amdgcn_mfma_f32_32x32x2f32(fa[kk].x, fb[j][kk].x, acc[j], 0, 0, 0);
+#pragma unroll
+        for (int j = 0; j < 8; ++j) acc[j] = __builtin_amdgcn_mfma_f32_32x32x2f32(fa[kk].y, fb[j][kk].y, acc[j], 0, 0, 0);
+#pragma unroll
+        for (int j = 0; j < 8; ++j) acc[j] = __builtin_amdgcn_mfma_f32_32x32x2f32(fa[kk].z, fb[j][kk].z, acc[j], 0, 0, 0);
+#pragma unroll
+        for (int j = 0; j < 8; ++j) acc[j] = __builtin_amdgcn_mfma_f32_32x32x2f32(fa[kk].w, fb[j][kk].w, acc[j], 0, 0, 0);
+    }
+    if (!nok) return;
+#pragma unroll
+    for (int r = 0; r < 16; ++r) {
+        const long long p = p0 + (r & 3) + 8 * (r >> 2) + 4 * (lane >> 5);
+        if (p >= P) continue;
+        const vc_bf16x8 x = *reinterpret_cast<const vc_bf16x8*>(a + p * lda + nl);
+        vc_bf16x8 o;
+#pragma unroll
+        for (int j = 0; j < 8; ++j) {
+            const float c = acc[j][r] + bs[j];
+            o[j] = (__bf16)((float)x[j] + c);
+        }
+        *reinterpret_cast<vc_bf16x8*>(z + p * ldz + nl) = o;
+    }
+}
+
+extern "C" __global__ __launch_bounds__(256) void vec1x1_bwd_bf16_kernel(const __bf16* __restrict__ g, int ldg, const float* __restrict__ v, int ldv,
+                                                                         const float* __restrict__ wt, long long P, int N,
+                                                                         float* __restrict__ dwpart, float* __restrict__ dbpart,
+                                                                         float* __restrict__ dv, int lddv) {
+    const int lane = threadIdx.x & 63, wave = threadIdx.x >> 6;
+    const int li = lane & 15, q = lane >> 4;
+    const long long P0 = (long long)blockIdx.x * VC_BWD_P;
+
+    if (P0 + 16 * wave < P) {
+        const long long p = P0 + 16 * wave + li;
+        const bool pok = p < P;
+        const __bf16* gp = g + (pok ? p : 0) * ldg + q * 8;
+        const float* wp = wt + (size_t)li * N + q * 8;
+        vc_f32x4 acc = {0.f, 0.f, 0.f, 0.f};
+        for (int c = 0; c < N; c += 32) {
+            vc_bf16x8 x = *reinterpret_cast<const vc_bf16x8*>(gp + c);
+            const float4 b0 = *reinterpret_cast<const float4*>(wp + c), b1 = *reinterpret_cast<const float4*>(wp + c + 4);
+            float ge[8];
+#pragma unroll
+            for (int e = 0; e < 8; ++e) ge[e] = pok ? (float)x[e] : 0.f;
+            acc = __builtin_amdgcn_mfma_f32_16x16x4f32(ge[0], b0.x, acc, 0, 0, 0);
+            acc = __builtin_amdgcn_mfma_f32_16x16x4f32(ge[1], b0.y, acc, 0, 0, 0);
+            acc = __builtin_amdgcn_mfma_f32_16x16x4f32(ge[2], b0.z, acc, 0, 0, 0);
+            acc = __builtin_amdgcn_mfma_f32_16x16x4f32(ge[3], b0.w, acc, 0, 0, 0);
+            acc = __builtin_amdgcn_mfma_f32_16x16x4f32(ge[4], b1.x, acc, 0, 0, 0);
+            acc = __builtin_amdgcn_mfma_f32_16x16x4f32(ge[5], b1.y, acc, 0, 0, 0);
+            acc = __builtin_amdgcn_mfma_f32_16x16x4f32(ge[6], b1.z, acc, 0, 0, 0);
+            acc = __builtin_amdgcn_mfma_f32_16x16x4f32(ge[7], b1.w, acc, 0, 0, 0);
+        }
+#pragma unroll
+        for (int r = 0; r < 4; ++r) {
+            const long long pp = P0 + 16 * wave + 4 * q + r;
+            if (pp < P) dv[pp * lddv + li] = acc[r];
+        }
+    }
+
+    float* dws = dwpart + (size_t)blockIdx.x * N * VC_K;
+    float* dbs = dbpart + (size_t)blockIdx.x * N;
+    const int ncg = (N + VC_BWD_N - 1) / VC_BWD_N;
+    for (int cg = wave; cg < ncg; cg += 4) {
+        const int n0 = cg * VC_BWD_N + li * 8;
+        const bool nok = n0 < N;
+        vc_f32x4 acc[8];
+        float dbv[8];
+#pragma unroll
+        for (int e = 0; e < 8; ++e) { acc[e] = vc_f32x4{0.f, 0.f, 0.f, 0.f}; dbv[e] = 0.f; }
+#pragma unroll 4
+        for (int s = 0; s < VC_BWD_P / 4; ++s) {
+            const long long p = P0 + 4 * s + q;
+            const bool pok = p < P;
+            vc_bf16x8 x;
+#pragma unroll
+            for (int e = 0; e < 8; ++e) x[e] = (__bf16)0.f;
+            if (pok && nok) x = *reinterpret_cast<const vc_bf16x8*>(g + p * ldg + n0);
+            const float b = pok ? v[p * ldv + li] : 0.f;
+#pragma unroll
+            for (int e = 0; e < 8; ++e) {
+                const float ge = (float)x[e];
+                dbv[e] += ge;
+                acc[e] = __builtin_amdgcn_mfma_f32_16x16x4f32(ge, b, acc[e], 0, 0, 0);
+            }
+        }
+#pragma unroll
+        for (int e = 0; e < 8; ++e) {
+            float t = dbv[e];
+            t += __shfl_xor(t, 16);
+            t += __shfl_xor(t, 32);
+            dbv[e] = t;
+        }
+        if (q == 0 && nok) {
+            *reinterpret_cast<float4*>(dbs + n0) = make_float4(dbv[0], dbv[1], dbv[2], dbv[3]);
+            *reinterpret_cast<float4*>(dbs + n0 + 4) = make_float4(dbv[4], dbv[5], dbv[6], dbv[7]);
+        }
+#pragma unroll
+        for (int e = 0; e < 8; ++e)
+#pragma unroll
+            for (int r = 0; r < 4; ++r) {
+                const int n = cg * VC_BWD_N + 8 * (4 * q + r) + e;
+                if (n < N) dws[(size_t)n * VC_K + li] = acc[e][r];
+            }
+    }
+}
+
+static inline long long vec1x1_slabs(long long P) { return (P + VC_BWD_P - 1) / VC_BWD_P; }
+
+size_t vec1x1_bwd_ws_bytes(long long P, int N) { return (size_t)vec1x1_slabs(P) * N * (VC_K + 1) * sizeof(float); }
+
+int launch_vec1x1_fwd_bf16(const float* v, int ldv, const float* w, const float* bias, const void* a, int lda, void* z, int ldz,
+                           long long P, int N, hipStream_t s) {
+    const long long gx = (P + 127) / 128;
+    if (gx > 0x7fffffffLL) return UNETRIR_EINVAL;
+    hipLaunchKernelGGL(vec1x1_fwd_bf16_kernel, dim3((unsigned)gx, (unsigned)((N + VC_FWD_N - 1) / VC_FWD_N)), dim3(256), 0, s, v, ldv, w,
+                       bias, (const __bf16*)a, lda, (__bf16*)z, ldz, P, N);
+    return (int)hipGetLastError();
+}
+
+int launch_vec1x1_bwd_bf16(const void* g, int ldg, const float* v, int ldv, const float* wt, long long P, int N, float* dw, float* db,
+                           float* dv, int lddv, void* ws, hipStream_t s) {
+    const long long S = vec1x1_slabs(P);
+    if (S > 0x7fffffffLL) return UNETRIR_EINVAL;
+    float* dwpart = (float*)ws;
+    float* dbpart = dwpart + (size_t)S * N * VC_K;
+    hipLaunchKernelGGL(vec1x1_bwd_bf16_kernel, dim3((unsigned)S), dim3(256), 0, s, (const __bf16*)g, ldg, v, ldv, wt, P, N, dwpart, dbpart,
+                       dv, lddv);
+    int err = (int)hipGetLastError();
+    if (err) return err;
+    err = launch_splitk_reduce(dwpart, (int)S, (size_t)N * VC_K, dw, 0.f, nullptr, s);
+    if (err) return err;
+    return launch_splitk_reduce(dbpart, (int)S, (size_t)N, db, 0.f, nullptr, s);
+}
diff --git a/unet-rir_amd/csrc/wgrad3x3c.hip b/unet-rir_amd/csrc/wgrad3x3c.hip
--- /dev/null
+++ b/unet-rir_amd/csrc/wgrad3x3c.hip
@@ -0,0 +1,157 @@
+#include <hip/hip_runtime.h>
+#include <stdint.h>
+#include "kernels.h"
+
+typedef float wc_f32x4 __attribute__((ext_vector_type(4)));
+typedef __bf16 wc_bf16x4 __attribute__((ext_vector_type(4)));
+typedef __bf16 wc_bf16x8 __attribute__((ext_vector_type(8)));
+typedef __attribute__((address_space(3))) wc_bf16x4 wc_lds_bf16x4;
+
+#define WC_PX 64
+#define WC_XW (WC_PX + 2)
+#define WC_XBYTES (3 * WC_XW * 16 + 64)
+
+template <int NG>
+__global__ __launch_bounds__(256, NG <= 4 ? 2 : 1) void wgrad3x3c_bf16_kernel(const Wgrad3ArgsH a, int units, int units_per_slab, int nch) {
+    constexpr int N = NG * 16;
+    constexpr int DS = N * 2 + 32;
+    constexpr int WAVE_BYTES = WC_PX * DS + WC_XBYTES;
+    constexpr int RED_BYTES = N * 80 * 4;
+    constexpr int SMEM = 4 * WAVE_BYTES > RED_BYTES ? 4 * WAVE_BYTES : RED_BYTES;
+    constexpr int GP = N / 8;
+    __shared__ __attribute__((aligned(16))) unsigned char smem[SMEM];
+    const int lane = threadIdx.x & 63, wave = threadIdx.x >> 6;
+    const int l15 = lane & 15, lq = lane >> 4;
+    unsigned char* dsm = smem + wave * WAVE_BYTES;
+    unsigned char* xsm = dsm + WC_PX * DS;
+    if (lane < 4) *reinterpret_cast<uint4*>(xsm + 3 * WC_XW * 16 + lane * 16) = make_uint4(0u, 0u, 0u, 0u);
+
+    const int u_begin = blockIdx.x * units_per_slab;
+    const int u_end = min(units, u_begin + units_per_slab);
+
+    uint4 rd[GP], rx[4];
+    auto load_unit = [&](int u) {
+        const int R = u / nch, ci = u - R * nch;
+        const int img = R / a.OH, y = R - img * a.OH;
+        const int c0 = ci * WC_PX;
+        const __bf16* dyr = a.dy + ((size_t)R * a.OW + c0) * a.lddy;
+#pragma unroll
+        for (int j = 0; j < GP; ++j) {
+            const int idx = lane + 64 * j;
+            const int px = idx / GP, gr = idx - px * GP;
+            uint4 v = make_uint4(0u, 0u, 0u, 0u);
+            if (c0 + px < a.OW) v = *reinterpret_cast<const uint4*>(dyr + (size_t)px * a.lddy + gr * 8);
+            rd[j] = v;
+        }
+#pragma unroll
+        for (int j = 0; j < 4; ++j) {
+            const int idx = lane + 64 * j;
+            const int rr = idx / WC_XW, px = idx - rr * WC_XW;
+            const int iy = y - a.pad_t + rr, ix = c0 - a.pad_l + px;
+            uint4 v = make_uint4(0u, 0u, 0u, 0u);
+            if (idx < 3 * WC_XW && (unsigned)iy < (unsigned)a.IH && (unsigned)ix < (unsigned)a.IW)
+                v = *reinterpret_cast<const uint4*>(a.x + (((size_t)img * a.IH + iy) * a.IW + ix) * a.ldx);
+            rx[j] = v;
+        }
+    };
+
+    wc_f32x4 acc[NG][5];
+#pragma unroll
+    for (int g = 0; g < NG; ++g)
+#pragma unroll
+        for (int c = 0; c < 5; ++c) acc[g][c] = wc_f32x4{0.f, 0.f, 0.f, 0.f};
+
+    const int tr_r = l15 >> 2, tr_p = l15 & 3;
+    const int a_off = (4 * lq + tr_r) * DS + tr_p * 8;
+    int b_off[5];
+#pragma unroll
+    for (int cg = 0; cg < 5; ++cg) {
+        const int t = 2 * cg + (tr_p >> 1);
+        const int kh = t / 3, kw = t - kh * 3;
+        b_off[cg] = t < 9 ? ((kh * WC_XW + kw + 4 * lq + tr_r) * 16 + (tr_p & 1) * 8) : -1;
+    }
+    const int zero_off = 3 * WC_XW * 16 + (tr_p & 1) * 8;
+
+    int u = u_begin + wave;
+    if (u < u_end) load_unit(u);
+    for (; u < u_end; u += 4) {
+#pragma unroll
+        for (int j = 0; j < GP; ++j) {
+            const int idx = lane + 64 * j;
+            const int px = idx / GP, gr = idx - px * GP;
+            *reinterpret_cast<uint4*>(dsm + px * DS + gr * 16) = rd[j];
+        }
+#pragma unroll
+        for (int j = 0; j < 4; ++j) {
+            const int idx = lane + 64 * j;
+            if (idx < 3 * WC_XW) *reinterpret_cast<uint4*>(xsm + idx * 16) = rx[j];
+        }
+        if (u + 4 < u_end) load_unit(u + 4);
+#pragma unroll
+        for (int ks = 0; ks < 2; ++ks) {
+            wc_bf16x8 fb[5];
+#pragma unroll
+            for (int cg = 0; cg < 5; ++cg) {
+                const unsigned char* p0 = b_off[cg] >= 0 ? xsm + b_off[cg] + ks * 32 * 16 : xsm + zero_off;
+                const unsigned char* p1 = b_off[cg] >= 0 ? p0 + 16 * 16 : p0;
+                const wc_bf16x4 lo = __builtin_amdgcn_ds_read_tr16_b64_v4bf16((wc_lds_bf16x4*)p0);
+                const wc_bf16x4 hi = __builtin_amdgcn_ds_read_tr16_b64_v4bf16((wc_lds_bf16x4*)p1);
+                fb[cg] = __builtin_shufflevector(lo, hi, 0, 1, 2, 3, 4, 5, 6, 7);
+            }
+#pragma unroll
+            for (int g = 0; g < NG; ++g) {
+                const unsigned char* p0 = dsm + a_off + g * 32 + ks * 32 * DS;
+                const wc_bf16x4 lo = __builtin_amdgcn_ds_read_tr16_b64_v4bf16((wc_lds_bf16x4*)p0);
+                const wc_bf16x4 hi = __builtin_amdgcn_ds_read_tr16_b64_v4bf16((wc_lds_bf16x4*)(p0 + 16 * DS));
+                const wc_bf16x8 fa = __builtin_shufflevector(lo, hi, 0, 1, 2, 3, 4, 5, 6, 7);
+#pragma unroll
+                for (int cg = 0; cg < 5; ++cg) acc[g][cg] = __builtin_amdgcn_mfma_f32_16x16x32_bf16(fa, fb[cg], acc[g][cg], 0, 0, 0);
+            }
+        }
+    }
+
+    float* red = reinterpret_cast<float*>(smem);
+    for (int w = 0; w < 4; ++w) {
+        __syncthreads();
+        if (wave != w) continue;
+#pragma unroll
+        for (int g = 0; g < NG; ++g)
+#pragma unroll
+            for (int cg = 0; cg < 5; ++cg)
+#pragma unroll
+                for (int r = 0; r < 4; ++r) {
+                    const int n = 16 * g + 4 * lq + r, col = 16 * cg + l15;
+                    float v = acc[g][cg][r];
+                    if (w > 0) v += red[n * 80 + col];
+                    if (w < 3) red[n * 80 + col] = v;
+                    else if (col < 72) a.part[((size_t)blockIdx.x * N + n) * 72 + col] = v;
+                }
+    }
+}
+
+bool wgrad3x3c_applies(const Wgrad3ArgsH& a, bool with_ld) {
+    (void)with_ld;
+    return a.C == 8 && (a.N == 32 || a.N == 64 || a.N == 128) && a.pad_t == 1 && a.pad_l == 1 && a.OH == a.IH && a.OW == a.IW;
+}
+
+void wgrad3x3c_plan(const Wgrad3ArgsH& a, int max_slabs, int* nslabs, int* units_per_slab) {
+    const int nch = (a.OW + WC_PX - 1) / WC_PX;
+    const long long units = (long long)a.B * a.OH * nch;
+    if (max_slabs < 1) max_slabs = 1;
+    long long per = (units + max_slabs - 1) / max_slabs;
+    if (per < 1) per = 1;
+    *units_per_slab = (int)per;
+    *nslabs = (int)((units + per - 1) / per);
+}
+
+int launch_wgrad3x3c_bf16(const Wgrad3ArgsH& a, int nslabs, int units_per_slab, hipStream_t s) {
+    const int nch = (a.OW + WC_PX - 1) / WC_PX;
+    const long long units = (long long)a.B * a.OH * nch;
+    if (units > 0x7fffffffLL || (long long)nslabs * units_per_slab < units) return UNETRIR_EINVAL;
+    const dim3 grid((unsigned)nslabs), block(256);
+    if (a.N == 32) hipLaunchKernelGGL(wgrad3x3c_bf16_kernel<2>, grid, block, 0, s, a, (int)units, units_per_slab, nch);
+    else if (a.N == 64) hipLaunchKernelGGL(wgrad3x3c_bf16_kernel<4>, grid, block, 0, s, a, (int)units, units_per_slab, nch);
+    else if (a.N == 128) hipLaunchKernelGGL(wgrad3x3c_bf16_kernel<8>, grid, block, 0, s, a, (int)units, units_per_slab, nch);
+    else return UNETRIR_EINVAL;
+    return (int)hipGetLastError();
+}
diff --git a/unet-rir_amd/engine.py b/unet-rir_amd/engine.py
--- a/unet-rir_amd/engine.py
+++ b/unet-rir_amd/engine.py
@@ -52,6 +52,7 @@
 
 class UNetEngine(EngineBase):
     mask_on_side_stream = True
+    fuse_vec1x1 = True
 
     def __init__(self, H, W, B, F0=32, k=3, depth=4, batchnorm=True, inf_vector_shape=(2, 16), s0=1, s=2,
                  device="cuda:0", n_replicas=1, dtype="f32", overlap_wgrad=False, runtime=None, share=None):
@@ -190,7 +191,8 @@
             for d_ in (self.ya, self.aa, self.yb, self.ab, self.g_ya, self.g_aa, self.g_yb, self.g_ab):
                 d_[l] = A(h, w, c)
         self.logits, self.g_logits = F(self.H, self.W, 4), A(self.H, self.W, PAD)
-        if self.dtype == "bf16":
+        self.vec_fused = self.dtype == "bf16" and self.fuse_vec1x1 and ops.vec1x1_supported(self.g_z, VEC_CH, cL)
+        if self.dtype == "bf16" and not self.vec_fused:
             self.v1x1, self.g_z32 = F(self.h5, self.w5, cL), F(self.h5, self.w5, cL)
         self.pred = torch.empty((B, 2, self.H, self.W), dtype=torch.float32, device=dev)
         self.loss_out = torch.zeros(4, dtype=torch.float32, device=dev)
@@ -237,6 +239,8 @@
             need = max(need, ops.bn_ws_bytes(self.B * h * w, 2 * self.ch[l - 1]))
         if self.dense_direct:
             need = max(need, _lib.lib().unetrir_dense_dgrad_ws_bytes(self.B, self.vec_in, self.vec_dim))
+        if self.vec_fused:
+            need = max(need, ops.vec1x1_bwd_ws_bytes(self.B * self.h5 * self.w5, VEC_CH, self.ch[-1]))
         self.ws.reserve(need)
 
     def wf(self, name):
@@ -324,7 +328,7 @@
                 vsp_ = self.vd_sp
             else:
                 vsp_ = Act(self.v.base.view(B, self.h5, self.w5, VEC_CH))
-            if self.dtype != "f32":
+            if self.dtype != "f32" and not self.vec_fused:
                 ops.conv2d_fwd(self.geo["vec.conv"], vsp_, p["vec.conv.kernel"], p["vec.conv.bias"], self.v1x1)
             return vsp_
 
@@ -345,6 +349,8 @@
             self._join_wg()
         if self.dtype == "f32":
             ops.conv2d_fwd(self.geo["vec.conv"], vsp, p["vec.conv.kernel"], p["vec.conv.bias"], self.z, addend=self.a[self.L])
+        elif self.vec_fused:
+            ops.vec1x1_fwd(vsp, p["vec.conv.kernel"], p["vec.conv.bias"], self.a[self.L], self.z)
         else:
             ops.add_f32_to_bf16(self.a[self.L], self.v1x1, self.z)
         cur = self.z
@@ -434,12 +440,15 @@
         vsp = self.vd_sp if has_do else Act(self.v.base.view(B, self.h5, self.w5, VEC_CH))
         with self._wg() as ws_:
             gz = self.g_z
-            if self.dtype == "bf16":
-                ops.cast_bf16_to_f32(self.g_z, self.g_z32)
-                gz = self.g_z32
-            ops.conv2d_wgrad(self.geo["vec.conv"], vsp, gz, g["vec.conv.kernel"], ws_)
-            ops.colsum(gz, g["vec.conv.bias"], ws_)
-            ops.conv2d_dgrad(self.geo["vec.conv"], gz, pt["vec.conv.kernel"], self.g_vd_sp)
+            if self.vec_fused:
+                ops.vec1x1_bwd(gz, vsp, pt["vec.conv.kernel"], g["vec.conv.kernel"], g["vec.conv.bias"], self.g_vd_sp, ws_)
+            else:
+                if self.dtype == "bf16":
+                    ops.cast_bf16_to_f32(self.g_z, self.g_z32)
+                    gz = self.g_z32
+                ops.conv2d_wgrad(self.geo["vec.conv"], vsp, gz, g["vec.conv.kernel"], ws_)
+                ops.colsum(gz, g["vec.conv.bias"], ws_)
+                ops.conv2d_dgrad(self.geo["vec.conv"], gz, pt["vec.conv.kernel"], self.g_vd_sp)
             if has_do:
                 ops.mul(self.g_vd.base, self._mask, self.g_v.base)
                 gv = self.g_v
diff --git a/unet-rir_amd/ops.py b/unet-rir_amd/ops.py
--- a/unet-rir_amd/ops.py
+++ b/unet-rir_amd/ops.py
@@ -298,6 +298,25 @@
 
 def cast_bf16_to_f32(a: Act, y: Act):
     check(_lib.lib().unetrir_cast_bf16_to_f32(_p(a), _p(y), a.base.numel(), _stream()), "cast_bf16_to_f32")
+
+
+def vec1x1_supported(trunk: Act, K, N):
+    return trunk.sfx == "bf16" and trunk.base.is_cuda and bool(_lib.lib().unetrir_vec1x1_supported(int(K), int(N)))
+
+
+def vec1x1_fwd(v: Act, w, bias, a: Act, z: Act):
+    check(_lib.lib().unetrir_vec1x1_fwd_bf16(_p(v), v.ld, _p(w), _p(bias), _p(a), a.ld, _p(z), z.ld, a.P, v.C, a.C, _stream()),
+          "vec1x1_fwd")
+
+
+def vec1x1_bwd_ws_bytes(P, K, N):
+    return int(_lib.lib().unetrir_vec1x1_bwd_ws_bytes(int(P), int(K), int(N)))
+
+
+def vec1x1_bwd(g: Act, v: Act, wt, dw, db, dv: Act, ws: Workspace):
+    ws.reserve(vec1x1_bwd_ws_bytes(g.P, v.C, g.C))
+    check(_lib.lib().unetrir_vec1x1_bwd_bf16(_p(g), g.ld, _p(v), v.ld, _p(wt), g.P, v.C, g.C, _p(dw), _p(db), _p(dv), dv.ld, ws.ptr,
+                                             ws.nbytes, _stream()), "vec1x1_bwd")
 
 
 
```
